# nihaomiao/CVPR23_LFDM

Measured on AMD Instinct MI355X. Metric: 40-frame 128x128 videos/sec (DDIM-100), higher is better.
Workload: dtype f32; 1 GPU; MUG 128x128, 40-frame DDIM-100 sample, batch=1 per GPU (BASELINE.json configs[1]); global_batch=1, frames=40, latent=32, image=128, sampler=DDIM-100 eta=1, cond_scale=1, parallelism=replicas x1 (videos sharded, no collective)

## Files before the change

### cvpr23_lfdm_amd/csrc/attention.hip

```cpp
#include <stdlib.h>
#include "lfdm_device.h"
#include "../../include/lfdm_hip.h"

namespace {

constexpr int HEADS = 8;
constexpr int DH = 32;
constexpr int QKV_LD = 3 * HEADS * DH;
constexpr int OUT_LD = HEADS * DH;

template <int LP>
__global__ __launch_bounds__(64) void attention_kernel(const float* __restrict__ qkv, float* __restrict__ out, int batch,
                                                       int frames, int hw, int mode, const float* __restrict__ bias,
                                                       const float* __restrict__ rot_cos,
                                                       const float* __restrict__ rot_sin) {
  constexpr int NT = LP / 16;

  const int lane = threadIdx.x & 63;
  const int l15 = lane & 15, lq = lane >> 4;
  const int L = mode == 0 ? frames : hw;
  const int64_t unit = blockIdx.x;
  const int64_t seq = unit / HEADS;
  const int head = (int)(unit - seq * HEADS);
  int64_t row0, tstride;
  if (mode == 0) {
    const int64_t b = seq / hw, pix = seq - b * hw;
    row0 = b * frames * hw + pix;
    tstride = hw;
  } else {
    row0 = seq * hw;
    tstride = 1;
  }
  const float scale = 0.17677669529663687f;
  const float* base = qkv + head * DH;

  float qf[NT][8], kf[NT][8];
#pragma unroll
  for (int ti = 0; ti < NT; ++ti) {
    const int t = ti * 16 + l15;
    float4 q0 = make_float4(0.f, 0.f, 0.f, 0.f), q1 = q0, k0 = q0, k1 = q0;
    if (t < L) {
      const float* src = base + (row0 + (int64_t)t * tstride) * QKV_LD + 8 * lq;
      q0 = *reinterpret_cast<const float4*>(src);
      q1 = *reinterpret_cast<const float4*>(src + 4);
      k0 = *reinterpret_cast<const float4*>(src + OUT_LD);
      k1 = *reinterpret_cast<const float4*>(src + OUT_LD + 4);
    }
    qf[ti][0] = q0.x * scale; qf[ti][1] = q0.y * scale; qf[ti][2] = q0.z * scale; qf[ti][3] = q0.w * scale;
    qf[ti][4] = q1.x * scale; qf[ti][5] = q1.y * scale; qf[ti][6] = q1.z * scale; qf[ti][7] = q1.w * scale;
    kf[ti][0] = k0.x; kf[ti][1] = k0.y; kf[ti][2] = k0.z; kf[ti][3] = k0.w;
    kf[ti][4] = k1.x; kf[ti][5] = k1.y; kf[ti][6] = k1.z; kf[ti][7] = k1.w;
  }
  float vf[2][4 * NT];
#pragma unroll
  for (int tj = 0; tj < NT; ++tj)
#pragma unroll
    for (int r = 0; r < 4; ++r) {
      const int t = 16 * tj + 4 * lq + r;
      vf[0][4 * tj + r] = vf[1][4 * tj + r] = 0.f;
      if (t < L) {
        const float* src = base + (row0 + (int64_t)t * tstride) * QKV_LD + 2 * OUT_LD;
        vf[0][4 * tj + r] = src[l15];
        vf[1][4 * tj + r] = src[16 + l15];
      }
    }
  if (rot_cos) {
#pragma unroll
    for (int ti = 0; ti < NT; ++ti) {
      const int t = ti * 16 + l15;
      if (t < L) {
#pragma unroll
        for (int pr = 0; pr < 4; ++pr) {
          const float c = rot_cos[t * 16 + 4 * lq + pr], sn = rot_sin[t * 16 + 4 * lq + pr];
          const float qx = qf[ti][2 * pr], qy = qf[ti][2 * pr + 1];
          const float kx = kf[ti][2 * pr], ky = kf[ti][2 * pr + 1];
          qf[ti][2 * pr] = qx * c - qy * sn;
          qf[ti][2 * pr + 1] = qy * c + qx * sn;
          kf[ti][2 * pr] = kx * c - ky * sn;
          kf[ti][2 * pr + 1] = ky * c + kx * sn;
        }
      }
    }
  }

  f32x4 st[NT][NT];
#pragma unroll
  for (int ti = 0; ti < NT; ++ti)
#pragma unroll
    for (int tj = 0; tj < NT; ++tj) {
      f32x4 acc = {0.f, 0.f, 0.f, 0.f};
#pragma unroll
      for (int s = 0; s < 8; ++s) acc = mfma_16x16x4(kf[tj][s], qf[ti][s], acc);
      st[ti][tj] = acc;
    }
  const bool bias_vec = bias && (L % 4 == 0) && ((((uintptr_t)bias) & 15) == 0);
#pragma unroll
  for (int ti = 0; ti < NT; ++ti) {
    const int qt = ti * 16 + l15;
    float m = -3.0e38f;
#pragma unroll
    for (int tj = 0; tj < NT; ++tj) {
      float bv[4] = {0.f, 0.f, 0.f, 0.f};
      const int key0 = tj * 16 + lq * 4;
      if (bias && qt < L && key0 < L) {
        const float* bp = bias + ((int64_t)head * L + qt) * L + key0;
        if (bias_vec) {
          const float4 b4 = *reinterpret_cast<const float4*>(bp);
          bv[0] = b4.x; bv[1] = b4.y; bv[2] = b4.z; bv[3] = b4.w;
        } else {
#pragma unroll
          for (int r = 0; r < 4; ++r) bv[r] = (key0 + r < L) ? bp[r] : 0.f;
        }
      }
#pragma unroll
      for (int r = 0; r < 4; ++r) {
        float v = st[ti][tj][r];
        if (key0 + r >= L) v = -3.0e38f;
        else v += bv[r];
        st[ti][tj][r] = v;
        m = fmaxf(m, v);
      }
    }
    m = fmaxf(m, __shfl_xor(m, 16));
    m = fmaxf(m, __shfl_xor(m, 32));
    float sum = 0.f;
#pragma unroll
    for (int tj = 0; tj < NT; ++tj)
#pragma unroll
      for (int r = 0; r < 4; ++r) {
        const float e = (tj * 16 + lq * 4 + r) < L ? expf(st[ti][tj][r] - m) : 0.f;
        st[ti][tj][r] = e;
        sum += e;
      }
    sum += __shfl_xor(sum, 16);
    sum += __shfl_xor(sum, 32);
#pragma unroll
    for (int tj = 0; tj < NT; ++tj)
#pragma unroll
      for (int r = 0; r < 4; ++r) st[ti][tj][r] = st[ti][tj][r] / sum;
  }

#pragma unroll
  for (int ti = 0; ti < NT; ++ti) {
    f32x4 o[2];
    o[0] = (f32x4){0.f, 0.f, 0.f, 0.f};
    o[1] = o[0];
#pragma unroll
    for (int tj = 0; tj < NT; ++tj)
#pragma unroll
      for (int r = 0; r < 4; ++r) {
        o[0] = mfma_16x16x4(st[ti][tj][r], vf[0][4 * tj + r], o[0]);
        o[1] = mfma_16x16x4(st[ti][tj][r], vf[1][4 * tj + r], o[1]);
      }
#pragma unroll
    for (int r = 0; r < 4; ++r) {
      const int t = ti * 16 + lq * 4 + r;
      if (t < L) {
        float* dst = out + (row0 + (int64_t)t * tstride) * OUT_LD + head * DH;
        dst[l15] = o[0][r];
        dst[16 + l15] = o[1][r];
      }
    }
  }
}

__global__ __launch_bounds__(256) void linattn_context_kernel(const float* __restrict__ qkv, int hw,
                                                              float* __restrict__ ctx_out) {
  __shared__ float red[4][32];
  __shared__ float kmax[32];
  __shared__ float ek[64][33];
  __shared__ __attribute__((aligned(16))) float vv[64][36];
  const int tid = threadIdx.x;
  const int f = blockIdx.x >> 3, h = blockIdx.x & 7;
  const float* kbase = qkv + (int64_t)f * hw * QKV_LD + OUT_LD + h * DH;
  const float* vbase = kbase + OUT_LD;

  {
    const int c4 = tid & 7, part = tid >> 3;
    float4 m = make_float4(-3.0e38f, -3.0e38f, -3.0e38f, -3.0e38f);
    for (int n = part; n < hw; n += 128) {
      float4 v[4];
#pragma unroll
      for (int u = 0; u < 4; ++u) {
        const int nn = n + 32 * u;
        v[u] = nn < hw ? *reinterpret_cast<const float4*>(kbase + (int64_t)nn * QKV_LD + 4 * c4) : m;
      }
#pragma unroll
      for (int u = 0; u < 4; ++u) {
        m.x = fmaxf(m.x, v[u].x); m.y = fmaxf(m.y, v[u].y); m.z = fmaxf(m.z, v[u].z); m.w = fmaxf(m.w, v[u].w);
      }
    }
#pragma unroll
    for (int x = 8; x <= 32; x <<= 1) {
      m.x = fmaxf(m.x, __shfl_xor(m.x, x)); m.y = fmaxf(m.y, __shfl_xor(m.y, x));
      m.z = fmaxf(m.z, __shfl_xor(m.z, x)); m.w = fmaxf(m.w, __shfl_xor(m.w, x));
    }
    if ((tid & 63) < 8) {
      const int w = tid >> 6;
      red[w][4 * c4 + 0] = m.x; red[w][4 * c4 + 1] = m.y; red[w][4 * c4 + 2] = m.z; red[w][4 * c4 + 3] = m.w;
    }
    __syncthreads();
    if (tid < 32) kmax[tid] = fmaxf(fmaxf(red[0][tid], red[1][tid]), fmaxf(red[2][tid], red[3][tid]));
    __syncthreads();
  }

  const int d = tid >> 3, e0 = (tid & 7) * 4;
  float acc[4] = {0.f, 0.f, 0.f, 0.f};
  float ssum = 0.f;
  const int ln = tid >> 3, lc4 = tid & 7;
  float4 rk[2], rv[2];
  auto load_tile = [&](int n0) {
#pragma unroll
    for (int u = 0; u < 2; ++u) {
      const int n = n0 + ln + 32 * u;
      rk[u] = rv[u] = make_float4(0.f, 0.f, 0.f, 0.f);
      if (n < hw) {
        rk[u] = *reinterpret_cast<const float4*>(kbase + (int64_t)n * QKV_LD + 4 * lc4);
        rv[u] = *reinterpret_cast<const float4*>(vbase + (int64_t)n * QKV_LD + 4 * lc4);
      }
    }
  };
  load_tile(0);
  for (int n0 = 0; n0 < hw; n0 += 64) {
#pragma unroll
    for (int u = 0; u < 2; ++u) {
      const int nl = ln + 32 * u;
      const bool ok = n0 + nl < hw;
      ek[nl][4 * lc4 + 0] = ok ? expf(rk[u].x - kmax[4 * lc4 + 0]) : 0.f;
      ek[nl][4 * lc4 + 1] = ok ? expf(rk[u].y - kmax[4 * lc4 + 1]) : 0.f;
      ek[nl][4 * lc4 + 2] = ok ? expf(rk[u].z - kmax[4 * lc4 + 2]) : 0.f;
      ek[nl][4 * lc4 + 3] = ok ? expf(rk[u].w - kmax[4 * lc4 + 3]) : 0.f;
      *reinterpret_cast<float4*>(&vv[nl][4 * lc4]) = rv[u];
    }
    __syncthreads();
    if (n0 + 64 < hw) load_tile(n0 + 64);
#pragma unroll 8
    for (int n = 0; n < 64; ++n) {
      const float e = ek[n][d];
      const float4 v4 = *reinterpret_cast<const float4*>(&vv[n][e0]);
      acc[0] = fmaf(e, v4.x, acc[0]);
      acc[1] = fmaf(e, v4.y, acc[1]);
      acc[2] = fmaf(e, v4.z, acc[2]);
      acc[3] = fmaf(e, v4.w, acc[3]);
      ssum += e;
    }
    __syncthreads();
  }
  float* dst = ctx_out + ((int64_t)blockIdx.x * DH + d) * DH + e0;
  dst[0] = acc[0] / ssum;
  dst[1] = acc[1] / ssum;
  dst[2] = acc[2] / ssum;
  dst[3] = acc[3] / ssum;
}

__global__ __launch_bounds__(256) void linattn_output_kernel(const float* __restrict__ qkv,
                                                             const float* __restrict__ ctx, int hw,
                                                             float* __restrict__ out) {
  constexpr int CS = DH * DH + 4;
  __shared__ __attribute__((aligned(16))) float cs[HEADS * CS];
  const int tid = threadIdx.x;
  const int f = blockIdx.y;
  for (int i = tid; i < HEADS * DH * DH; i += 256) {
    const int h = i / (DH * DH), r = i - h * DH * DH;
    cs[h * CS + r] = ctx[(int64_t)f * HEADS * DH * DH + i];
  }
  __syncthreads();
  const int tok = blockIdx.x * 32 + (tid >> 3), h = tid & 7;
  if (tok >= hw) return;
  const int64_t row = (int64_t)f * hw + tok;
  const float* qp = qkv + row * QKV_LD + h * DH;
  float q[DH];
#pragma unroll
  for (int i = 0; i < DH / 4; ++i) {
    const float4 v = reinterpret_cast<const float4*>(qp)[i];
    q[4 * i] = v.x; q[4 * i + 1] = v.y; q[4 * i + 2] = v.z; q[4 * i + 3] = v.w;
  }
  float m = q[0];
#pragma unroll
  for (int i = 1; i < DH; ++i) m = fmaxf(m, q[i]);
  float sum = 0.f;
#pragma unroll
  for (int i = 0; i < DH; ++i) {
    q[i] = expf(q[i] - m);
    sum += q[i];
  }
  const float scale = 0.17677669529663687f;
#pragma unroll
  for (int i = 0; i < DH; ++i) q[i] = q[i] / sum * scale;
  float* op = out + row * OUT_LD + h * DH;
  const float* ch = cs + h * CS;
#pragma unroll
  for (int e4 = 0; e4 < DH / 4; ++e4) {
    float4 o = make_float4(0.f, 0.f, 0.f, 0.f);
#pragma unroll
    for (int dd = 0; dd < DH; ++dd) {
      const float4 c = *reinterpret_cast<const float4*>(ch + dd * DH + 4 * e4);
      o.x = fmaf(c.x, q[dd], o.x);
      o.y = fmaf(c.y, q[dd], o.y);
      o.z = fmaf(c.z, q[dd], o.z);
      o.w = fmaf(c.w, q[dd], o.w);
    }
    reinterpret_cast<float4*>(op)[e4] = o;
  }
}

}

extern "C" int lfdm_attention_cl_f32(const float* qkv, float* out, int batch, int frames, int hw,
                                     int mode, const float* bias, const float* rot_cos,
                                     const float* rot_sin, lfdm_stream_t stream_) {
  hipStream_t stream = (hipStream_t)stream_;
  const int L = mode == 0 ? frames : hw;
  if (!qkv || !out || batch <= 0 || frames <= 0 || hw <= 0 || (mode != 0 && mode != 1) ||
      L > 64 || ((rot_cos == nullptr) != (rot_sin == nullptr))) {
    lfdm_set_error("attention: unsupported shape (sequence length must be <= 64)");
    return LFDM_EINVAL;
  }
  const int64_t nseq = mode == 0 ? (int64_t)batch * hw : (int64_t)batch * frames;
  const int64_t units = nseq * HEADS;
  const dim3 grid((unsigned)units), block(64);
  if (L <= 16) LFDM_LAUNCH((attention_kernel<16>), grid, block, 0, stream, qkv, out, batch, frames, hw, mode, bias, rot_cos, rot_sin);
  else if (L <= 32) LFDM_LAUNCH((attention_kernel<32>), grid, block, 0, stream, qkv, out, batch, frames, hw, mode, bias, rot_cos, rot_sin);
  else if (L <= 48) LFDM_LAUNCH((attention_kernel<48>), grid, block, 0, stream, qkv, out, batch, frames, hw, mode, bias, rot_cos, rot_sin);
  else LFDM_LAUNCH((attention_kernel<64>), grid, block, 0, stream, qkv, out, batch, frames, hw, mode, bias, rot_cos, rot_sin);
  return lfdm_check_launch("attention");
}

extern "C" size_t lfdm_linear_attention_ws_bytes(int n_frames) {
  return (size_t)n_frames * HEADS * DH * DH * sizeof(float);
}

extern "C" int lfdm_linear_attention_cl_f32(const float* qkv, float* out, int n_frames, int hw,
                                            void* ws, size_t ws_bytes, lfdm_stream_t stream_) {
  hipStream_t stream = (hipStream_t)stream_;
  if (!qkv || !out || n_frames <= 0 || hw <= 0) {
    lfdm_set_error("linear_attention: bad arguments");
    return LFDM_EINVAL;
  }
  if (!ws || ws_bytes < lfdm_linear_attention_ws_bytes(n_frames)) {
    lfdm_set_error("linear_attention: workspace too small");
    return LFDM_EWORKSPACE;
  }
  float* ctx = reinterpret_cast<float*>(ws);
  LFDM_LAUNCH(linattn_context_kernel, dim3(n_frames * HEADS), dim3(256), 0, stream, qkv, hw, ctx);
  LFDM_LAUNCH(linattn_output_kernel, dim3((hw + 31) / 32, n_frames), dim3(256), 0, stream, qkv,
              (const float*)ctx, hw, out);
  return lfdm_check_launch("linear_attention");
}
```

### cvpr23_lfdm_amd/csrc/attention_fused.hip

```cpp
#include <stdlib.h>

#include "lfdm_device.h"
#include "../../include/lfdm_hip.h"

namespace {

constexpr int HEADS = 8;
constexpr int DH = 32;
constexpr int OUT_LD = HEADS * DH;

#if defined(LFDM_EMU_BUILD)
static inline float fast_exp(float x) { return expf(x); }
#else
__device__ __forceinline__ float fast_exp(float x) { return __expf(x); }
#endif

template <int NT>
__device__ __forceinline__ void attend_store(const float (&qf)[NT][8], const float (&kf)[NT][8], const float (&vf)[2][4 * NT],
                                             int head, int L, int l15, int lq, const float* __restrict__ bias, bool bias_vec,
                                             float* __restrict__ out, int64_t row0, int hw, float* o_lds = nullptr) {
  f32x4 st[NT][NT];
#pragma unroll
  for (int ti = 0; ti < NT; ++ti)
#pragma unroll
    for (int tj = 0; tj < NT; ++tj) {
      f32x4 acc = {0.f, 0.f, 0.f, 0.f};
#pragma unroll
      for (int s = 0; s < 8; ++s) acc = mfma_16x16x4(kf[tj][s], qf[ti][s], acc);
      st[ti][tj] = acc;
    }
#pragma unroll
  for (int ti = 0; ti < NT; ++ti) {
    const int qt = ti * 16 + l15;
    float m = -3.0e38f;
#pragma unroll
    for (int tj = 0; tj < NT; ++tj) {
      float bv[4] = {0.f, 0.f, 0.f, 0.f};
      const int key0 = tj * 16 + lq * 4;
      if (bias && qt < L && key0 < L) {
        const float* bp = bias + ((int64_t)head * L + qt) * L + key0;
        if (bias_vec) {
          const float4 b4 = *reinterpret_cast<const float4*>(bp);
          bv[0] = b4.x; bv[1] = b4.y; bv[2] = b4.z; bv[3] = b4.w;
        } else {
#pragma unroll
          for (int r = 0; r < 4; ++r) bv[r] = (key0 + r < L) ? bp[r] : 0.f;
        }
      }
#pragma unroll
      for (int r = 0; r < 4; ++r) {
        const float v = (key0 + r >= L) ? -3.0e38f : st[ti][tj][r] + bv[r];
        st[ti][tj][r] = v;
        m = fmaxf(m, v);
      }
    }
    m = fmaxf(m, __shfl_xor(m, 16));
    m = fmaxf(m, __shfl_xor(m, 32));
    float sum = 0.f;
#pragma unroll
    for (int tj = 0; tj < NT; ++tj)
#pragma unroll
      for (int r = 0; r < 4; ++r) {
        const int key = tj * 16 + lq * 4 + r;
        const float e = key < L ? fast_exp(st[ti][tj][r] - m) : 0.f;
        st[ti][tj][r] = e;
        sum += e;
      }
    sum += __shfl_xor(sum, 16);
    sum += __shfl_xor(sum, 32);
    const float inv = 1.0f / sum;
#pragma unroll
    for (int tj = 0; tj < NT; ++tj)
#pragma unroll
      for (int r = 0; r < 4; ++r) st[ti][tj][r] = st[ti][tj][r] * inv;
  }

#pragma unroll
  for (int ti = 0; ti < NT; ++ti) {
    f32x4 o[2];
    o[0] = (f32x4){0.f, 0.f, 0.f, 0.f};
    o[1] = o[0];
#pragma unroll
    for (int tj = 0; tj < NT; ++tj)
#pragma unroll
      for (int r = 0; r < 4; ++r) {
        o[0] = mfma_16x16x4(st[ti][tj][r], vf[0][4 * tj + r], o[0]);
        o[1] = mfma_16x16x4(st[ti][tj][r], vf[1][4 * tj + r], o[1]);
      }
#pragma unroll
    for (int r = 0; r < 4; ++r) {
      const int t = ti * 16 + lq * 4 + r;
      if (t < L) {
        if (o_lds) {
#pragma unroll
          for (int half = 0; half < 2; ++half) {
            const int c = head * DH + 16 * half + l15;
            o_lds[t * OUT_LD + ((((c >> 2) ^ (t & 15)) << 2) | (c & 3))] = o[half][r];
          }
        } else {
          float* dst = out + (row0 + (int64_t)t * hw) * OUT_LD + head * DH;
          dst[l15] = o[0][r];
          dst[16 + l15] = o[1][r];
        }
      }
    }
  }
}

template <int LP, int C, bool ROT_RELOAD = false, bool WPACK = false>
__device__ __forceinline__ void tattn_heads(const float* __restrict__ x, int ldx, int head_begin, int heads_per_block,
                                            const float* __restrict__ wqkv, float* __restrict__ out, int frames, int hw, int64_t seq,
                                            const float* __restrict__ bias, const float* __restrict__ rot_cos,
                                            const float* __restrict__ rot_sin, float eps, float* o_lds) {
  constexpr int NT = LP / 16;
  constexpr int CQ = C / 4;

  const int lane = threadIdx.x & 63;
  const int l15 = lane & 15, lq = lane >> 4;
  const int L = frames;
  const int64_t b = seq / hw, pix = seq - b * hw;
  const int64_t row0 = b * frames * hw + pix;
  const float scale = 0.17677669529663687f;

  float xf[NT][CQ];
#pragma unroll
  for (int ti = 0; ti < NT; ++ti) {
    const int t = ti * 16 + l15;
    float s1 = 0.f, s2 = 0.f;
    if (t < L) {
      const float* src = x + (row0 + (int64_t)t * hw) * ldx + CQ * lq;
#pragma unroll
      for (int q = 0; q < CQ / 4; ++q) {
        const float4 v = *reinterpret_cast<const float4*>(src + 4 * q);
        xf[ti][4 * q] = v.x; xf[ti][4 * q + 1] = v.y; xf[ti][4 * q + 2] = v.z; xf[ti][4 * q + 3] = v.w;
        s1 += (v.x + v.y) + (v.z + v.w);
        s2 += (v.x * v.x + v.y * v.y) + (v.z * v.z + v.w * v.w);
      }
    } else {
#pragma unroll
      for (int s = 0; s < CQ; ++s) xf[ti][s] = 0.f;
    }
    s1 += __shfl_xor(s1, 16); s2 += __shfl_xor(s2, 16);
    s1 += __shfl_xor(s1, 32); s2 += __shfl_xor(s2, 32);
    const float mean = s1 * (1.0f / (float)C);
    float var = s2 * (1.0f / (float)C) - mean * mean;
    if (var < 0.f) var = 0.f;
    const float rstd = 1.0f / sqrtf(var + eps);
    if (t < L) {
#pragma unroll
      for (int s = 0; s < CQ; ++s) xf[ti][s] = (xf[ti][s] - mean) * rstd;
    }
  }

  float rc[NT][4], rs[NT][4];
  if (rot_cos && !ROT_RELOAD) {
#pragma unroll
    for (int ti = 0; ti < NT; ++ti) {
      const int t = ti * 16 + l15;
      const int tt = t < L ? t : 0;
#pragma unroll
      for (int fi = 0; fi < 2; ++fi)
#pragma unroll
        for (int pr = 0; pr < 2; ++pr) {
          rc[ti][2 * fi + pr] = rot_cos[tt * 16 + 8 * fi + 2 * lq + pr];
          rs[ti][2 * fi + pr] = rot_sin[tt * 16 + 8 * fi + 2 * lq + pr];
        }
    }
  }
  const bool bias_vec = bias && (L % 4 == 0) && ((((uintptr_t)bias) & 15) == 0);

#pragma unroll 1
  for (int head = head_begin; head < head_begin + heads_per_block; ++head) {
    float qf[NT][8], kf[NT][8];
    {
      float wa[4][CQ];
#pragma unroll
      for (int g = 0; g < 4; ++g) {
        const float* wsrc = WPACK ? wqkv + ((int64_t)(((g >> 1) * HEADS + head) * 2 + (g & 1)) * (CQ / 4) * 64 + lane) * 4
                                  : wqkv + ((int64_t)((g >> 1) * OUT_LD + head * DH + 16 * (g & 1) + l15)) * C + CQ * lq;
#pragma unroll
        for (int q = 0; q < CQ / 4; ++q) {
          const float4 v = *reinterpret_cast<const float4*>(wsrc + (WPACK ? 256 * q : 4 * q));
          wa[g][4 * q] = v.x; wa[g][4 * q + 1] = v.y; wa[g][4 * q + 2] = v.z; wa[g][4 * q + 3] = v.w;
        }
      }
#pragma unroll
      for (int g = 0; g < 4; ++g) {
        f32x4 acc[NT];
#pragma unroll
        for (int ti = 0; ti < NT; ++ti) acc[ti] = (f32x4){0.f, 0.f, 0.f, 0.f};
#pragma unroll
        for (int s = 0; s < CQ; ++s)
#pragma unroll
          for (int ti = 0; ti < NT; ++ti) acc[ti] = mfma_16x16x4(wa[g][s], xf[ti][s], acc[ti]);
#pragma unroll
        for (int ti = 0; ti < NT; ++ti)
#pragma unroll
          for (int r = 0; r < 4; ++r) {
            if ((g >> 1) == 0) qf[ti][4 * (g & 1) + r] = acc[ti][r] * scale;
            else kf[ti][4 * (g & 1) + r] = acc[ti][r];
          }
      }
    }
    if (rot_cos) {
#pragma unroll
      for (int ti = 0; ti < NT; ++ti) {
#pragma unroll
        for (int fi = 0; fi < 2; ++fi)
#pragma unroll
          for (int pr = 0; pr < 2; ++pr) {
            float c, sn;
            if (ROT_RELOAD) {
              const int t = ti * 16 + l15, tt = t < L ? t : 0;
              c = rot_cos[tt * 16 + 8 * fi + 2 * lq + pr];
              sn = rot_sin[tt * 16 + 8 * fi + 2 * lq + pr];
            } else {
              c = rc[ti][2 * fi + pr];
              sn = rs[ti][2 * fi + pr];
            }
            const float qx = qf[ti][4 * fi + 2 * pr], qy = qf[ti][4 * fi + 2 * pr + 1];
            const float kx = kf[ti][4 * fi + 2 * pr], ky = kf[ti][4 * fi + 2 * pr + 1];
            qf[ti][4 * fi + 2 * pr] = qx * c - qy * sn;
            qf[ti][4 * fi + 2 * pr + 1] = qy * c + qx * sn;
            kf[ti][4 * fi + 2 * pr] = kx * c - ky * sn;
            kf[ti][4 * fi + 2 * pr + 1] = ky * c + kx * sn;
          }
      }
    }
    float vf[2][4 * NT];
    {
      float wb[2][CQ];
#pragma unroll
      for (int half = 0; half < 2; ++half) {
        const float* wsrc = WPACK ? wqkv + ((int64_t)((2 * HEADS + head) * 2 + half) * (CQ / 4) * 64 + lane) * 4
                                  : wqkv + ((int64_t)(2 * OUT_LD + head * DH + 16 * half + l15)) * C + CQ * lq;
#pragma unroll
        for (int q = 0; q < CQ / 4; ++q) {
          const float4 v = *reinterpret_cast<const float4*>(wsrc + (WPACK ? 256 * q : 4 * q));
          wb[half][4 * q] = v.x; wb[half][4 * q + 1] = v.y; wb[half][4 * q + 2] = v.z; wb[half][4 * q + 3] = v.w;
        }
      }
#pragma unroll
      for (int half = 0; half < 2; ++half) {
        f32x4 acc[NT];
#pragma unroll
        for (int ti = 0; ti < NT; ++ti) acc[ti] = (f32x4){0.f, 0.f, 0.f, 0.f};
#pragma unroll
        for (int s = 0; s < CQ; ++s)
#pragma unroll
          for (int ti = 0; ti < NT; ++ti) acc[ti] = mfma_16x16x4(xf[ti][s], wb[half][s], acc[ti]);
#pragma unroll
        for (int ti = 0; ti < NT; ++ti)
#pragma unroll
          for (int r = 0; r < 4; ++r) vf[half][4 * ti + r] = acc[ti][r];
      }
    }

    attend_store<NT>(qf, kf, vf, head, L, l15, lq, bias, bias_vec, out, row0, hw, o_lds);
  }
}

template <int LP, int C>
__global__ __launch_bounds__(64, 2) void temporal_attn_fused_kernel(const float* __restrict__ x, int ldx, int heads_per_block,
                                                                 const float* __restrict__ wqkv,
                                                                 float* __restrict__ out, int batch, int frames, int hw,
                                                                 const float* __restrict__ bias,
                                                                 const float* __restrict__ rot_cos,
                                                                 const float* __restrict__ rot_sin, float eps) {
  tattn_heads<LP, C>(x, ldx, blockIdx.y * heads_per_block, heads_per_block, wqkv, out, frames, hw, blockIdx.x, bias, rot_cos, rot_sin, eps, nullptr);
}

template <int LP, int LROWS, int NW>
__global__ __launch_bounds__(64 * NW, 2) void temporal_attn_fused_out_kernel(const float* __restrict__ x, int ldx,
                                                                          const float* __restrict__ wqkv, const float* __restrict__ wout,
                                                                          float* __restrict__ out, int ldo, int frames, int hw,
                                                                          const float* __restrict__ bias, const float* __restrict__ rot_cos,
                                                                          const float* __restrict__ rot_sin, float eps) {
  constexpr int C = 64, NT = LP / 16, CT = C / 16;
  __shared__ __attribute__((aligned(16))) float o_lds[LROWS * OUT_LD];
  const int wave = lfdm_uniform((int)(threadIdx.x >> 6));
  const int lane = threadIdx.x & 63, l15 = lane & 15, lq = lane >> 4;
  const int L = frames;
  const int64_t seq = blockIdx.x;
  tattn_heads<LP, C, (NW < 8), true>(x, ldx, wave * (HEADS / NW), HEADS / NW, wqkv, nullptr, frames, hw, seq, bias, rot_cos, rot_sin, eps, o_lds);
  __syncthreads();
  const int64_t b = seq / hw, pix = seq - b * hw;
  const int64_t row0 = b * frames * hw + pix;
  for (int tile = wave; tile < NT * CT; tile += NW) {
    const int ti = tile / CT, ct = tile - ti * CT;
    const int t = ti * 16 + l15;
    const int tr = t < L ? t : L - 1;
    const float* arow = o_lds + tr * OUT_LD;
    const float* brow = wout + ((int64_t)ct * (OUT_LD / 16) * 64 + lane) * 4;
    f32x4 acc = {0.f, 0.f, 0.f, 0.f}, acc1 = acc;
    float xr[4];
#pragma unroll
    for (int r = 0; r < 4; ++r) {
      const int tok = ti * 16 + 4 * lq + r;
      xr[r] = x[(row0 + (int64_t)(tok < L ? tok : L - 1) * hw) * ldx + ct * 16 + l15];
    }
#pragma unroll 4
    for (int S = 0; S < OUT_LD / 16; S += 2) {
      const float4 a = *reinterpret_cast<const float4*>(arow + (((4 * S + lq) ^ (tr & 15)) << 2));
      const float4 a1 = *reinterpret_cast<const float4*>(arow + (((4 * S + 4 + lq) ^ (tr & 15)) << 2));
      const float4 w = *reinterpret_cast<const float4*>(brow + 256 * S);
      const float4 w1 = *reinterpret_cast<const float4*>(brow + 256 * S + 256);
      acc = mfma_16x16x4(a.x, w.x, acc);
      acc1 = mfma_16x16x4(a1.x, w1.x, acc1);
      acc = mfma_16x16x4(a.y, w.y, acc);
      acc1 = mfma_16x16x4(a1.y, w1.y, acc1);
      acc = mfma_16x16x4(a.z, w.z, acc);
      acc1 = mfma_16x16x4(a1.z, w1.z, acc1);
      acc = mfma_16x16x4(a.w, w.w, acc);
      acc1 = mfma_16x16x4(a1.w, w1.w, acc1);
    }
#pragma unroll
    for (int r = 0; r < 4; ++r) acc[r] += acc1[r];
#pragma unroll
    for (int r = 0; r < 4; ++r) {
      const int tok = ti * 16 + 4 * lq + r;
      if (tok < L) {
        const int64_t row = row0 + (int64_t)tok * hw;
        out[row * ldo + ct * 16 + l15] = acc[r] + xr[r];
      }
    }
  }
}

template <int LP>
__global__ __launch_bounds__(64, 1) void temporal_attn_fused_wide_kernel(const float* __restrict__ x, int ldx, int channels,
                                                                      int heads_per_block, const float* __restrict__ wqkv,
                                                                      float* __restrict__ out, int batch, int frames, int hw,
                                                                      const float* __restrict__ bias,
                                                                      const float* __restrict__ rot_cos,
                                                                      const float* __restrict__ rot_sin, float eps) {
  constexpr int NT = LP / 16;
  const int lane = threadIdx.x & 63;
  const int l15 = lane & 15, lq = lane >> 4;
  const int L = frames;
  const int64_t seq = blockIdx.x;
  const int64_t b = seq / hw, pix = seq - b * hw;
  const int64_t row0 = b * frames * hw + pix;
  const float scale = 0.17677669529663687f;
  const int ncb = channels / 64;

  float mean[NT], rstd[NT];
#pragma unroll
  for (int ti = 0; ti < NT; ++ti) {
    const int t = ti * 16 + l15;
    float s1 = 0.f, s2 = 0.f;
    if (t < L) {
      const float* src = x + (row0 + (int64_t)t * hw) * ldx + 16 * lq;
      for (int cb = 0; cb < ncb; ++cb)
#pragma unroll
        for (int q = 0; q < 4; ++q) {
          const float4 v = *reinterpret_cast<const float4*>(src + 64 * cb + 4 * q);
          s1 += (v.x + v.y) + (v.z + v.w);
          s2 += (v.x * v.x + v.y * v.y) + (v.z * v.z + v.w * v.w);
        }
    }
    s1 += __shfl_xor(s1, 16); s2 += __shfl_xor(s2, 16);
    s1 += __shfl_xor(s1, 32); s2 += __shfl_xor(s2, 32);
    const float m = s1 / (float)channels;
    float var = s2 / (float)channels - m * m;
    if (var < 0.f) var = 0.f;
    mean[ti] = m;
    rstd[ti] = 1.0f / sqrtf(var + eps);
  }
  const bool bias_vec = bias && (L % 4 == 0) && ((((uintptr_t)bias) & 15) == 0);

  const int head_begin = blockIdx.y * heads_per_block;
#pragma unroll 1
  for (int head = head_begin; head < head_begin + heads_per_block; ++head) {
    f32x4 aq[2][NT], ak[2][NT], av[2][NT];
#pragma unroll
    for (int g = 0; g < 2; ++g)
#pragma unroll
      for (int ti = 0; ti < NT; ++ti) aq[g][ti] = ak[g][ti] = av[g][ti] = (f32x4){0.f, 0.f, 0.f, 0.f};
#pragma unroll 1
    for (int cb = 0; cb < ncb; ++cb) {
      float w[6][16];
#pragma unroll
      for (int g = 0; g < 6; ++g) {
        const float* wsrc = wqkv + ((int64_t)((g >> 1) * OUT_LD + head * DH + 16 * (g & 1) + l15)) * channels + 64 * cb + 16 * lq;
#pragma unroll
        for (int q = 0; q < 4; ++q) {
          const float4 v = *reinterpret_cast<const float4*>(wsrc + 4 * q);
          w[g][4 * q] = v.x; w[g][4 * q + 1] = v.y; w[g][4 * q + 2] = v.z; w[g][4 * q + 3] = v.w;
        }
      }
#pragma unroll
      for (int ti = 0; ti < NT; ++ti) {
        const int t = ti * 16 + l15;
        float xf[16];
        if (t < L) {
          const float* src = x + (row0 + (int64_t)t * hw) * ldx + 64 * cb + 16 * lq;
#pragma unroll
          for (int q = 0; q < 4; ++q) {
            const float4 v = *reinterpret_cast<const float4*>(src + 4 * q);
            xf[4 * q] = (v.x - mean[ti]) * rstd[ti]; xf[4 * q + 1] = (v.y - mean[ti]) * rstd[ti];
            xf[4 * q + 2] = (v.z - mean[ti]) * rstd[ti]; xf[4 * q + 3] = (v.w - mean[ti]) * rstd[ti];
          }
        } else {
#pragma unroll
          for (int s2 = 0; s2 < 16; ++s2) xf[s2] = 0.f;
        }
#pragma unroll
        for (int s2 = 0; s2 < 16; ++s2) {
          aq[0][ti] = mfma_16x16x4(w[0][s2], xf[s2], aq[0][ti]);
          aq[1][ti] = mfma_16x16x4(w[1][s2], xf[s2], aq[1][ti]);
          ak[0][ti] = mfma_16x16x4(w[2][s2], xf[s2], ak[0][ti]);
          ak[1][ti] = mfma_16x16x4(w[3][s2], xf[s2], ak[1][ti]);
          av[0][ti] = mfma_16x16x4(xf[s2], w[4][s2], av[0][ti]);
          av[1][ti] = mfma_16x16x4(xf[s2], w[5][s2], av[1][ti]);
        }
      }
    }
    float qf[NT][8], kf[NT][8], vf[2][4 * NT];
#pragma unroll
    for (int ti = 0; ti < NT; ++ti)
#pragma unroll
      for (int fi = 0; fi < 2; ++fi)
#pragma unroll
        for (int r = 0; r < 4; ++r) {
          qf[ti][4 * fi + r] = aq[fi][ti][r] * scale;
          kf[ti][4 * fi + r] = ak[fi][ti][r];
          vf[fi][4 * ti + r] = av[fi][ti][r];
        }
    if (rot_cos) {
#pragma unroll
      for (int ti = 0; ti < NT; ++ti) {
        const int t = ti * 16 + l15;
        const int tt = t < L ? t : 0;
#pragma unroll
        for (int fi = 0; fi < 2; ++fi)
#pragma unroll
          for (int pr = 0; pr < 2; ++pr) {
            const float c = rot_cos[tt * 16 + 8 * fi + 2 * lq + pr], sn = rot_sin[tt * 16 + 8 * fi + 2 * lq + pr];
            const float qx = qf[ti][4 * fi + 2 * pr], qy = qf[ti][4 * fi + 2 * pr + 1];
            const float kx = kf[ti][4 * fi + 2 * pr], ky = kf[ti][4 * fi + 2 * pr + 1];
            qf[ti][4 * fi + 2 * pr] = qx * c - qy * sn;
            qf[ti][4 * fi + 2 * pr + 1] = qy * c + qx * sn;
            kf[ti][4 * fi + 2 * pr] = kx * c - ky * sn;
            kf[ti][4 * fi + 2 * pr + 1] = ky * c + kx * sn;
          }
      }
    }
    attend_store<NT>(qf, kf, vf, head, L, l15, lq, bias, bias_vec, out, row0, hw);
  }
}

int launch_fused_wide(const float* x, int ldx, int channels, const float* wqkv, float* out, int batch, int frames, int hw,
                      const float* bias, const float* rot_cos, const float* rot_sin, float eps, hipStream_t stream) {
  const int64_t nseq = (int64_t)batch * hw;
  int hpb = 8;
  while (hpb > 1 && nseq * (HEADS / hpb) < 2048) hpb >>= 1;
  const dim3 grid((unsigned)nseq, (unsigned)(HEADS / hpb)), block(64);
  if (frames <= 16) LFDM_LAUNCH((temporal_attn_fused_wide_kernel<16>), grid, block, 0, stream, x, ldx, channels, hpb, wqkv, out, batch, frames, hw, bias, rot_cos, rot_sin, eps);
  else if (frames <= 32) LFDM_LAUNCH((temporal_attn_fused_wide_kernel<32>), grid, block, 0, stream, x, ldx, channels, hpb, wqkv, out, batch, frames, hw, bias, rot_cos, rot_sin, eps);
  else if (frames <= 48) LFDM_LAUNCH((temporal_attn_fused_wide_kernel<48>), grid, block, 0, stream, x, ldx, channels, hpb, wqkv, out, batch, frames, hw, bias, rot_cos, rot_sin, eps);
  else LFDM_LAUNCH((temporal_attn_fused_wide_kernel<64>), grid, block, 0, stream, x, ldx, channels, hpb, wqkv, out, batch, frames, hw, bias, rot_cos, rot_sin, eps);
  return lfdm_check_launch("temporal_attention_fused_wide");
}

template <int C>
int launch_fused(const float* x, int ldx, const float* wqkv, float* out, int batch, int frames, int hw, const float* bias,
                 const float* rot_cos, const float* rot_sin, float eps, hipStream_t stream) {
  const int64_t nseq = (int64_t)batch * hw;
  int hpb = 8;
  while (hpb > 1 && nseq * (HEADS / hpb) < 2048) hpb >>= 1;
  if (const char* e = lfdm_knob("LFDM_TATTN_HPB")) {
    const int v = atoi(e);
    if (v == 1 || v == 2 || v == 4 || v == 8) hpb = v;
  }
  const dim3 grid((unsigned)nseq, (unsigned)(HEADS / hpb)), block(64);
  if (frames <= 16) LFDM_LAUNCH((temporal_attn_fused_kernel<16, C>), grid, block, 0, stream, x, ldx, hpb, wqkv, out, batch, frames, hw, bias, rot_cos, rot_sin, eps);
  else if (frames <= 32) LFDM_LAUNCH((temporal_attn_fused_kernel<32, C>), grid, block, 0, stream, x, ldx, hpb, wqkv, out, batch, frames, hw, bias, rot_cos, rot_sin, eps);
  else if (frames <= 48) LFDM_LAUNCH((temporal_attn_fused_kernel<48, C>), grid, block, 0, stream, x, ldx, hpb, wqkv, out, batch, frames, hw, bias, rot_cos, rot_sin, eps);
  else LFDM_LAUNCH((temporal_attn_fused_kernel<64, C>), grid, block, 0, stream, x, ldx, hpb, wqkv, out, batch, frames, hw, bias, rot_cos, rot_sin, eps);
  return lfdm_check_launch("temporal_attention_fused");
}

template <int LP, int LROWS>
int launch_fused_out_lp(const float* x, int ldx, const float* wqkv, const float* wout, float* out, int ldo, int batch, int frames, int hw,
                        const float* bias, const float* rot_cos, const float* rot_sin, float eps, hipStream_t stream) {
  const int64_t nseq = (int64_t)batch * hw;
  int nw = 2;
  while (nw < 8 && nseq * nw < 2048) nw <<= 1;
  if (const char* e = getenv("LFDM_TATTN_OUT_NW")) {
    const int v = atoi(e);
    if (v == 1 || v == 2 || v == 4 || v == 8) nw = v;
  }
  const dim3 grid((unsigned)nseq);
  if (nw == 1) LFDM_LAUNCH((temporal_attn_fused_out_kernel<LP, LROWS, 1>), grid, dim3(64), 0, stream, x, ldx, wqkv, wout, out, ldo, frames, hw, bias, rot_cos, rot_sin, eps);
  else if (nw == 2) LFDM_LAUNCH((temporal_attn_fused_out_kernel<LP, LROWS, 2>), grid, dim3(128), 0, stream, x, ldx, wqkv, wout, out, ldo, frames, hw, bias, rot_cos, rot_sin, eps);
  else if (nw == 4) LFDM_LAUNCH((temporal_attn_fused_out_kernel<LP, LROWS, 4>), grid, dim3(256), 0, stream, x, ldx, wqkv, wout, out, ldo, frames, hw, bias, rot_cos, rot_sin, eps);
  else LFDM_LAUNCH((temporal_attn_fused_out_kernel<LP, LROWS, 8>), grid, dim3(512), 0, stream, x, ldx, wqkv, wout, out, ldo, frames, hw, bias, rot_cos, rot_sin, eps);
  return lfdm_check_launch("temporal_attention_fused_out");
}

}

extern "C" int lfdm_temporal_attention_fused_out_cl_f32(const float* x, int ldx, int channels, const float* wqkv, const float* wout,
                                                        float* out, int ldo, int batch, int frames, int hw, const float* bias,
                                                        const float* rot_cos, const float* rot_sin, float ln_eps, lfdm_stream_t stream_) {
  hipStream_t stream = (hipStream_t)stream_;
  if (!x || !wqkv || !wout || !out || batch <= 0 || frames <= 0 || frames > 64 || hw <= 0 || channels != 64 || ldx < 64 || ldx % 4 != 0 ||
      ldo < 64 || (((uintptr_t)x | (uintptr_t)wqkv | (uintptr_t)wout) & 15) || ((rot_cos == nullptr) != (rot_sin == nullptr)) || out == x) {
    lfdm_set_error("temporal_attention_fused_out: needs C == 64, frames <= 64, 16-byte aligned rows, out != x");
    return LFDM_EINVAL;
  }
  if (frames <= 16) return launch_fused_out_lp<16, 16>(x, ldx, wqkv, wout, out, ldo, batch, frames, hw, bias, rot_cos, rot_sin, ln_eps, stream);
  if (frames <= 32) return launch_fused_out_lp<32, 32>(x, ldx, wqkv, wout, out, ldo, batch, frames, hw, bias, rot_cos, rot_sin, ln_eps, stream);
  if (frames <= 40) return launch_fused_out_lp<48, 40>(x, ldx, wqkv, wout, out, ldo, batch, frames, hw, bias, rot_cos, rot_sin, ln_eps, stream);
  if (frames <= 48) return launch_fused_out_lp<48, 48>(x, ldx, wqkv, wout, out, ldo, batch, frames, hw, bias, rot_cos, rot_sin, ln_eps, stream);
  return launch_fused_out_lp<64, 64>(x, ldx, wqkv, wout, out, ldo, batch, frames, hw, bias, rot_cos, rot_sin, ln_eps, stream);
}

extern "C" int lfdm_temporal_attention_fused_cl_f32(const float* x, int ldx, int channels, const float* wqkv, float* out,
                                                    int batch, int frames, int hw, const float* bias,
                                                    const float* rot_cos, const float* rot_sin, float ln_eps,
                                                    lfdm_stream_t stream_) {
  hipStream_t stream = (hipStream_t)stream_;
  if (!x || !wqkv || !out || batch <= 0 || frames <= 0 || frames > 64 || hw <= 0 || ldx < channels || ldx % 4 != 0 ||
      (((uintptr_t)x | (uintptr_t)wqkv) & 15) || ((rot_cos == nullptr) != (rot_sin == nullptr)) ||
      channels < 64 || channels % 64 != 0) {
    lfdm_set_error("temporal_attention_fused: needs C % 64 == 0, frames <= 64, 16-byte aligned rows");
    return LFDM_EINVAL;
  }
  if (channels == 64) return launch_fused<64>(x, ldx, wqkv, out, batch, frames, hw, bias, rot_cos, rot_sin, ln_eps, stream);
  return launch_fused_wide(x, ldx, channels, wqkv, out, batch, frames, hw, bias, rot_cos, rot_sin, ln_eps, stream);
}
```

### cvpr23_lfdm_amd/csrc/attn_lowres.hip

```cpp
#include <stdlib.h>

#include "lfdm_device.h"
#include "../../include/lfdm_hip.h"

namespace {

constexpr int HEADS = 8;
constexpr int DH = 32;
constexpr int OUT_LD = HEADS * DH;
constexpr int NQ = 3 * DH;
constexpr int LDQ = NQ + 4;
constexpr float ATT_SCALE = 0.17677669529663687f;

template <int NT, int D>
__device__ __forceinline__ void project_wave_d(const float* __restrict__ x, int ldx, int64_t row0, int64_t rstride, int nrows,
                                               int c_begin, int c_end, const float* __restrict__ wf, int C, int head,
                                               f32x4 (&acc)[NT][6], float (&s1)[NT], float (&s2)[NT]) {
  const int lane = threadIdx.x & 63, l15 = lane & 15, ks = lane >> 4;
  const float* arow[NT];
#pragma unroll
  for (int ti = 0; ti < NT; ++ti) {
    int r = 16 * ti + l15;
    if (r >= nrows) r = nrows - 1;
    arow[ti] = x + (row0 + (int64_t)r * rstride) * ldx + 4 * ks;
    s1[ti] = s2[ti] = 0.f;
  }
  const float* brow[6];
#pragma unroll
  for (int nj = 0; nj < 6; ++nj) {
    const int gcol = (nj >> 1) * OUT_LD + head * DH + (nj & 1) * 16 + l15;
    brow[nj] = wf + (int64_t)gcol * C + 4 * ks;
#pragma unroll
    for (int ti = 0; ti < NT; ++ti) acc[ti][nj] = (f32x4){0.f, 0.f, 0.f, 0.f};
  }
  float4 ra[D][NT], rb[D][6];
  const int last = c_end - 16;
#pragma unroll
  for (int d = 0; d < D; ++d) {
    const int c = c_begin + 16 * d < last ? c_begin + 16 * d : last;
#pragma unroll
    for (int ti = 0; ti < NT; ++ti) ra[d][ti] = *reinterpret_cast<const float4*>(arow[ti] + c);
#pragma unroll
    for (int nj = 0; nj < 6; ++nj) rb[d][nj] = *reinterpret_cast<const float4*>(brow[nj] + c);
  }
  for (int c0 = c_begin; c0 < c_end; c0 += 16 * D) {
#pragma unroll
    for (int d = 0; d < D; ++d) {
      float4 a[NT], b[6];
#pragma unroll
      for (int ti = 0; ti < NT; ++ti) a[ti] = ra[d][ti];
#pragma unroll
      for (int nj = 0; nj < 6; ++nj) b[nj] = rb[d][nj];
      const int cn = c0 + 16 * (d + D) < last ? c0 + 16 * (d + D) : last;
#pragma unroll
      for (int ti = 0; ti < NT; ++ti) ra[d][ti] = *reinterpret_cast<const float4*>(arow[ti] + cn);
#pragma unroll
      for (int nj = 0; nj < 6; ++nj) rb[d][nj] = *reinterpret_cast<const float4*>(brow[nj] + cn);
#pragma unroll
      for (int ti = 0; ti < NT; ++ti) {
        s1[ti] += (a[ti].x + a[ti].y) + (a[ti].z + a[ti].w);
        s2[ti] += (a[ti].x * a[ti].x + a[ti].y * a[ti].y) + (a[ti].z * a[ti].z + a[ti].w * a[ti].w);
      }
#pragma unroll
      for (int nj = 0; nj < 6; ++nj)
#pragma unroll
        for (int ti = 0; ti < NT; ++ti) {
          acc[ti][nj] = mfma_16x16x4(a[ti].x, b[nj].x, acc[ti][nj]);
          acc[ti][nj] = mfma_16x16x4(a[ti].y, b[nj].y, acc[ti][nj]);
          acc[ti][nj] = mfma_16x16x4(a[ti].z, b[nj].z, acc[ti][nj]);
          acc[ti][nj] = mfma_16x16x4(a[ti].w, b[nj].w, acc[ti][nj]);
        }
    }
  }
#pragma unroll
  for (int ti = 0; ti < NT; ++ti) {
    s1[ti] += __shfl_xor(s1[ti], 16); s2[ti] += __shfl_xor(s2[ti], 16);
    s1[ti] += __shfl_xor(s1[ti], 32); s2[ti] += __shfl_xor(s2[ti], 32);
  }
}

template <int NT, int G, int D>
__device__ __forceinline__ void project_wave_asm(const float* __restrict__ x, int ldx, int64_t row0, int64_t rstride, int nrows,
                                                 int c_begin, const float* __restrict__ wf, int C, int head,
                                                 f32x4 (&acc)[NT][6], float (&s1)[NT], float (&s2)[NT]) {
  const int lane = threadIdx.x & 63, l15 = lane & 15, ks = lane >> 4;
  const float* arow[NT];
#pragma unroll
  for (int ti = 0; ti < NT; ++ti) {
    int r = 16 * ti + l15;
    if (r >= nrows) r = nrows - 1;
    arow[ti] = x + (row0 + (int64_t)r * rstride) * ldx + c_begin + 4 * ks;
    s1[ti] = s2[ti] = 0.f;
  }
  const float* brow[6];
#pragma unroll
  for (int nj = 0; nj < 6; ++nj) {
    const int gcol = (nj >> 1) * OUT_LD + head * DH + (nj & 1) * 16 + l15;
    brow[nj] = wf + (int64_t)gcol * C + c_begin + 4 * ks;
#pragma unroll
    for (int ti = 0; ti < NT; ++ti) acc[ti][nj] = (f32x4){0.f, 0.f, 0.f, 0.f};
  }
  f32x4 ra[D][NT], rb[D][6];
  auto issue = [&](auto gc) {
    constexpr int g = decltype(gc)::value, st = g % D;
    lfdm_static_for<0, NT>([&](auto ti) { lfdm_gload_f4<64 * g>(ra[st][decltype(ti)::value], arow[decltype(ti)::value]); });
    lfdm_static_for<0, 6>([&](auto nj) { lfdm_gload_f4<64 * g>(rb[st][decltype(nj)::value], brow[decltype(nj)::value]); });
  };
  lfdm_static_for<0, (D < G ? D : G)>(issue);
  lfdm_static_for<0, G>([&](auto gc) {
    constexpr int g = decltype(gc)::value, st = g % D;
    constexpr int younger = (G - 1 - g) < (D - 1) ? (G - 1 - g) : (D - 1);
    lfdm_vmwait<younger * (NT + 6)>();
#pragma unroll
    for (int ti = 0; ti < NT; ++ti) lfdm_tie(ra[st][ti]);
#pragma unroll
    for (int nj = 0; nj < 6; ++nj) lfdm_tie(rb[st][nj]);
    f32x4 a[NT], b[6];
#pragma unroll
    for (int ti = 0; ti < NT; ++ti) a[ti] = ra[st][ti];
#pragma unroll
    for (int nj = 0; nj < 6; ++nj) b[nj] = rb[st][nj];
    if constexpr (NT <= 2 && g + D < G) issue(std::integral_constant<int, g + D>{});
#pragma unroll
    for (int ti = 0; ti < NT; ++ti) {
      s1[ti] += (a[ti][0] + a[ti][1]) + (a[ti][2] + a[ti][3]);
      s2[ti] += (a[ti][0] * a[ti][0] + a[ti][1] * a[ti][1]) + (a[ti][2] * a[ti][2] + a[ti][3] * a[ti][3]);
    }
#pragma unroll
    for (int e = 0; e < 4; ++e)
#pragma unroll
      for (int nj = 0; nj < 6; ++nj)
#pragma unroll
        for (int ti = 0; ti < NT; ++ti) acc[ti][nj] = mfma_16x16x4(a[ti][e], b[nj][e], acc[ti][nj]);
    if constexpr (NT > 2 && g + D < G) issue(std::integral_constant<int, g + D>{});
  });
#pragma unroll
  for (int ti = 0; ti < NT; ++ti) {
    s1[ti] += __shfl_xor(s1[ti], 16); s2[ti] += __shfl_xor(s2[ti], 16);
    s1[ti] += __shfl_xor(s1[ti], 32); s2[ti] += __shfl_xor(s2[ti], 32);
  }
}

template <int NT, bool ASM = true>
__device__ __forceinline__ void project_wave(const float* __restrict__ x, int ldx, int64_t row0, int64_t rstride, int nrows,
                                             int c_begin, int c_end, const float* __restrict__ wf, int C, int head,
                                             f32x4 (&acc)[NT][6], float (&s1)[NT], float (&s2)[NT]) {
  const int groups = ASM ? (c_end - c_begin) >> 4 : 0;
  constexpr int D = NT == 1 ? 4 : 2;
  if (groups == 8) project_wave_asm<NT, 8, D>(x, ldx, row0, rstride, nrows, c_begin, wf, C, head, acc, s1, s2);
  else if (groups == 4) project_wave_asm<NT, 4, D>(x, ldx, row0, rstride, nrows, c_begin, wf, C, head, acc, s1, s2);
  else if (groups == 2) project_wave_asm<NT, 2, 2>(x, ldx, row0, rstride, nrows, c_begin, wf, C, head, acc, s1, s2);
  else project_wave_d<NT, 1>(x, ldx, row0, rstride, nrows, c_begin, c_end, wf, C, head, acc, s1, s2);
}

template <int NT, bool ASM = true>
__device__ __forceinline__ void project_ksplit(const float* __restrict__ x, int ldx, int64_t row0, int64_t rstride, int nrows,
                                               const float* __restrict__ wf, int C, int head, float eps, float* part,
                                               float* pstat, float* wsl, float wsum_val) {
  constexpr int R = 16 * NT;
  const int tid = threadIdx.x, lane = tid & 63, wave = tid >> 6, l15 = lane & 15, ks = lane >> 4;
  f32x4 acc[NT][6];
  float s1[NT], s2[NT];
  const int cw = C / 4;
  project_wave<NT, ASM>(x, ldx, row0, rstride, nrows, wave * cw, (wave + 1) * cw, wf, C, head, acc, s1, s2);
  float* mine = part + wave * (R * LDQ);
  if (tid < NQ) wsl[tid] = wsum_val;
#pragma unroll
  for (int ti = 0; ti < NT; ++ti) {
    if (ks == 0) {
      pstat[(0 * 4 + wave) * R + 16 * ti + l15] = s1[ti];
      pstat[(1 * 4 + wave) * R + 16 * ti + l15] = s2[ti];
    }
#pragma unroll
    for (int nj = 0; nj < 6; ++nj)
#pragma unroll
      for (int r = 0; r < 4; ++r) mine[(16 * ti + 4 * ks + r) * LDQ + 16 * nj + l15] = acc[ti][nj][r];
  }
  __syncthreads();
  const float inv_c = 1.0f / (float)C;
  for (int it = tid; it < R * (NQ / 4); it += 256) {
    const int row = it / (NQ / 4), q4 = it - row * (NQ / 4);
    float sv = 0.f, qv = 0.f;
#pragma unroll
    for (int w = 0; w < 4; ++w) {
      sv += pstat[(0 * 4 + w) * R + row];
      qv += pstat[(1 * 4 + w) * R + row];
    }
    const float mean = sv * inv_c;
    float var = qv * inv_c - mean * mean;
    if (var < 0.f) var = 0.f;
    const float rstd = 1.0f / sqrtf(var + eps);
    float4 v = *reinterpret_cast<const float4*>(part + row * LDQ + 4 * q4);
#pragma unroll
    for (int w = 1; w < 4; ++w) {
      const float4 u = *reinterpret_cast<const float4*>(part + w * (R * LDQ) + row * LDQ + 4 * q4);
      v.x += u.x; v.y += u.y; v.z += u.z; v.w += u.w;
    }
    const float4 ws = *reinterpret_cast<const float4*>(wsl + 4 * q4);
    v.x = rstd * (v.x - mean * ws.x); v.y = rstd * (v.y - mean * ws.y);
    v.z = rstd * (v.z - mean * ws.z); v.w = rstd * (v.w - mean * ws.w);
    *reinterpret_cast<float4*>(part + row * LDQ + 4 * q4) = v;
  }
  __syncthreads();
}

__device__ __forceinline__ float load_wsum(const float* __restrict__ wsum, int head) {
  const int tid = threadIdx.x;
  return tid < NQ ? wsum[(tid >> 5) * OUT_LD + head * DH + (tid & 31)] : 0.f;
}

template <int NT, bool MSPLIT>
__global__ __launch_bounds__(256) void linattn_lowres_kernel(const float* __restrict__ x, int ldx, int C,
                                                             const float* __restrict__ wf, const float* __restrict__ wsum,
                                                             float* __restrict__ out, int hw, float eps) {
  constexpr int R = 16 * NT;
  constexpr int ROWS = MSPLIT ? 4 * R : R;
  __shared__ __attribute__((aligned(16))) float qkv[(MSPLIT ? ROWS : 4 * R) * LDQ];
  __shared__ float pstat[2 * 4 * R];
  __shared__ __attribute__((aligned(16))) float wsl[NQ];
  __shared__ float red[8][DH], kmax[DH], ksum[DH];
  __shared__ __attribute__((aligned(16))) float ctx[DH][DH + 4];
  const int tid = threadIdx.x, lane = tid & 63, wave = tid >> 6, l15 = lane & 15, ks = lane >> 4;
  const int f = blockIdx.x >> 3, head = blockIdx.x & 7;
  const int64_t row0 = (int64_t)f * hw;
  const float wsum_val = load_wsum(wsum, head);

  if (MSPLIT) {
    f32x4 acc[NT][6];
    float s1[NT], s2[NT];
    const int nrows_w = hw - wave * R;
    project_wave<NT>(x, ldx, row0 + wave * R, 1, nrows_w < R ? nrows_w : R, 0, C, wf, C, head, acc, s1, s2);
    if (tid < NQ) wsl[tid] = wsum_val;
    if (ks == 0) {
#pragma unroll
      for (int ti = 0; ti < NT; ++ti) {
        const float mean = s1[ti] / (float)C;
        float var = s2[ti] / (float)C - mean * mean;
        if (var < 0.f) var = 0.f;
        pstat[wave * R + 16 * ti + l15] = mean;
        pstat[4 * R + wave * R + 16 * ti + l15] = 1.0f / sqrtf(var + eps);
      }
    }
    __syncthreads();
#pragma unroll
    for (int ti = 0; ti < NT; ++ti)
#pragma unroll
      for (int r = 0; r < 4; ++r) {
        const int rl = 16 * ti + 4 * ks + r;
        const float mean = pstat[wave * R + rl], rstd = pstat[4 * R + wave * R + rl];
#pragma unroll
        for (int nj = 0; nj < 6; ++nj)
          qkv[(wave * R + rl) * LDQ + 16 * nj + l15] = rstd * (acc[ti][nj][r] - mean * wsl[16 * nj + l15]);
      }
    __syncthreads();
  } else {
    project_ksplit<NT>(x, ldx, row0, 1, hw, wf, C, head, eps, qkv, pstat, wsl, wsum_val);
  }

  {
    const int d = tid & 31, part = tid >> 5;
    float m = -3.0e38f;
    for (int n = part; n < hw; n += 8) m = fmaxf(m, qkv[n * LDQ + DH + d]);
    red[part][d] = m;
    __syncthreads();
    if (tid < DH) {
      float mm = red[0][tid];
#pragma unroll
      for (int p = 1; p < 8; ++p) mm = fmaxf(mm, red[p][tid]);
      kmax[tid] = mm;
    }
    __syncthreads();
    const float mx = kmax[d];
    float s = 0.f;
    for (int n = part; n < hw; n += 8) {
      const float e = expf(qkv[n * LDQ + DH + d] - mx);
      qkv[n * LDQ + DH + d] = e;
      s += e;
    }
    red[part][d] = s;
    __syncthreads();
    if (tid < DH) {
      float ss = 0.f;
#pragma unroll
      for (int p = 0; p < 8; ++p) ss += red[p][tid];
      ksum[tid] = ss;
    }
    __syncthreads();
  }
  {
    const int d = tid >> 3, e0 = (tid & 7) * 4;
    float a0 = 0.f, a1 = 0.f, a2 = 0.f, a3 = 0.f;
    for (int n = 0; n < hw; ++n) {
      const float e = qkv[n * LDQ + DH + d];
      const float4 v4 = *reinterpret_cast<const float4*>(qkv + n * LDQ + 2 * DH + e0);
      a0 = fmaf(e, v4.x, a0); a1 = fmaf(e, v4.y, a1); a2 = fmaf(e, v4.z, a2); a3 = fmaf(e, v4.w, a3);
    }
    const float ss = ksum[d];
    *reinterpret_cast<float4*>(&ctx[d][e0]) = make_float4(a0 / ss, a1 / ss, a2 / ss, a3 / ss);
  }
  for (int n0 = 0; n0 < hw; n0 += 32) {
    const bool live = n0 + (tid >> 3) < hw;
    const int n = live ? n0 + (tid >> 3) : hw - 1;
    float4 q4 = *reinterpret_cast<const float4*>(qkv + n * LDQ + 4 * (tid & 7));
    float m = fmaxf(fmaxf(q4.x, q4.y), fmaxf(q4.z, q4.w));
    m = fmaxf(m, __shfl_xor(m, 1)); m = fmaxf(m, __shfl_xor(m, 2)); m = fmaxf(m, __shfl_xor(m, 4));
    q4.x = expf(q4.x - m); q4.y = expf(q4.y - m); q4.z = expf(q4.z - m); q4.w = expf(q4.w - m);
    float s = (q4.x + q4.y) + (q4.z + q4.w);
    s += __shfl_xor(s, 1); s += __shfl_xor(s, 2); s += __shfl_xor(s, 4);
    q4.x = q4.x / s * ATT_SCALE; q4.y = q4.y / s * ATT_SCALE; q4.z = q4.z / s * ATT_SCALE; q4.w = q4.w / s * ATT_SCALE;
    if (live) *reinterpret_cast<float4*>(qkv + n * LDQ + 4 * (tid & 7)) = q4;
  }
  __syncthreads();
  for (int it = tid; it < hw * 8; it += 256) {
    const int n = it >> 3, e0 = (it & 7) * 4;
    float4 o = make_float4(0.f, 0.f, 0.f, 0.f);
#pragma unroll
    for (int d4 = 0; d4 < DH / 4; ++d4) {
      const float4 q4 = *reinterpret_cast<const float4*>(qkv + n * LDQ + 4 * d4);
      const float qd[4] = {q4.x, q4.y, q4.z, q4.w};
#pragma unroll
      for (int i = 0; i < 4; ++i) {
        const float4 c4 = *reinterpret_cast<const float4*>(&ctx[4 * d4 + i][e0]);
        o.x = fmaf(c4.x, qd[i], o.x); o.y = fmaf(c4.y, qd[i], o.y); o.z = fmaf(c4.z, qd[i], o.z); o.w = fmaf(c4.w, qd[i], o.w);
      }
    }
    *reinterpret_cast<float4*>(out + (row0 + n) * OUT_LD + head * DH + e0) = o;
  }
}

template <int NT>
__global__ __launch_bounds__(256) void attn_lowres_kernel(const float* __restrict__ x, int ldx, int C,
                                                          const float* __restrict__ wf, const float* __restrict__ wsum,
                                                          float* __restrict__ out, int frames, int hw, int mode,
                                                          const float* __restrict__ bias, const float* __restrict__ rot_cos,
                                                          const float* __restrict__ rot_sin, float eps) {
  constexpr int R = 16 * NT;
  __shared__ __attribute__((aligned(16))) float qkv[4 * R * LDQ];
  __shared__ float pstat[2 * 4 * R];
  __shared__ __attribute__((aligned(16))) float wsl[NQ];
  const int tid = threadIdx.x, lane = tid & 63, wave = tid >> 6, l15 = lane & 15, lq = lane >> 4;
  const int64_t unit = blockIdx.x;
  const int64_t seq = unit >> 3;
  const int head = (int)(unit & 7);
  int64_t row0, tstride;
  if (mode == 0) {
    const int64_t b = seq / hw, pix = seq - b * hw;
    row0 = b * frames * hw + pix;
    tstride = hw;
  } else {
    row0 = seq * hw;
    tstride = 1;
  }
  const int L = mode == 0 ? frames : hw;
  const float wsum_val = load_wsum(wsum, head);
  project_ksplit<NT, (NT <= 3)>(x, ldx, row0, tstride, L, wf, C, head, eps, qkv, pstat, wsl, wsum_val);

  for (int ti = wave; ti < NT; ti += 4) {
    float qf[8], kf[NT][8];
    {
      const int t = ti * 16 + l15;
      const float* src = qkv + t * LDQ + 8 * lq;
      const float4 q0 = *reinterpret_cast<const float4*>(src), q1 = *reinterpret_cast<const float4*>(src + 4);
      qf[0] = q0.x * ATT_SCALE; qf[1] = q0.y * ATT_SCALE; qf[2] = q0.z * ATT_SCALE; qf[3] = q0.w * ATT_SCALE;
      qf[4] = q1.x * ATT_SCALE; qf[5] = q1.y * ATT_SCALE; qf[6] = q1.z * ATT_SCALE; qf[7] = q1.w * ATT_SCALE;
      if (rot_cos && t < L) {
#pragma unroll
        for (int pr = 0; pr < 4; ++pr) {
          const float c = rot_cos[t * 16 + 4 * lq + pr], sn = rot_sin[t * 16 + 4 * lq + pr];
          const float qx = qf[2 * pr], qy = qf[2 * pr + 1];
          qf[2 * pr] = qx * c - qy * sn;
          qf[2 * pr + 1] = qy * c + qx * sn;
        }
      }
    }
#pragma unroll
    for (int tj = 0; tj < NT; ++tj) {
      const int t = tj * 16 + l15;
      const float* src = qkv + t * LDQ + DH + 8 * lq;
      const float4 k0 = *reinterpret_cast<const float4*>(src), k1 = *reinterpret_cast<const float4*>(src + 4);
      kf[tj][0] = k0.x; kf[tj][1] = k0.y; kf[tj][2] = k0.z; kf[tj][3] = k0.w;
      kf[tj][4] = k1.x; kf[tj][5] = k1.y; kf[tj][6] = k1.z; kf[tj][7] = k1.w;
      if (rot_cos && t < L) {
#pragma unroll
        for (int pr = 0; pr < 4; ++pr) {
          const float c = rot_cos[t * 16 + 4 * lq + pr], sn = rot_sin[t * 16 + 4 * lq + pr];
          const float kx = kf[tj][2 * pr], ky = kf[tj][2 * pr + 1];
          kf[tj][2 * pr] = kx * c - ky * sn;
          kf[tj][2 * pr + 1] = ky * c + kx * sn;
        }
      }
    }
    f32x4 st[NT];
#pragma unroll
    for (int tj = 0; tj < NT; ++tj) {
      f32x4 a = {0.f, 0.f, 0.f, 0.f};
#pragma unroll
      for (int s = 0; s < 8; ++s) a = mfma_16x16x4(kf[tj][s], qf[s], a);
      st[tj] = a;
    }
    const int qt = ti * 16 + l15;
    float m = -3.0e38f;
#pragma unroll
    for (int tj = 0; tj < NT; ++tj)
#pragma unroll
      for (int r = 0; r < 4; ++r) {
        const int key = tj * 16 + lq * 4 + r;
        float v = st[tj][r];
        if (key >= L) v = -3.0e38f;
        else if (bias && qt < L) v += bias[((int64_t)head * L + qt) * L + key];
        st[tj][r] = v;
        m = fmaxf(m, v);
      }
    m = fmaxf(m, __shfl_xor(m, 16));
    m = fmaxf(m, __shfl_xor(m, 32));
    float sum = 0.f;
#pragma unroll
    for (int tj = 0; tj < NT; ++tj)
#pragma unroll
      for (int r = 0; r < 4; ++r) {
        const float e = (tj * 16 + lq * 4 + r) < L ? expf(st[tj][r] - m) : 0.f;
        st[tj][r] = e;
        sum += e;
      }
    sum += __shfl_xor(sum, 16);
    sum += __shfl_xor(sum, 32);
    f32x4 o0 = {0.f, 0.f, 0.f, 0.f}, o1 = o0;
#pragma unroll
    for (int tj = 0; tj < NT; ++tj)
#pragma unroll
      for (int r = 0; r < 4; ++r) {
        const float p = st[tj][r] / sum;
        const float* vr = qkv + (16 * tj + 4 * lq + r) * LDQ + 2 * DH;
        o0 = mfma_16x16x4(p, vr[l15], o0);
        o1 = mfma_16x16x4(p, vr[16 + l15], o1);
      }
#pragma unroll
    for (int r = 0; r < 4; ++r) {
      const int t = ti * 16 + lq * 4 + r;
      if (t < L) {
        float* dst = out + (row0 + (int64_t)t * tstride) * OUT_LD + head * DH;
        dst[l15] = o0[r];
        dst[16 + l15] = o1[r];
      }
    }
  }
}

bool lowres_args_ok(const float* x, int ldx, int channels, const float* wqkv, const float* wsum, const float* out) {
  return x && wqkv && wsum && out && channels >= 64 && channels % 64 == 0 && ldx >= channels && ldx % 4 == 0 &&
         ((((uintptr_t)x) | ((uintptr_t)wqkv) | ((uintptr_t)out)) & 15) == 0;
}

}

extern "C" int lfdm_linear_attention_lowres_cl_f32(const float* x, int ldx, int channels, const float* wqkv, const float* wsum,
                                                   float* out, int n_frames, int hw, float ln_eps, lfdm_stream_t stream_) {
  hipStream_t stream = (hipStream_t)stream_;
  if (!lowres_args_ok(x, ldx, channels, wqkv, wsum, out) || n_frames <= 0 || hw <= 0 || hw > 256 || (int64_t)n_frames * HEADS > 0x7fffffff) {
    lfdm_set_error("linear_attention_lowres: needs C % 64 == 0, 1 <= hw <= 256 pixels per frame, 16-byte aligned rows");
    return LFDM_EINVAL;
  }
  const dim3 grid((unsigned)(n_frames * HEADS)), block(256);
  if (hw <= 16) LFDM_LAUNCH((linattn_lowres_kernel<1, false>), grid, block, 0, stream, x, ldx, channels, wqkv, wsum, out, hw, ln_eps);
  else if (hw <= 32) LFDM_LAUNCH((linattn_lowres_kernel<2, false>), grid, block, 0, stream, x, ldx, channels, wqkv, wsum, out, hw, ln_eps);
  else if (hw <= 64) LFDM_LAUNCH((linattn_lowres_kernel<4, false>), grid, block, 0, stream, x, ldx, channels, wqkv, wsum, out, hw, ln_eps);
  else if (hw > 192) LFDM_LAUNCH((linattn_lowres_kernel<4, true>), grid, block, 0, stream, x, ldx, channels, wqkv, wsum, out, hw, ln_eps);
  else {
    lfdm_set_error("linear_attention_lowres: 64 < hw <= 192 pixels per frame is not built (use the unfused entry points)");
    return LFDM_EINVAL;
  }
  return lfdm_check_launch("linear_attention_lowres");
}

extern "C" int lfdm_attention_lowres_cl_f32(const float* x, int ldx, int channels, const float* wqkv, const float* wsum,
                                            float* out, int batch, int frames, int hw, int mode, const float* bias,
                                            const float* rot_cos, const float* rot_sin, float ln_eps, lfdm_stream_t stream_) {
  hipStream_t stream = (hipStream_t)stream_;
  const int L = mode == 0 ? frames : hw;
  const int64_t nseq = mode == 0 ? (int64_t)batch * hw : (int64_t)batch * frames;
  if (!lowres_args_ok(x, ldx, channels, wqkv, wsum, out) || batch <= 0 || frames <= 0 || hw <= 0 || (mode != 0 && mode != 1) || L > 64 ||
      ((rot_cos == nullptr) != (rot_sin == nullptr)) || nseq * HEADS > 0x7fffffff) {
    lfdm_set_error("attention_lowres: needs C % 64 == 0, <= 64 tokens per sequence, 16-byte aligned rows");
    return LFDM_EINVAL;
  }
  const dim3 grid((unsigned)(nseq * HEADS)), block(256);
  if (L <= 16) LFDM_LAUNCH((attn_lowres_kernel<1>), grid, block, 0, stream, x, ldx, channels, wqkv, wsum, out, frames, hw, mode, bias, rot_cos, rot_sin, ln_eps);
  else if (L <= 32) LFDM_LAUNCH((attn_lowres_kernel<2>), grid, block, 0, stream, x, ldx, channels, wqkv, wsum, out, frames, hw, mode, bias, rot_cos, rot_sin, ln_eps);
  else if (L <= 48) LFDM_LAUNCH((attn_lowres_kernel<3>), grid, block, 0, stream, x, ldx, channels, wqkv, wsum, out, frames, hw, mode, bias, rot_cos, rot_sin, ln_eps);
  else LFDM_LAUNCH((attn_lowres_kernel<4>), grid, block, 0, stream, x, ldx, channels, wqkv, wsum, out, frames, hw, mode, bias, rot_cos, rot_sin, ln_eps);
  return lfdm_check_launch("attention_lowres");
}
```

### cvpr23_lfdm_amd/csrc/conv_pw.hip

```cpp
#include <stdlib.h>

#include "lfdm_device.h"
#include "../../include/lfdm_hip.h"

namespace {

template <int TN, int KW, bool LN, bool GATHER = false>
__global__ __launch_bounds__(256) void conv_pw_kernel(lfdm_conv_params p, int gx, int ny) {
  constexpr int NW = 4 / KW;
  constexpr int LD = 36;
  __shared__ __attribute__((aligned(16))) float scratch[4 * 32 * LD];
  __shared__ float s_ln[2][4][32];
  constexpr int BN = (4 / KW) * TN * 32;
  __shared__ __attribute__((aligned(16))) float s_ga[BN], s_gb[BN];
  __shared__ float s_gstat[2][64];

  const int tid = threadIdx.x, lane = tid & 63;
  const int wave = lfdm_uniform(tid >> 6);
  const int wk = wave % KW, wn = wave / KW;
  const int id = blockIdx.x, slot = id >> 3;
  const int bx = (id & 7) + 8 * (slot / ny), by = slot % ny;
  if (bx >= gx) return;
  const int M = p.n_img * p.hq * p.wq;
  const int m0 = bx * 32;
  const int n0 = by * (NW * TN * 32);
  const int K = GATHER ? p.kh * p.kw * p.c0 : p.c0 + p.c1;
  const int kw_len = K / KW;
  const int kbeg = wk * kw_len;
  const int ng = kw_len >> 5;
  const int l31 = lane & 31, kh = lane >> 5;

  const int64_t in_rows = GATHER ? (int64_t)p.n_img * p.hi * p.wi : (int64_t)M;
  const lfdm_buf buf0 = lfdm_make_buf(p.src0, (uint32_t)(((in_rows - 1) * p.ld0 + p.c0) * 4));
  const lfdm_buf buf1 = p.c1 > 0 ? lfdm_make_buf(p.src1, (uint32_t)(((int64_t)(M - 1) * p.ld1 + p.c1) * 4)) : buf0;
  const bool wpk = p.weight_pw != nullptr;
  const lfdm_buf bufw = lfdm_make_buf(wpk ? p.weight_pw : p.weight, (uint32_t)((int64_t)(K >> 5) * p.coutp * 128));
  const uint32_t ustride = wpk ? 1024u : 32u;
  const int row = m0 + l31;
  const bool row_ok = row < M;
  int g_pix0 = 0;
  unsigned g_valid = 0;
  if (GATHER && row_ok) {
    const int ox = row % p.wq, t1 = row / p.wq;
    const int oy = t1 % p.hq, n = t1 / p.hq;
    const int iy0 = oy * p.stride - p.pad_y, ix0 = ox * p.stride - p.pad_x;
    g_pix0 = (n * p.hi + iy0) * p.wi + ix0;
    for (int ky = 0; ky < p.kh; ++ky)
      for (int kx = 0; kx < p.kw; ++kx)
        if (iy0 + ky >= 0 && iy0 + ky < p.hi && ix0 + kx >= 0 && ix0 + kx < p.wi) g_valid |= 1u << (ky * p.kw + kx);
  }
  const uint32_t a_off0 = row_ok ? ((uint32_t)row * (uint32_t)p.ld0 + 4u * kh) * 4u : LFDM_BUF_OOB;
  const uint32_t a_off1 = row_ok ? ((uint32_t)row * (uint32_t)p.ld1 + 4u * kh) * 4u : LFDM_BUF_OOB;
  uint32_t b_off[TN];
#pragma unroll
  for (int j = 0; j < TN; ++j) {
    const int n = n0 + (wn * TN + j) * 32 + l31;
    b_off[j] = n >= p.coutp ? LFDM_BUF_OOB : wpk ? (uint32_t)(n >> 5) * 4096u + (uint32_t)lane * 16u : ((uint32_t)n * 32u + 4u * kh) * 4u;
  }
  const uint32_t wgroup_bytes = (uint32_t)p.coutp * 128u;

  f32x16 acc[TN];
#pragma unroll
  for (int j = 0; j < TN; ++j)
#pragma unroll
    for (int r = 0; r < 16; ++r) acc[j][r] = 0.f;
  float ln_s = 0.f, ln_q = 0.f;

  float4 ra[4], rb[4][TN];
  auto fetch = [&](int g) {
    const int kk = kbeg + 32 * g;
    const bool second = !GATHER && kk >= p.c0;
    const lfdm_buf buf = second ? buf1 : buf0;
    uint32_t abase = second ? a_off1 + (uint32_t)(kk - p.c0) * 4u : a_off0 + (uint32_t)kk * 4u;
    bool a_ok = row_ok;
    if (GATHER) {
      const int tap = kk / p.c0, cch = kk - tap * p.c0;
      const int ky = tap / p.kw, kx = tap - ky * p.kw;
      a_ok = (g_valid >> tap) & 1u;
      abase = ((uint32_t)(g_pix0 + ky * p.wi + kx) * (uint32_t)p.ld0 + (uint32_t)cch + 4u * kh) * 4u;
    }
    const uint32_t wbase = (uint32_t)(kk >> 5) * wgroup_bytes;
#pragma unroll
    for (int u = 0; u < 4; ++u) {
      ra[u] = lfdm_buf_load_f4(buf, a_ok ? abase + 32u * u : LFDM_BUF_OOB);
#pragma unroll
      for (int j = 0; j < TN; ++j)
        rb[u][j] = lfdm_buf_load_f4(bufw, b_off[j] == LFDM_BUF_OOB ? LFDM_BUF_OOB : wbase + b_off[j] + ustride * u);
    }
  };

  fetch(0);
  if (p.res_gn_partial) {
    const int groups = p.res_gn_groups, nchunk = p.res_gn_nchunk, cg = p.cout / groups;
    const int b = m0 / p.res_gn_pixels;
    const int g_lo = n0 / cg;
    const int g_hi = (((n0 + BN < p.cout ? n0 + BN : p.cout) - 1) / cg);
    const int sub = tid & 31;
    const int pcol = n0 + tid;
    const bool pcol_ok = tid < BN && pcol < p.cout;
    const float pre_gamma = p.res_gn_gamma[pcol_ok ? pcol : 0], pre_beta = p.res_gn_beta[pcol_ok ? pcol : 0];
    for (int g0 = g_lo; g0 <= g_hi; g0 += 8) {
      const int g = g0 + (tid >> 5);
      double sm = 0.0, sq = 0.0;
      if (g <= g_hi) {
        const float2* src = reinterpret_cast<const float2*>(p.res_gn_partial) + ((int64_t)b * nchunk) * groups + g;
        int k = sub;
        for (; k + 96 < nchunk; k += 128) {
          const float2 v0 = src[(int64_t)k * groups], v1 = src[(int64_t)(k + 32) * groups];
          const float2 v2 = src[(int64_t)(k + 64) * groups], v3 = src[(int64_t)(k + 96) * groups];
          sm += (double)v0.x; sq += (double)v0.y;
          sm += (double)v1.x; sq += (double)v1.y;
          sm += (double)v2.x; sq += (double)v2.y;
          sm += (double)v3.x; sq += (double)v3.y;
        }
        for (; k < nchunk; k += 32) {
          const float2 v = src[(int64_t)k * groups];
          sm += (double)v.x;
          sq += (double)v.y;
        }
      }
      for (int msk = 16; msk >= 1; msk >>= 1) {
        sm += __shfl_xor(sm, msk);
        sq += __shfl_xor(sq, msk);
      }
      if (g <= g_hi && sub == 0) {
        const double n = (double)p.res_gn_pixels * (double)cg;
        const double mean = sm / n;
        double var = sq / n - mean * mean;
        if (var < 0.0) var = 0.0;
        s_gstat[0][g - g_lo] = (float)mean;
        s_gstat[1][g - g_lo] = (float)(1.0 / sqrt(var + (double)p.res_gn_eps));
      }
    }
    __syncthreads();
    if (pcol_ok) {
      const int g = pcol / cg - g_lo;
      const float a = s_gstat[1][g] * pre_gamma;
      s_ga[tid] = a;
      s_gb[tid] = pre_beta - s_gstat[0][g] * a;
    }
    if constexpr (BN > 256) {
      for (int c = tid + 256; c < BN; c += 256) {
        const int col = n0 + c;
        if (col >= p.cout) break;
        const int g = col / cg - g_lo;
        const float a = s_gstat[1][g] * p.res_gn_gamma[col];
        s_ga[c] = a;
        s_gb[c] = p.res_gn_beta[col] - s_gstat[0][g] * a;
      }
    }
  }
  for (int g = 0; g < ng; ++g) {
    float4 a[4], b[4][TN];
#pragma unroll
    for (int u = 0; u < 4; ++u) {
      a[u] = ra[u];
#pragma unroll
      for (int j = 0; j < TN; ++j) b[u][j] = rb[u][j];
    }
    fetch(g + 1 < ng ? g + 1 : g);
#pragma unroll
    for (int u = 0; u < 4; ++u) {
      if (LN) {
        ln_s += (a[u].x + a[u].y) + (a[u].z + a[u].w);
        ln_q += (a[u].x * a[u].x + a[u].y * a[u].y) + (a[u].z * a[u].z + a[u].w * a[u].w);
      }
#pragma unroll
      for (int j = 0; j < TN; ++j) {
        acc[j] = mfma_32x32x2(a[u].x, b[u][j].x, acc[j]);
        acc[j] = mfma_32x32x2(a[u].y, b[u][j].y, acc[j]);
        acc[j] = mfma_32x32x2(a[u].z, b[u][j].z, acc[j]);
        acc[j] = mfma_32x32x2(a[u].w, b[u][j].w, acc[j]);
      }
    }
  }

  if (LN) {
    ln_s += __shfl_xor(ln_s, 32);
    ln_q += __shfl_xor(ln_q, 32);
    if (lane < 32) {
      s_ln[0][wave][l31] = ln_s;
      s_ln[1][wave][l31] = ln_q;
    }
  }

  const int trow = tid >> 3, c4 = tid & 7;
  const int orow = m0 + trow;
  const bool vec_row = orow < M;
  float mean = 0.f, rstd = 1.f;
  constexpr int NP = NW * TN;
  float4 pre_b[NP], pre_w[NP], pre_r[NP];
#pragma unroll
  for (int g = 0; g < NW; ++g)
#pragma unroll
    for (int j = 0; j < TN; ++j) {
      const int col = n0 + (g * TN + j) * 32 + 4 * c4;
      const bool ok = vec_row && col < p.cout;
      const float4 z = make_float4(0.f, 0.f, 0.f, 0.f);
      pre_b[g * TN + j] = (ok && p.bias) ? *reinterpret_cast<const float4*>(p.bias + col) : z;
      pre_w[g * TN + j] = (LN && ok) ? *reinterpret_cast<const float4*>(p.ln_wsum + col) : z;
      pre_r[g * TN + j] = (ok && p.residual) ? *reinterpret_cast<const float4*>(p.residual + (int64_t)orow * p.ldr + col) : z;
    }
#pragma unroll
  for (int j = 0; j < TN; ++j) {
    if (j > 0) __syncthreads();
#pragma unroll
    for (int r = 0; r < 16; ++r)
      scratch[wave * (32 * LD) + ((r & 3) + 8 * (r >> 2) + 4 * kh) * LD + l31] = acc[j][r];
    __syncthreads();
    if (LN && j == 0) {
      float sv = 0.f, qv = 0.f;
#pragma unroll
      for (int k = 0; k < KW; ++k) {
        sv += s_ln[0][k][trow];
        qv += s_ln[1][k][trow];
      }
      const float inv_c = 1.0f / (float)K;
      mean = sv * inv_c;
      float var = qv * inv_c - mean * mean;
      if (var < 0.f) var = 0.f;
      rstd = 1.0f / sqrtf(var + p.ln_eps);
    }
#pragma unroll
    for (int g = 0; g < NW; ++g) {
      float4 v = *reinterpret_cast<const float4*>(scratch + (g * KW) * (32 * LD) + trow * LD + 4 * c4);
#pragma unroll
      for (int k = 1; k < KW; ++k) {
        const float4 u = *reinterpret_cast<const float4*>(scratch + (g * KW + k) * (32 * LD) + trow * LD + 4 * c4);
        v.x += u.x; v.y += u.y; v.z += u.z; v.w += u.w;
      }
      const int col = n0 + (g * TN + j) * 32 + 4 * c4;
      if (!vec_row || col >= p.cout) continue;
      if (LN) {
        const float4 ws = pre_w[g * TN + j];
        v.x = rstd * (v.x - mean * ws.x); v.y = rstd * (v.y - mean * ws.y);
        v.z = rstd * (v.z - mean * ws.z); v.w = rstd * (v.w - mean * ws.w);
      }
      {
        const float4 bb = pre_b[g * TN + j];
        float4 rr = pre_r[g * TN + j];
        if (p.res_gn_partial) {
          const float4 ga = *reinterpret_cast<const float4*>(s_ga + col - n0), gb = *reinterpret_cast<const float4*>(s_gb + col - n0);
          rr.x = siluf_(fmaf(rr.x, ga.x, gb.x)); rr.y = siluf_(fmaf(rr.y, ga.y, gb.y));
          rr.z = siluf_(fmaf(rr.z, ga.z, gb.z)); rr.w = siluf_(fmaf(rr.w, ga.w, gb.w));
        }
        v.x += bb.x + rr.x; v.y += bb.y + rr.y; v.z += bb.z + rr.z; v.w += bb.w + rr.w;
      }
      if (p.act) {
        v.x = apply_act(v.x, p.act); v.y = apply_act(v.y, p.act);
        v.z = apply_act(v.z, p.act); v.w = apply_act(v.w, p.act);
      }
      *reinterpret_cast<float4*>(p.out + (int64_t)orow * p.ldo + col) = v;
    }
  }
}

template <int TN, int KW>
void launch_pw(const lfdm_conv_params& p, int gx, int ny, hipStream_t stream) {
  const dim3 grid((unsigned)(((gx + 7) / 8) * 8 * ny)), block(256);
  if (p.kh * p.kw > 1) {
    if constexpr (TN <= 2 && KW == 4) LFDM_LAUNCH((conv_pw_kernel<TN, 4, false, true>), grid, block, 0, stream, p, gx, ny);
    return;
  }
  if (p.ln_wsum) LFDM_LAUNCH((conv_pw_kernel<TN, KW, true>), grid, block, 0, stream, p, gx, ny);
  else LFDM_LAUNCH((conv_pw_kernel<TN, KW, false>), grid, block, 0, stream, p, gx, ny);
}

int env_int(const char* name, int dflt) {
  const char* e = lfdm_knob(name);
  return e ? atoi(e) : dflt;
}

}

void lfdm_conv_pw_shape(const lfdm_conv_params& p, int* tn, int* kw) {
  const int K = p.kh * p.kw > 1 ? p.kh * p.kw * p.c0 : p.c0 + p.c1;
  const int64_t M = (int64_t)p.n_img * p.hq * p.wq;
  if (p.kh * p.kw > 1) {
    *tn = (p.coutp % 64 == 0 && ((M + 31) / 32) * (p.coutp / 64) >= 256) ? 2 : 1;
    *kw = 4;
    return;
  }
  int k = K % 128 == 0 ? 4 : K % 64 == 0 ? 2 : 1;
  const int fk = env_int("LFDM_PW_KW", 0);
  if ((fk == 1 || fk == 2 || fk == 4) && K % (32 * fk) == 0) k = fk;
  int t = (M <= 1024 && p.coutp >= 768 && p.coutp % ((4 / k) * 96) == 0) ? 3 : 1;
  const int ft = env_int("LFDM_PW_TN", 0);
  if (ft >= 1 && ft <= 3) t = ft;
  *tn = t;
  *kw = k;
}

int lfdm_conv_pw_launch(const lfdm_conv_params& p, hipStream_t stream) {
  int tn, kw;
  lfdm_conv_pw_shape(p, &tn, &kw);
  const int64_t M = (int64_t)p.n_img * p.hq * p.wq;
  const int gx = (int)((M + 31) / 32);
  const int bn = (4 / kw) * tn * 32;
  const int ny = (p.coutp + bn - 1) / bn;
#define LFDM_PW_CASE(T, W) if (tn == T && kw == W) launch_pw<T, W>(p, gx, ny, stream)
  LFDM_PW_CASE(1, 4); else LFDM_PW_CASE(2, 4); else LFDM_PW_CASE(3, 4);
  else LFDM_PW_CASE(1, 2); else LFDM_PW_CASE(2, 2); else LFDM_PW_CASE(3, 2);
  else LFDM_PW_CASE(1, 1); else LFDM_PW_CASE(2, 1); else LFDM_PW_CASE(3, 1);
#undef LFDM_PW_CASE
  return lfdm_check_launch("conv_pw");
}
```

### cvpr23_lfdm_amd/csrc/lfdm_device.h

```cpp
#pragma once
#include <stddef.h>
#include <stdint.h>
#include <type_traits>

#if defined(LFDM_EMU_BUILD)
#include "hip_emu.h"
typedef emu_f32x16 f32x16;
typedef emu_f32x4 f32x4;
#define LFDM_LAUNCH(kern, grid, block, smem, stream, ...) \
  emu::launch(grid, block, smem, [=]() { kern(__VA_ARGS__); })
static inline f32x16 mfma_32x32x2(float a, float b, f32x16 c) { return emu_mfma_32x32x2(a, b, c); }
static inline f32x4 mfma_16x16x4(float a, float b, f32x4 c) { return emu_mfma_16x16x4(a, b, c); }
static inline f32x4 mfma_4x4x1(float a, float b, f32x4 c) { return emu_mfma_4x4x1(a, b, c); }
struct lfdm_bf16x8 { uint16_t h[8]; };
static inline uint16_t lfdm_f32_to_bf16(float f) {
  uint32_t u;
  memcpy(&u, &f, 4);
  if ((u & 0x7fffffffu) > 0x7f800000u) return (uint16_t)((u >> 16) | 0x40u);
  u += 0x7fffu + ((u >> 16) & 1u);
  return (uint16_t)(u >> 16);
}
static inline float lfdm_bf16_to_f32(uint16_t h) {
  const uint32_t u = (uint32_t)h << 16;
  float f;
  memcpy(&f, &u, 4);
  return f;
}
static inline lfdm_bf16x8 lfdm_cvt_bf16x8(float4 a0, float4 a1) {
  const float f[8] = {a0.x, a0.y, a0.z, a0.w, a1.x, a1.y, a1.z, a1.w};
  lfdm_bf16x8 r;
  for (int i = 0; i < 8; ++i) r.h[i] = lfdm_f32_to_bf16(f[i]);
  return r;
}
static inline uint32_t lfdm_cvt_pk_bf16(float lo, float hi) { return (uint32_t)lfdm_f32_to_bf16(lo) | ((uint32_t)lfdm_f32_to_bf16(hi) << 16); }
static inline lfdm_bf16x8 lfdm_bf16x8_bits(float4 v) {
  lfdm_bf16x8 r;
  memcpy(&r, &v, 16);
  return r;
}
static inline f32x16 mfma_32x32x16_bf16(lfdm_bf16x8 a, lfdm_bf16x8 b, f32x16 c) {
  struct Pair { lfdm_bf16x8 a, b; };
  struct Whole { lfdm_bf16x8 a[2], b[2]; };
  const unsigned lane = emu::lane_id(), h = lane >> 5;
  const Pair other = emu::wave_read_from(Pair{a, b}, lane ^ 32u);
  Whole mine;
  mine.a[h] = a;
  mine.a[1 - h] = other.a;
  mine.b[h] = b;
  mine.b[1 - h] = other.b;
  for (int r = 0; r < 16; ++r) {
    const unsigned row = (r & 3) + 8 * (r >> 2) + 4 * h;
    const Whole src = emu::wave_read_from(mine, row);
    float acc = c[r];
    for (int k = 0; k < 16; ++k)
      acc = fmaf(lfdm_bf16_to_f32(src.a[k >> 3].h[k & 7]), lfdm_bf16_to_f32(mine.b[k >> 3].h[k & 7]), acc);
    c[r] = acc;
  }
  return c;
}
#else
#include <hip/hip_runtime.h>
typedef float f32x16 __attribute__((ext_vector_type(16)));
typedef float f32x4 __attribute__((ext_vector_type(4)));
#define LFDM_LAUNCH(kern, grid, block, smem, stream, ...) \
  hipLaunchKernelGGL(kern, grid, block, smem, stream, __VA_ARGS__)
__device__ __forceinline__ f32x16 mfma_32x32x2(float a, float b, f32x16 c) {
  return __builtin_amdgcn_mfma_f32_32x32x2f32(a, b, c, 0, 0, 0);
}
__device__ __forceinline__ f32x4 mfma_16x16x4(float a, float b, f32x4 c) {
  return __builtin_amdgcn_mfma_f32_16x16x4f32(a, b, c, 0, 0, 0);
}
__device__ __forceinline__ f32x4 mfma_4x4x1(float a, float b, f32x4 c) {
  return __builtin_amdgcn_mfma_f32_4x4x1f32(a, b, c, 0, 0, 0);
}
typedef __bf16 lfdm_bf16x8 __attribute__((ext_vector_type(8)));
typedef __bf16 lfdm_bf16x2 __attribute__((ext_vector_type(2)));
typedef float lfdm_f32x8 __attribute__((ext_vector_type(8)));
typedef float lfdm_f32x2 __attribute__((ext_vector_type(2)));
__device__ __forceinline__ lfdm_bf16x8 lfdm_cvt_bf16x8(float4 a0, float4 a1) {
  const lfdm_f32x8 f = {a0.x, a0.y, a0.z, a0.w, a1.x, a1.y, a1.z, a1.w};
  return __builtin_convertvector(f, lfdm_bf16x8);
}
__device__ __forceinline__ uint32_t lfdm_cvt_pk_bf16(float lo, float hi) {
  const lfdm_f32x2 f = {lo, hi};
  return __builtin_bit_cast(uint32_t, __builtin_convertvector(f, lfdm_bf16x2));
}
__device__ __forceinline__ lfdm_bf16x8 lfdm_bf16x8_bits(float4 v) { return __builtin_bit_cast(lfdm_bf16x8, v); }
__device__ __forceinline__ f32x16 mfma_32x32x16_bf16(lfdm_bf16x8 a, lfdm_bf16x8 b, f32x16 c) {
  return __builtin_amdgcn_mfma_f32_32x32x16_bf16(a, b, c, 0, 0, 0);
}
#endif

#define LFDM_WAVE 64

template <int BEGIN, int END, class F>
__device__ __forceinline__ void lfdm_static_for(F&& f) {
  if constexpr (BEGIN < END) {
    f(std::integral_constant<int, BEGIN>{});
    lfdm_static_for<BEGIN + 1, END>(f);
  }
}

#if defined(LFDM_EMU_BUILD)
struct lfdm_buf {
  const char* base;
  uint32_t bytes;
};
static inline lfdm_buf lfdm_make_buf(const void* p, uint32_t bytes) { return lfdm_buf{(const char*)p, bytes}; }
static inline float4 lfdm_buf_load_f4(lfdm_buf b, uint32_t off) {
  float4 v = make_float4(0.f, 0.f, 0.f, 0.f);
  if ((uint64_t)off + 16u <= (uint64_t)b.bytes) memcpy(&v, b.base + off, 16);
  return v;
}
static inline float2 lfdm_buf_load_f2(lfdm_buf b, uint32_t off) {
  float2 v = make_float2(0.f, 0.f);
  if ((uint64_t)off + 8u <= (uint64_t)b.bytes) memcpy(&v, b.base + off, 8);
  return v;
}
#else
typedef __amdgpu_buffer_rsrc_t lfdm_buf;
typedef int lfdm_i32x4 __attribute__((ext_vector_type(4)));
__device__ __forceinline__ lfdm_buf lfdm_make_buf(const void* p, uint32_t bytes) {
  return __builtin_amdgcn_make_buffer_rsrc(const_cast<void*>(p), 0, (int)bytes, 0x00020000);
}
__device__ __forceinline__ float4 lfdm_buf_load_f4(lfdm_buf b, uint32_t off) {
  const lfdm_i32x4 v = __builtin_amdgcn_raw_buffer_load_b128(b, (int)off, 0, 0);
  float4 f;
  f.x = __int_as_float(v.x);
  f.y = __int_as_float(v.y);
  f.z = __int_as_float(v.z);
  f.w = __int_as_float(v.w);
  return f;
}
typedef int lfdm_i32x2 __attribute__((ext_vector_type(2)));
__device__ __forceinline__ float2 lfdm_buf_load_f2(lfdm_buf b, uint32_t off) {
  const lfdm_i32x2 v = __builtin_amdgcn_raw_buffer_load_b64(b, (int)off, 0, 0);
  return make_float2(__int_as_float(v.x), __int_as_float(v.y));
}
#endif
#define LFDM_BUF_OOB 0xFFFFFFF0u

#if defined(LFDM_EMU_BUILD)
static inline void lfdm_buf_store_f4_sc1(lfdm_buf b, uint32_t off, float4 v) {
  if ((uint64_t)off + 16u <= (uint64_t)b.bytes) memcpy(const_cast<char*>(b.base) + off, &v, 16);
}
static inline float4 lfdm_buf_load_f4_sc1(lfdm_buf b, uint32_t off) { return lfdm_buf_load_f4(b, off); }
#else
__device__ __forceinline__ void lfdm_buf_store_f4_sc1(lfdm_buf b, uint32_t off, float4 v) {
  lfdm_i32x4 d;
  d.x = __float_as_int(v.x); d.y = __float_as_int(v.y); d.z = __float_as_int(v.z); d.w = __float_as_int(v.w);
  __builtin_amdgcn_raw_buffer_store_b128(d, b, (int)off, 0, 16);
}
__device__ __forceinline__ float4 lfdm_buf_load_f4_sc1(lfdm_buf b, uint32_t off) {
  const lfdm_i32x4 v = __builtin_amdgcn_raw_buffer_load_b128(b, (int)off, 0, 16);
  float4 f;
  f.x = __int_as_float(v.x); f.y = __int_as_float(v.y); f.z = __int_as_float(v.z); f.w = __int_as_float(v.w);
  return f;
}
#endif

#if defined(LFDM_EMU_BUILD)
template <int OFF = 0> static inline void lfdm_gload_f4(f32x4& dst, const float* p) { memcpy(&dst, (const char*)p + OFF, 16); }
template <int N> static inline void lfdm_vmwait() {}
template <int N> static inline void lfdm_vmwait(f32x4&) {}
template <int N> static inline void lfdm_vmwait(f32x4&, f32x4&) {}
template <int N> static inline void lfdm_vmwait(f32x4&, f32x4&, f32x4&, f32x4&) {}
static inline void lfdm_tie(f32x4&) {}
static inline int lfdm_uniform(int v) { return v; }
#else
template <int OFF = 0>
__device__ __forceinline__ void lfdm_gload_f4(f32x4& dst, const float* p) {
  asm volatile("global_load_dwordx4 %0, %1, off offset:%2" : "=v"(dst) : "v"(p), "n"(OFF) : "memory");
}
template <int N> __device__ __forceinline__ void lfdm_vmwait() { asm volatile("s_waitcnt vmcnt(%0)" ::"n"(N) : "memory"); }
template <int N> __device__ __forceinline__ void lfdm_vmwait(f32x4& a) { asm volatile("s_waitcnt vmcnt(%1)" : "+v"(a) : "n"(N) : "memory"); }
template <int N> __device__ __forceinline__ void lfdm_vmwait(f32x4& a, f32x4& b) {
  asm volatile("s_waitcnt vmcnt(%2)" : "+v"(a), "+v"(b) : "n"(N) : "memory");
}
template <int N> __device__ __forceinline__ void lfdm_vmwait(f32x4& a, f32x4& b, f32x4& c, f32x4& d) {
  asm volatile("s_waitcnt vmcnt(%4)" : "+v"(a), "+v"(b), "+v"(c), "+v"(d) : "n"(N) : "memory");
}
__device__ __forceinline__ void lfdm_tie(f32x4& a) { asm volatile("" : "+v"(a)::"memory"); }
__device__ __forceinline__ int lfdm_uniform(int v) { return __builtin_amdgcn_readfirstlane(v); }
#endif

#if defined(LFDM_EMU_BUILD)
#define LFDM_DRAIN_STORES() ((void)0)
#define LFDM_FENCE_RELEASE_AGENT() ((void)0)
#define LFDM_FENCE_ACQUIRE_AGENT() ((void)0)
static inline unsigned lfdm_ticket_take(unsigned* c) { return __atomic_fetch_add(c, 1u, __ATOMIC_SEQ_CST); }
static inline void lfdm_ticket_reset(unsigned* c) { __atomic_store_n(c, 0u, __ATOMIC_SEQ_CST); }
#else
#define LFDM_DRAIN_STORES() asm volatile("s_waitcnt vmcnt(0)" ::: "memory")
#define LFDM_FENCE_RELEASE_AGENT() __builtin_amdgcn_fence(__ATOMIC_RELEASE, "agent")
#define LFDM_FENCE_ACQUIRE_AGENT() __builtin_amdgcn_fence(__ATOMIC_ACQUIRE, "agent")
__device__ __forceinline__ unsigned lfdm_ticket_take(unsigned* c) {
  return __hip_atomic_fetch_add(c, 1u, __ATOMIC_RELAXED, __HIP_MEMORY_SCOPE_AGENT);
}
__device__ __forceinline__ void lfdm_ticket_reset(unsigned* c) {
  __hip_atomic_store(c, 0u, __ATOMIC_RELAXED, __HIP_MEMORY_SCOPE_AGENT);
}
#endif

#if defined(__HIP_DEVICE_COMPILE__) && !defined(__gfx950__) && !defined(LFDM_EMU_BUILD)
#error "fence-free hand-off (lfdm_agent_store_u64 / lfdm_agent_load_u64 / lfdm_ticket_take) validated on gfx950 only: re-validate, or use LFDM_FENCE_RELEASE_AGENT / LFDM_FENCE_ACQUIRE_AGENT, before building for another target"
#endif
#if defined(LFDM_EMU_BUILD)
static inline void lfdm_agent_store_u64(unsigned long long* p, unsigned long long v) { __atomic_store_n(p, v, __ATOMIC_SEQ_CST); }
static inline unsigned long long lfdm_agent_load_u64(const unsigned long long* p) { return __atomic_load_n(p, __ATOMIC_SEQ_CST); }
static inline unsigned lfdm_agent_load_u32(const unsigned* p) { return __atomic_load_n(p, __ATOMIC_SEQ_CST); }
static inline void lfdm_sleep() {}
#else
__device__ __forceinline__ void lfdm_agent_store_u64(unsigned long long* p, unsigned long long v) {
  __hip_atomic_store(p, v, __ATOMIC_RELAXED, __HIP_MEMORY_SCOPE_AGENT);
}
__device__ __forceinline__ unsigned long long lfdm_agent_load_u64(const unsigned long long* p) {
  return __hip_atomic_load(p, __ATOMIC_RELAXED, __HIP_MEMORY_SCOPE_AGENT);
}
__device__ __forceinline__ unsigned lfdm_agent_load_u32(const unsigned* p) { return __hip_atomic_load(p, __ATOMIC_RELAXED, __HIP_MEMORY_SCOPE_AGENT); }
__device__ __forceinline__ void lfdm_sleep() { __builtin_amdgcn_s_sleep(2); }
#endif

#if defined(LFDM_EMU_BUILD)
static inline void lfdm_wave_lds_sync() { emu::wave_sync(); }
#else
__device__ __forceinline__ void lfdm_wave_lds_sync() {
  __builtin_amdgcn_fence(__ATOMIC_RELEASE, "wavefront");
  __builtin_amdgcn_wave_barrier();
  __builtin_amdgcn_fence(__ATOMIC_ACQUIRE, "wavefront");
}
#endif

__device__ __forceinline__ float wave_sum(float v) {
#pragma unroll
  for (int m = 32; m >= 1; m >>= 1) v += __shfl_xor(v, m);
  return v;
}
__device__ __forceinline__ float wave_max(float v) {
#pragma unroll
  for (int m = 32; m >= 1; m >>= 1) v = fmaxf(v, __shfl_xor(v, m));
  return v;
}
__device__ __forceinline__ float sigmoidf_(float x) { return 1.0f / (1.0f + expf(-x)); }
__device__ __forceinline__ float siluf_(float x) { return x / (1.0f + expf(-x)); }

#if defined(LFDM_EMU_BUILD)
static inline float silu_fast_(float x) { return x / (1.0f + expf(-x)); }
#else
__device__ __forceinline__ float silu_fast_(float x) { return x * __builtin_amdgcn_rcpf(1.0f + __expf(-x)); }
#endif

#if defined(LFDM_TUNING_KNOBS) || defined(LFDM_EMU_BUILD)
static inline const char* lfdm_knob(const char* name) { return getenv(name); }
#else
static inline const char* lfdm_knob(const char*) { return nullptr; }
#endif

__device__ __forceinline__ float apply_act(float v, int act) {
  if (act == 1) return v > 0.f ? v : 0.f;
  if (act == 2) return sigmoidf_(v);
  if (act == 3) return siluf_(v);
  return v;
}

extern "C" void lfdm_set_error(const char* msg);
int lfdm_check_launch(const char* what);
```

### cvpr23_lfdm_amd/csrc/linattn_fused.hip

```cpp
#include <stdlib.h>

#include "lfdm_device.h"
#include "../../include/lfdm_hip.h"

namespace {

constexpr int HEADS = 8;
constexpr int DH = 32;
constexpr int OUT_LD = HEADS * DH;
constexpr int C = 64;
constexpr int CH = C / 2;
constexpr int SPLIT_TOK = 32;
constexpr int PART = DH * DH + 2 * DH;
constexpr float LA_SCALE = 0.17677669529663687f;

__device__ __forceinline__ void load_xraw(const float* __restrict__ xrow, int kh, float4 (&raw)[CH / 4]) {
#pragma unroll
  for (int q = 0; q < CH / 4; ++q) raw[q] = *reinterpret_cast<const float4*>(xrow + CH * kh + 4 * q);
}
__device__ __forceinline__ void xhat_stats(const float4 (&raw)[CH / 4], float eps, float& mean, float& rstd) {
  float s1 = 0.f, s2 = 0.f;
#pragma unroll
  for (int q = 0; q < CH / 4; ++q) {
    const float4 v = raw[q];
    s1 += (v.x + v.y) + (v.z + v.w);
    s2 += (v.x * v.x + v.y * v.y) + (v.z * v.z + v.w * v.w);
  }
  s1 += __shfl_xor(s1, 32);
  s2 += __shfl_xor(s2, 32);
  mean = s1 * (1.0f / (float)C);
  float var = s2 * (1.0f / (float)C) - mean * mean;
  if (var < 0.f) var = 0.f;
  rstd = 1.0f / sqrtf(var + eps);
}
__device__ __forceinline__ void xhat_apply(const float4 (&raw)[CH / 4], bool ok, float mean, float rstd, float (&xf)[CH]) {
#pragma unroll
  for (int q = 0; q < CH / 4; ++q) {
    const float4 v = raw[q];
    xf[4 * q] = ok ? (v.x - mean) * rstd : 0.f;
    xf[4 * q + 1] = ok ? (v.y - mean) * rstd : 0.f;
    xf[4 * q + 2] = ok ? (v.z - mean) * rstd : 0.f;
    xf[4 * q + 3] = ok ? (v.w - mean) * rstd : 0.f;
  }
}
__device__ __forceinline__ void load_xhat(const float* __restrict__ xrow, bool ok, int kh, float eps, float (&xf)[CH]) {
  float4 raw[CH / 4];
  float mean, rstd;
  load_xraw(xrow, kh, raw);
  xhat_stats(raw, eps, mean, rstd);
  xhat_apply(raw, ok, mean, rstd, xf);
}

__device__ __forceinline__ void load_wfrag(const float* __restrict__ wp, int which, int head, int lane, float (&wf)[CH]) {
  const float* src = wp + ((int64_t)(which * HEADS + head) * (CH / 4) * 64 + lane) * 4;
#pragma unroll
  for (int q = 0; q < CH / 4; ++q) {
    const float4 v = *reinterpret_cast<const float4*>(src + 256 * q);
    wf[4 * q] = v.x; wf[4 * q + 1] = v.y; wf[4 * q + 2] = v.z; wf[4 * q + 3] = v.w;
  }
}

__global__ __launch_bounds__(64, 3) void linattn_fused_ctx_kernel(const float* __restrict__ x, int ldx,
                                                                  const float* __restrict__ wqkv, int hw, float eps,
                                                                  float* __restrict__ part, int split_tok) {
  const int lane = threadIdx.x & 63, l31 = lane & 31, kh = lane >> 5;
  const int f = blockIdx.x >> 3, h = blockIdx.x & 7;
  const int split = blockIdx.y, nsplit = gridDim.y;
  const int n0 = split * split_tok;
  const int n1 = (n0 + split_tok < hw) ? n0 + split_tok : hw;

  float wk[CH], wv[CH];
  load_wfrag(wqkv, 1, h, lane, wk);
  load_wfrag(wqkv, 2, h, lane, wv);

  float m_run = -3.0e38f, s_run = 0.f;
  f32x16 ctx;
#pragma unroll
  for (int r = 0; r < 16; ++r) ctx[r] = 0.f;
  for (int t0 = n0; t0 < n1; t0 += 32) {
    const int n = t0 + l31;
    float xf[CH];
    load_xhat(x + ((int64_t)f * hw + (n < n1 ? n : n1 - 1)) * ldx, n < n1, kh, eps, xf);
    f32x16 ka, va;
#pragma unroll
    for (int r = 0; r < 16; ++r) ka[r] = va[r] = 0.f;
#pragma unroll
    for (int s = 0; s < CH; ++s) {
      ka = mfma_32x32x2(xf[s], wk[s], ka);
      va = mfma_32x32x2(xf[s], wv[s], va);
    }
    float m = -3.0e38f;
#pragma unroll
    for (int r = 0; r < 16; ++r) {
      const int tok = t0 + (r & 3) + 8 * (r >> 2) + 4 * kh;
      if (tok < n1) m = fmaxf(m, ka[r]);
    }
    m = fmaxf(m, __shfl_xor(m, 32));
    const float m_new = fmaxf(m_run, m);
    const float alpha = expf(m_run - m_new);
    float ssum = 0.f;
    float e[16];
#pragma unroll
    for (int r = 0; r < 16; ++r) {
      const int tok = t0 + (r & 3) + 8 * (r >> 2) + 4 * kh;
      e[r] = tok < n1 ? expf(ka[r] - m_new) : 0.f;
      ssum += e[r];
    }
    ssum += __shfl_xor(ssum, 32);
    s_run = s_run * alpha + ssum;
    m_run = m_new;
#pragma unroll
    for (int r = 0; r < 16; ++r) ctx[r] *= __shfl(alpha, (r & 3) + 8 * (r >> 2) + 4 * kh);
#pragma unroll
    for (int r = 0; r < 16; ++r) ctx = mfma_32x32x2(e[r], va[r], ctx);
  }
  float* dst = part + ((int64_t)blockIdx.x * nsplit + split) * PART;
#pragma unroll
  for (int r = 0; r < 16; ++r) dst[((r & 3) + 8 * (r >> 2) + 4 * kh) * DH + l31] = ctx[r];
  if (kh == 0) {
    dst[DH * DH + l31] = m_run;
    dst[DH * DH + DH + l31] = s_run;
  }
}

__global__ __launch_bounds__(256) void linattn_fused_merge_kernel(const float* __restrict__ part, int nsplit,
                                                                  float* __restrict__ ctx_out) {
  constexpr int MAXS = 64;
  __shared__ float s_w[MAXS][DH];
  const int tid = threadIdx.x;
  const float* base = part + (int64_t)blockIdx.x * nsplit * PART;
  if (nsplit <= 8) {
    constexpr int PS = 8;
    float cv[4][PS], pm[PS], psum[PS];
#pragma unroll
    for (int p = 0; p < PS; ++p) {
      const int pc = p < nsplit ? p : nsplit - 1;
#pragma unroll
      for (int e = 0; e < 4; ++e) cv[e][p] = base[(int64_t)pc * PART + tid + 256 * e];
      pm[p] = base[(int64_t)pc * PART + DH * DH + (tid & (DH - 1))];
      psum[p] = base[(int64_t)pc * PART + DH * DH + DH + (tid & (DH - 1))];
    }
    if (tid < DH) {
      float mm = -3.0e38f;
#pragma unroll
      for (int p = 0; p < PS; ++p)
        if (p < nsplit) mm = fmaxf(mm, pm[p]);
      float den = 0.f, w[PS];
#pragma unroll
      for (int p = 0; p < PS; ++p) {
        w[p] = p < nsplit ? expf(pm[p] - mm) : 0.f;
        den += w[p] * psum[p];
      }
      const float inv = 1.0f / den;
#pragma unroll
      for (int p = 0; p < PS; ++p)
        if (p < nsplit) s_w[p][tid] = w[p] * inv;
    }
    __syncthreads();
#pragma unroll
    for (int e = 0; e < 4; ++e) {
      const int i = tid + 256 * e, d = i >> 5;
      float acc = 0.f;
#pragma unroll
      for (int p = 0; p < PS; ++p)
        if (p < nsplit) acc += s_w[p][d] * cv[e][p];
      ctx_out[(int64_t)blockIdx.x * DH * DH + i] = acc;
    }
    return;
  }
  if (tid < DH) {
    float mm = -3.0e38f;
#pragma unroll 4
    for (int p = 0; p < nsplit; ++p) mm = fmaxf(mm, base[(int64_t)p * PART + DH * DH + tid]);
    float den = 0.f;
#pragma unroll 4
    for (int p = 0; p < nsplit; ++p) {
      const float w = expf(base[(int64_t)p * PART + DH * DH + tid] - mm);
      s_w[p][tid] = w;
      den += w * base[(int64_t)p * PART + DH * DH + DH + tid];
    }
    const float inv = 1.0f / den;
    for (int p = 0; p < nsplit; ++p) s_w[p][tid] *= inv;
  }
  __syncthreads();
  for (int i = tid; i < DH * DH; i += 256) {
    const int d = i >> 5;
    float acc = 0.f;
#pragma unroll 4
    for (int p = 0; p < nsplit; ++p) acc += s_w[p][d] * base[(int64_t)p * PART + i];
    ctx_out[(int64_t)blockIdx.x * DH * DH + i] = acc;
  }
}

__global__ __launch_bounds__(64, 2) void linattn_fused_out_kernel(const float* __restrict__ x, int ldx,
                                                                  const float* __restrict__ wqkv,
                                                                  const float* __restrict__ ctx, int hw, float eps,
                                                                  float* __restrict__ out) {
  const int lane = threadIdx.x & 63, l31 = lane & 31, kh = lane >> 5;
  const int f = blockIdx.y;
  const int n = blockIdx.x * 32 + l31;
  float xf[CH];
  load_xhat(x + ((int64_t)f * hw + (n < hw ? n : 0)) * ldx, n < hw, kh, eps, xf);
  const int hpb = HEADS / gridDim.z;
#pragma unroll 1
  for (int h = blockIdx.z * hpb; h < (blockIdx.z + 1) * hpb; ++h) {
    float wq[CH];
    load_wfrag(wqkv, 0, h, lane, wq);
    f32x16 q;
#pragma unroll
    for (int r = 0; r < 16; ++r) q[r] = 0.f;
#pragma unroll
    for (int s = 0; s < CH; ++s) q = mfma_32x32x2(wq[s], xf[s], q);
    float m = q[0];
#pragma unroll
    for (int r = 1; r < 16; ++r) m = fmaxf(m, q[r]);
    m = fmaxf(m, __shfl_xor(m, 32));
    float sum = 0.f;
#pragma unroll
    for (int r = 0; r < 16; ++r) {
      q[r] = expf(q[r] - m);
      sum += q[r];
    }
    sum += __shfl_xor(sum, 32);
    const float inv = LA_SCALE / sum;
    const float* cb = ctx + ((int64_t)f * HEADS + h) * DH * DH + l31;
    f32x16 o;
#pragma unroll
    for (int r = 0; r < 16; ++r) o[r] = 0.f;
#pragma unroll
    for (int r = 0; r < 16; ++r) o = mfma_32x32x2(q[r] * inv, cb[((r & 3) + 8 * (r >> 2) + 4 * kh) * DH], o);
#pragma unroll
    for (int r = 0; r < 16; ++r) {
      const int tok = blockIdx.x * 32 + (r & 3) + 8 * (r >> 2) + 4 * kh;
      if (tok < hw) out[((int64_t)f * hw + tok) * OUT_LD + h * DH + l31] = o[r];
    }
  }
}


constexpr int LDY = C + 4;
__global__ __launch_bounds__(256, 2) void linattn_fused_out2_kernel(const float* __restrict__ x, int ldx, const float* __restrict__ wqkv,
                                                                    const float* __restrict__ wout, const float* __restrict__ bias_out,
                                                                    const float* __restrict__ ctx, int hw, float eps, float* __restrict__ out,
                                                                    int ldo) {
  __shared__ __attribute__((aligned(16))) float s_y[4 * 32 * LDY];
  const int tid = threadIdx.x;
  const int wave = lfdm_uniform(tid >> 6);
  const int lane = tid & 63, l31 = lane & 31, kh = lane >> 5;
  const int f = blockIdx.y;
  const int n0 = blockIdx.x * 32;
  const int n = n0 + l31;
  float xf[CH];
  load_xhat(x + ((int64_t)f * hw + (n < hw ? n : 0)) * ldx, n < hw, kh, eps, xf);
  f32x16 yT[2];
#pragma unroll
  for (int cb = 0; cb < 2; ++cb)
#pragma unroll
    for (int r = 0; r < 16; ++r) yT[cb][r] = 0.f;
#pragma unroll 1
  for (int h = 2 * wave; h < 2 * wave + 2; ++h) {
    float wq[CH];
    load_wfrag(wqkv, 0, h, lane, wq);
    f32x16 q;
#pragma unroll
    for (int r = 0; r < 16; ++r) q[r] = 0.f;
#pragma unroll
    for (int s = 0; s < CH; ++s) q = mfma_32x32x2(wq[s], xf[s], q);
    float m = q[0];
#pragma unroll
    for (int r = 1; r < 16; ++r) m = fmaxf(m, q[r]);
    m = fmaxf(m, __shfl_xor(m, 32));
    float sum = 0.f;
#pragma unroll
    for (int r = 0; r < 16; ++r) {
      q[r] = expf(q[r] - m);
      sum += q[r];
    }
    sum += __shfl_xor(sum, 32);
    const float inv = LA_SCALE / sum;
    const float* cb_ = ctx + ((int64_t)f * HEADS + h) * DH * DH + l31;
    f32x16 oT;
#pragma unroll
    for (int r = 0; r < 16; ++r) oT[r] = 0.f;
#pragma unroll
    for (int r = 0; r < 16; ++r) oT = mfma_32x32x2(cb_[((r & 3) + 8 * (r >> 2) + 4 * kh) * DH], q[r] * inv, oT);
#pragma unroll
    for (int cb = 0; cb < 2; ++cb) {
      const float* wsrc = wout + ((int64_t)((h * 2 + cb) * 4) * 64 + lane) * 4;
      float4 wo[4];
#pragma unroll
      for (int qd = 0; qd < 4; ++qd) wo[qd] = *reinterpret_cast<const float4*>(wsrc + 256 * qd);
#pragma unroll
      for (int qd = 0; qd < 4; ++qd) {
        yT[cb] = mfma_32x32x2(wo[qd].x, oT[4 * qd + 0], yT[cb]);
        yT[cb] = mfma_32x32x2(wo[qd].y, oT[4 * qd + 1], yT[cb]);
        yT[cb] = mfma_32x32x2(wo[qd].z, oT[4 * qd + 2], yT[cb]);
        yT[cb] = mfma_32x32x2(wo[qd].w, oT[4 * qd + 3], yT[cb]);
      }
    }
  }
  float* ys = s_y + (wave * 32 + l31) * LDY;
#pragma unroll
  for (int cb = 0; cb < 2; ++cb)
#pragma unroll
    for (int g = 0; g < 4; ++g)
      *reinterpret_cast<float4*>(ys + 32 * cb + 8 * g + 4 * kh) = make_float4(yT[cb][4 * g], yT[cb][4 * g + 1], yT[cb][4 * g + 2], yT[cb][4 * g + 3]);
  __syncthreads();
  const int tok = tid >> 3, c8 = (tid & 7) * 8;
  if (n0 + tok < hw) {
    const int64_t row = (int64_t)f * hw + n0 + tok;
#pragma unroll
    for (int j = 0; j < 2; ++j) {
      const int c = c8 + 4 * j;
      float4 v = *reinterpret_cast<const float4*>(x + row * ldx + c);
      const float4 b4 = bias_out ? *reinterpret_cast<const float4*>(bias_out + c) : make_float4(0.f, 0.f, 0.f, 0.f);
      v.x += b4.x; v.y += b4.y; v.z += b4.z; v.w += b4.w;
#pragma unroll
      for (int w4 = 0; w4 < 4; ++w4) {
        const float4 u = *reinterpret_cast<const float4*>(s_y + (w4 * 32 + tok) * LDY + c);
        v.x += u.x; v.y += u.y; v.z += u.z; v.w += u.w;
      }
      *reinterpret_cast<float4*>(out + row * ldo + c) = v;
    }
  }
}

}

extern "C" size_t lfdm_linear_attention_fused_ws_bytes(int n_frames, int hw) {
  const int nsplit = (hw + SPLIT_TOK - 1) / SPLIT_TOK;
  return ((size_t)n_frames * HEADS * nsplit * PART + (size_t)n_frames * HEADS * DH * DH) * sizeof(float);
}

namespace {
void launch_ctx_and_merge(const float* x, int ldx, const float* wqkv, int n_frames, int hw, float ln_eps, void* ws, float** ctx_out,
                          hipStream_t stream) {
  const int tiles = (hw + 31) / 32;
  const int64_t pairs = (int64_t)n_frames * HEADS;
  int want = (int)((pairs <= 1536 ? 3072 : 4 * 3072 + pairs - 1) / pairs);
  if (const char* e = lfdm_knob("LFDM_LINATTN_SPLITS")) want = atoi(e);
  if (want < 1) want = 1;
  if (want > 64) want = 64;
  if (want > tiles) want = tiles;
  const int split_tok = ((tiles + want - 1) / want) * 32;
  const int nsplit = (hw + split_tok - 1) / split_tok;
  float* part = (float*)ws;
  float* ctx = part + (size_t)n_frames * HEADS * ((hw + SPLIT_TOK - 1) / SPLIT_TOK) * PART;
  LFDM_LAUNCH(linattn_fused_ctx_kernel, dim3(n_frames * HEADS, nsplit), dim3(64), 0, stream, x, ldx, wqkv, hw, ln_eps, part, split_tok);
  LFDM_LAUNCH(linattn_fused_merge_kernel, dim3(n_frames * HEADS), dim3(256), 0, stream, (const float*)part, nsplit, ctx);
  *ctx_out = ctx;
}
}

extern "C" int lfdm_linear_attention_fused_cl_f32(const float* x, int ldx, int channels, const float* wqkv, float* out,
                                                  int n_frames, int hw, float ln_eps, void* ws, size_t ws_bytes,
                                                  lfdm_stream_t stream_) {
  hipStream_t stream = (hipStream_t)stream_;
  if (!x || !wqkv || !out || n_frames <= 0 || hw <= 0 || hw > 64 * 64 || channels != C || ldx < C || ldx % 4 != 0 ||
      (((uintptr_t)x | (uintptr_t)wqkv) & 15) || (int64_t)n_frames * HEADS > 0x7fffffff) {
    lfdm_set_error("linear_attention_fused: needs C == 64 and 16-byte aligned rows");
    return LFDM_EINVAL;
  }
  if (!ws || ws_bytes < lfdm_linear_attention_fused_ws_bytes(n_frames, hw)) {
    lfdm_set_error("linear_attention_fused: workspace too small");
    return LFDM_EWORKSPACE;
  }
  float* ctx = nullptr;
  launch_ctx_and_merge(x, ldx, wqkv, n_frames, hw, ln_eps, ws, &ctx, stream);
  const int64_t otiles = (int64_t)((hw + 31) / 32) * n_frames;
  const int hgroups = otiles >= 4096 ? 1 : (otiles >= 2048 ? 2 : 4);
  LFDM_LAUNCH(linattn_fused_out_kernel, dim3((hw + 31) / 32, n_frames, hgroups), dim3(64), 0, stream, x, ldx, wqkv,
              (const float*)ctx, hw, ln_eps, out);
  return lfdm_check_launch("linear_attention_fused");
}

extern "C" int lfdm_linear_attention_fused_out_cl_f32(const float* x, int ldx, int channels, const float* wqkv, const float* wout,
                                                      const float* bias_out, float* out, int ldo, int n_frames, int hw, float ln_eps,
                                                      void* ws, size_t ws_bytes, lfdm_stream_t stream_) {
  hipStream_t stream = (hipStream_t)stream_;
  if (!x || !wqkv || !wout || !out || out == x || n_frames <= 0 || hw <= 0 || hw > 64 * 64 || channels != C || ldx < C || ldx % 4 != 0 || ldo < C ||
      ldo % 4 != 0 || (((uintptr_t)x | (uintptr_t)wqkv | (uintptr_t)wout | (uintptr_t)out | (uintptr_t)bias_out) & 15) ||
      (int64_t)n_frames * HEADS > 0x7fffffff || n_frames > 65535) {
    lfdm_set_error("linear_attention_fused_out: needs C == 64, 16-byte aligned rows, out != x, <= 65535 frames");
    return LFDM_EINVAL;
  }
  if (!ws || ws_bytes < lfdm_linear_attention_fused_ws_bytes(n_frames, hw)) {
    lfdm_set_error("linear_attention_fused_out: workspace too small");
    return LFDM_EWORKSPACE;
  }
  float* ctx = nullptr;
  launch_ctx_and_merge(x, ldx, wqkv, n_frames, hw, ln_eps, ws, &ctx, stream);
  LFDM_LAUNCH(linattn_fused_out2_kernel, dim3((hw + 31) / 32, n_frames), dim3(256), 0, stream, x, ldx, wqkv, wout, bias_out, (const float*)ctx, hw,
              ln_eps, out, ldo);
  return lfdm_check_launch("linear_attention_fused_out");
}
```

### cvpr23_lfdm_amd/csrc/norm.hip

```cpp
#include <stdlib.h>
#include "lfdm_device.h"
#include "../../include/lfdm_hip.h"

namespace {

constexpr int GN_MAX_CHUNKS = 256;

__host__ __device__ inline int gn_num_chunks(int pixels) {
  int n = (pixels + 15) / 16;
  if (n < 1) n = 1;
  if (n > GN_MAX_CHUNKS) n = GN_MAX_CHUNKS;
  return n;
}

__global__ __launch_bounds__(256) void gn_partial_kernel(const float* __restrict__ x, int pixels,
                                                         int channels, int groups,
                                                         float* __restrict__ partial) {
  __shared__ float red_s[256], red_q[256];
  const int tid = threadIdx.x;
  const int c4n = channels >> 2;
  const int rows_per_iter = 256 / c4n;
  const int c4 = tid % c4n, prow = tid / c4n;
  const int nchunk = gridDim.x, chunk = blockIdx.x, b = blockIdx.y;
  const int per = (pixels + nchunk - 1) / nchunk;
  const int p0 = chunk * per;
  const int p1 = (p0 + per < pixels) ? p0 + per : pixels;
  const float* xb = x + (int64_t)b * pixels * channels;
  float s = 0.f, q = 0.f;
  if (prow < rows_per_iter) {
    for (int p = p0 + prow; p < p1; p += rows_per_iter) {
      const float4 v = *reinterpret_cast<const float4*>(xb + (int64_t)p * channels + 4 * c4);
      s += (v.x + v.y) + (v.z + v.w);
      q += (v.x * v.x + v.y * v.y) + (v.z * v.z + v.w * v.w);
    }
  }
  red_s[tid] = s;
  red_q[tid] = q;
  __syncthreads();
  if (tid < groups) {
    const int cg4 = c4n / groups;
    float ts = 0.f, tq = 0.f;
    for (int r = 0; r < rows_per_iter; ++r)
      for (int k = 0; k < cg4; ++k) {
        const int t = r * c4n + tid * cg4 + k;
        ts += red_s[t];
        tq += red_q[t];
      }
    float* dst = partial + (((int64_t)b * nchunk + chunk) * groups + tid) * 2;
    dst[0] = ts;
    dst[1] = tq;
  }
}

constexpr int GN_MAX_C = 1024;
template <int NT>
__global__ __launch_bounds__(NT) void gn_apply_kernel(
    const float* __restrict__ x, float* __restrict__ out, int pixels, int channels, int groups,
    const float* __restrict__ partial, int nchunk, const float* __restrict__ gamma,
    const float* __restrict__ beta, const float* __restrict__ scale_shift, int ss_ld, float eps, int silu,
    const float* __restrict__ residual, int xcd_r) {
  __shared__ float s_mean[64], s_rstd[64];
  __shared__ __attribute__((aligned(16))) float s_a[GN_MAX_C], s_b[GN_MAX_C];
  const int b = blockIdx.y, tid = threadIdx.x;
  unsigned jb = blockIdx.x;
  if (xcd_r > 0) {
    const unsigned r8 = 8u * (unsigned)xcd_r, q = jb / r8, rem = jb - q * r8;
    jb = q * r8 + (rem & 7u) * (unsigned)xcd_r + (rem >> 3);
  }
  const int c4n = channels >> 2;
  const int64_t per_b = (int64_t)pixels * c4n;
  const float4* xb = reinterpret_cast<const float4*>(x) + (int64_t)b * per_b;
  float4* ob = reinterpret_cast<float4*>(out) + (int64_t)b * per_b;
  const float4* rb = residual ? reinterpret_cast<const float4*>(residual) + (int64_t)b * per_b : nullptr;
  const int64_t stride = (int64_t)gridDim.x * NT;
  const int64_t i0 = (int64_t)jb * NT + tid;
  float4 pre_v[2], pre_r[2];
#pragma unroll
  for (int k = 0; k < 2; ++k) {
    const int64_t i = i0 + k * stride;
    pre_v[k] = make_float4(0.f, 0.f, 0.f, 0.f);
    pre_r[k] = make_float4(0.f, 0.f, 0.f, 0.f);
    if (i < per_b) {
      pre_v[k] = xb[i];
      if (rb) pre_r[k] = rb[i];
    }
  }
  constexpr int PREC = 2;
  float p_g[PREC], p_b[PREC], p_sc[PREC], p_sh[PREC];
#pragma unroll
  for (int j = 0; j < PREC; ++j) {
    const int c = tid + j * NT, cc = c < channels ? c : 0;
    p_g[j] = gamma[cc];
    p_b[j] = beta[cc];
    p_sc[j] = scale_shift ? scale_shift[(int64_t)b * ss_ld + cc] : 0.f;
    p_sh[j] = scale_shift ? scale_shift[(int64_t)b * ss_ld + channels + cc] : 0.f;
  }
  const int lpg = (NT >= 64 * groups) ? 64 : 32;
  const int gpp = NT / lpg;
  const int sub = tid & (lpg - 1);
  for (int g0 = 0; g0 < groups; g0 += gpp) {
    const int g = g0 + tid / lpg;
    double s = 0.0, q = 0.0;
    if (g < groups) {
      const float2* src = reinterpret_cast<const float2*>(partial) + ((int64_t)b * nchunk) * groups + g;
      int k = sub;
      for (; k + 3 * lpg < nchunk; k += 4 * lpg) {
        const float2 v0 = src[(int64_t)k * groups], v1 = src[(int64_t)(k + lpg) * groups];
        const float2 v2 = src[(int64_t)(k + 2 * lpg) * groups], v3 = src[(int64_t)(k + 3 * lpg) * groups];
        s += (double)v0.x; q += (double)v0.y;
        s += (double)v1.x; q += (double)v1.y;
        s += (double)v2.x; q += (double)v2.y;
        s += (double)v3.x; q += (double)v3.y;
      }
      for (; k < nchunk; k += lpg) {
        const float2 v = src[(int64_t)k * groups];
        s += (double)v.x;
        q += (double)v.y;
      }
    }
    for (int m = lpg >> 1; m >= 1; m >>= 1) {
      s += __shfl_xor(s, m);
      q += __shfl_xor(q, m);
    }
    if (g < groups && sub == 0) {
      const double n = (double)pixels * (double)(channels / groups);
      const double mean = s / n;
      double var = q / n - mean * mean;
      if (var < 0.0) var = 0.0;
      s_mean[g] = (float)mean;
      s_rstd[g] = (float)(1.0 / sqrt(var + (double)eps));
    }
  }
  __syncthreads();
  const int cg = channels / groups;
  {
    int j = 0;
    for (int c = tid; c < channels; c += NT, ++j) {
      const int g = c / cg;
      const bool pre = j < PREC;
      const float a = s_rstd[g] * (pre ? (j == 0 ? p_g[0] : p_g[1]) : gamma[c]);
      float bb = (pre ? (j == 0 ? p_b[0] : p_b[1]) : beta[c]) - s_mean[g] * a;
      float aa = a;
      if (scale_shift) {
        const float sc = (pre ? (j == 0 ? p_sc[0] : p_sc[1]) : scale_shift[(int64_t)b * ss_ld + c]) + 1.0f;
        const float sh = pre ? (j == 0 ? p_sh[0] : p_sh[1]) : scale_shift[(int64_t)b * ss_ld + channels + c];
        aa = a * sc;
        bb = bb * sc + sh;
      }
      s_a[c] = aa;
      s_b[c] = bb;
    }
  }
  __syncthreads();
  int k = 0;
  for (int64_t i = i0; i < per_b; i += stride, ++k) {
    const int c4 = (int)(i % c4n);
    const float4 v = k == 0 ? pre_v[0] : k == 1 ? pre_v[1] : xb[i];
    const float4 a = *reinterpret_cast<const float4*>(s_a + 4 * c4);
    const float4 d = *reinterpret_cast<const float4*>(s_b + 4 * c4);
    float4 y;
    y.x = fmaf(v.x, a.x, d.x);
    y.y = fmaf(v.y, a.y, d.y);
    y.z = fmaf(v.z, a.z, d.z);
    y.w = fmaf(v.w, a.w, d.w);
    if (silu) {
      y.x = siluf_(y.x);
      y.y = siluf_(y.y);
      y.z = siluf_(y.z);
      y.w = siluf_(y.w);
    }
    if (rb) {
      const float4 r = k == 0 ? pre_r[0] : k == 1 ? pre_r[1] : rb[i];
      y.x += r.x;
      y.y += r.y;
      y.z += r.z;
      y.w += r.w;
    }
    ob[i] = y;
  }
}

template <int C4N>
__global__ __launch_bounds__(256) void layernorm_small_kernel(const float* __restrict__ x, float* __restrict__ out, int64_t rows,
                                                              const float* __restrict__ gamma, float eps) {
  constexpr int RPW = 64 / C4N, C = 4 * C4N;
  const int lane = threadIdx.x & 63, wave = threadIdx.x >> 6;
  const int sub = lane / C4N, f = lane % C4N;
  const float4 g = reinterpret_cast<const float4*>(gamma)[f];
  auto group_sum = [&](float v) {
#pragma unroll
    for (int m = 1; m < C4N; m <<= 1) v += __shfl_xor(v, m);
    return v;
  };
  const int64_t stride = (int64_t)gridDim.x * 4 * RPW * 2;
  for (int64_t row0 = ((int64_t)blockIdx.x * 4 + wave) * RPW * 2; row0 < rows; row0 += stride) {
    float4 v[2];
    bool live[2];
#pragma unroll
    for (int u = 0; u < 2; ++u) {
      const int64_t row = row0 + u * RPW + sub;
      live[u] = row < rows;
      v[u] = live[u] ? reinterpret_cast<const float4*>(x + row * C)[f] : make_float4(0.f, 0.f, 0.f, 0.f);
    }
#pragma unroll
    for (int u = 0; u < 2; ++u) {
      const float mean = group_sum((v[u].x + v[u].y) + (v[u].z + v[u].w)) / (float)C;
      const float a = v[u].x - mean, b = v[u].y - mean, c = v[u].z - mean, d = v[u].w - mean;
      const float var = group_sum((a * a + b * b) + (c * c + d * d)) / (float)C;
      const float denom = sqrtf(var + eps);
      if (live[u]) {
        float4 y;
        y.x = a / denom * g.x;
        y.y = b / denom * g.y;
        y.z = c / denom * g.z;
        y.w = d / denom * g.w;
        reinterpret_cast<float4*>(out + (row0 + u * RPW + sub) * C)[f] = y;
      }
    }
  }
}

__global__ __launch_bounds__(256) void layernorm_kernel(const float* __restrict__ x,
                                                        float* __restrict__ out, int64_t rows,
                                                        int channels, const float* __restrict__ gamma,
                                                        float eps) {
  const int lane = threadIdx.x & 63, wave = threadIdx.x >> 6;
  const int c4n = channels >> 2;
  for (int64_t row = (int64_t)blockIdx.x * 4 + wave; row < rows; row += (int64_t)gridDim.x * 4) {
    const float4* xr = reinterpret_cast<const float4*>(x + row * channels);
    float4 v[4];
    float s = 0.f;
#pragma unroll
    for (int i = 0; i < 4; ++i) {
      const int f = lane + 64 * i;
      v[i] = make_float4(0.f, 0.f, 0.f, 0.f);
      if (f < c4n) {
        v[i] = xr[f];
        s += (v[i].x + v[i].y) + (v[i].z + v[i].w);
      }
    }
    const float mean = wave_sum(s) / (float)channels;
    float q = 0.f;
#pragma unroll
    for (int i = 0; i < 4; ++i) {
      const int f = lane + 64 * i;
      if (f < c4n) {
        const float a = v[i].x - mean, b = v[i].y - mean, c = v[i].z - mean, d = v[i].w - mean;
        q += (a * a + b * b) + (c * c + d * d);
      }
    }
    const float var = wave_sum(q) / (float)channels;
    const float denom = sqrtf(var + eps);
    float4* orow = reinterpret_cast<float4*>(out + row * channels);
#pragma unroll
    for (int i = 0; i < 4; ++i) {
      const int f = lane + 64 * i;
      if (f < c4n) {
        const float4 g = reinterpret_cast<const float4*>(gamma)[f];
        float4 y;
        y.x = (v[i].x - mean) / denom * g.x;
        y.y = (v[i].y - mean) / denom * g.y;
        y.z = (v[i].z - mean) / denom * g.z;
        y.w = (v[i].w - mean) / denom * g.w;
        orow[f] = y;
      }
    }
  }
}

__global__ __launch_bounds__(256) void affine_act_kernel(const float* __restrict__ x,
                                                         float* __restrict__ out, int64_t rows,
                                                         int channels, int ldx, int ldo,
                                                         const float* __restrict__ a,
                                                         const float* __restrict__ b, int act) {
  const int c4n = channels >> 2;
  const int64_t total = rows * c4n;
  for (int64_t i = (int64_t)blockIdx.x * 256 + threadIdx.x; i < total; i += (int64_t)gridDim.x * 256) {
    const int64_t r = i / c4n;
    const int c = (int)(i - r * c4n) * 4;
    const float4 v = *reinterpret_cast<const float4*>(x + r * ldx + c);
    const float4 aa = *reinterpret_cast<const float4*>(a + c);
    const float4 bb = *reinterpret_cast<const float4*>(b + c);
    float4 y;
    y.x = apply_act(fmaf(v.x, aa.x, bb.x), act);
    y.y = apply_act(fmaf(v.y, aa.y, bb.y), act);
    y.z = apply_act(fmaf(v.z, aa.z, bb.z), act);
    y.w = apply_act(fmaf(v.w, aa.w, bb.w), act);
    *reinterpret_cast<float4*>(out + r * ldo + c) = y;
  }
}

__global__ __launch_bounds__(256) void avgpool2_kernel(const float* __restrict__ x,
                                                       float* __restrict__ out, int n_img, int h,
                                                       int w, int channels) {
  const int c4n = channels >> 2;
  const int ho = h >> 1, wo = w >> 1;
  const int64_t total = (int64_t)n_img * ho * wo * c4n;
  for (int64_t i = (int64_t)blockIdx.x * 256 + threadIdx.x; i < total; i += (int64_t)gridDim.x * 256) {
    const int c = (int)(i % c4n) * 4;
    int64_t pix = i / c4n;
    const int ox = (int)(pix % wo);
    pix /= wo;
    const int oy = (int)(pix % ho);
    const int n = (int)(pix / ho);
    const float* base = x + (((int64_t)n * h + 2 * oy) * w + 2 * ox) * channels + c;
    const float4 v00 = *reinterpret_cast<const float4*>(base);
    const float4 v01 = *reinterpret_cast<const float4*>(base + channels);
    const float4 v10 = *reinterpret_cast<const float4*>(base + (int64_t)w * channels);
    const float4 v11 = *reinterpret_cast<const float4*>(base + (int64_t)w * channels + channels);
    float4 y;
    y.x = ((v00.x + v01.x) + (v10.x + v11.x)) * 0.25f;
    y.y = ((v00.y + v01.y) + (v10.y + v11.y)) * 0.25f;
    y.z = ((v00.z + v01.z) + (v10.z + v11.z)) * 0.25f;
    y.w = ((v00.w + v01.w) + (v10.w + v11.w)) * 0.25f;
    *reinterpret_cast<float4*>(out + (((int64_t)n * ho + oy) * wo + ox) * channels + c) = y;
  }
}

__global__ __launch_bounds__(256) void planar_to_cl_kernel(const float* __restrict__ x,
                                                           float* __restrict__ out, int channels,
                                                           int hw, int ldo) {
  __shared__ float tile[32][33];
  const int n = blockIdx.z, p0 = blockIdx.x * 32, c0 = blockIdx.y * 32;
  const int tx = threadIdx.x & 31, ty = threadIdx.x >> 5;
  for (int i = ty; i < 32; i += 8) {
    const int c = c0 + i, p = p0 + tx;
    tile[i][tx] = (c < channels && p < hw) ? x[((int64_t)n * channels + c) * hw + p] : 0.f;
  }
  __syncthreads();
  for (int i = ty; i < 32; i += 8) {
    const int p = p0 + i, c = c0 + tx;
    if (p < hw && c < channels) out[((int64_t)n * hw + p) * ldo + c] = tile[tx][i];
  }
}

__global__ __launch_bounds__(256) void cl_to_planar_kernel(const float* __restrict__ x,
                                                           float* __restrict__ out, int channels,
                                                           int hw, int ldx) {
  __shared__ float tile[32][33];
  const int n = blockIdx.z, p0 = blockIdx.x * 32, c0 = blockIdx.y * 32;
  const int tx = threadIdx.x & 31, ty = threadIdx.x >> 5;
  for (int i = ty; i < 32; i += 8) {
    const int p = p0 + i, c = c0 + tx;
    tile[i][tx] = (p < hw && c < channels) ? x[((int64_t)n * hw + p) * ldx + c] : 0.f;
  }
  __syncthreads();
  for (int i = ty; i < 32; i += 8) {
    const int c = c0 + i, p = p0 + tx;
    if (c < channels && p < hw) out[((int64_t)n * channels + c) * hw + p] = tile[tx][i];
  }
}

inline unsigned grid_for(int64_t work_items, unsigned cap = 8192) {
  int64_t nb = (work_items + 255) / 256;
  if (nb < 1) nb = 1;
  if (nb > cap) nb = cap;
  return (unsigned)nb;
}

void launch_gn_apply(const float* x, float* out, int batch, int pixels, int channels, int groups,
                     const float* partial, int nchunk, const float* gamma, const float* beta,
                     const float* scale_shift, int ss_ld, float eps, int silu, const float* residual,
                     hipStream_t stream) {
  const int64_t per_b = (int64_t)pixels * (channels / 4);
  static const int env_f4 = [] { const char* e = lfdm_knob("LFDM_GN_F4"); return e ? atoi(e) : 0; }();
  static const int env_nt = [] { const char* e = lfdm_knob("LFDM_GN_BLOCK"); return e ? atoi(e) : 0; }();
  int f4 = 2, nt = 256;
  if ((int64_t)nchunk * groups >= 4096) {
    nt = per_b >= (1 << 20) ? 1024 : 512;
    f4 = per_b >= (1 << 20) ? 8 : 2;
  }
  if (env_f4 > 0) f4 = env_f4;
  if (env_nt == 256 || env_nt == 512 || env_nt == 1024) nt = env_nt;
  int64_t nb = (per_b + (int64_t)nt * f4 - 1) / ((int64_t)nt * f4);
  if (nb < 1) nb = 1;
  if (nb > 8192) nb = 8192;
  const dim3 grid((unsigned)nb, batch);
  int xcd_r = 0;
  {
    const char* e = lfdm_knob("LFDM_GN_XCD");
    const int64_t blk_f4 = 128ll * (channels / 4);
    if (!(e && e[0] == '0') && blk_f4 % nt == 0) {
      const int64_t r = blk_f4 / nt;
      if (r >= 1 && r <= 64 && (r & (r - 1)) == 0 && nb % (8 * r) == 0 && (per_b % ((int64_t)nt)) == 0) xcd_r = (int)r;
    }
  }
  if (nt == 1024)
    LFDM_LAUNCH(gn_apply_kernel<1024>, grid, dim3(1024), 0, stream, x, out, pixels, channels, groups, partial, nchunk, gamma, beta,
                scale_shift, ss_ld, eps, silu, residual, xcd_r);
  else if (nt == 512)
    LFDM_LAUNCH(gn_apply_kernel<512>, grid, dim3(512), 0, stream, x, out, pixels, channels, groups, partial, nchunk, gamma, beta,
                scale_shift, ss_ld, eps, silu, residual, xcd_r);
  else
    LFDM_LAUNCH(gn_apply_kernel<256>, grid, dim3(256), 0, stream, x, out, pixels, channels, groups, partial, nchunk, gamma, beta,
                scale_shift, ss_ld, eps, silu, residual, xcd_r);
}



}

extern "C" size_t lfdm_groupnorm_ws_bytes(int batch, int pixels, int channels) {
  const size_t partial = (size_t)batch * gn_num_chunks(pixels) * 64 * 2;
  const size_t ab = (size_t)batch * 2 * channels;
  return (partial + ab) * sizeof(float);
}

extern "C" int lfdm_groupnorm_silu_cl_f32(const float* x, float* out, int batch, int pixels,
                                          int channels, int groups, const float* gamma,
                                          const float* beta, const float* scale_shift, int ss_ld,
                                          const float* residual, float eps, int apply_silu, void* ws,
                                          size_t ws_bytes, lfdm_stream_t stream_) {
  hipStream_t stream = (hipStream_t)stream_;
  if (!x || !out || !gamma || !beta || batch <= 0 || pixels <= 0 || channels <= 0 || groups <= 0 ||
      groups > 64 || (scale_shift && ss_ld < 2 * channels) || channels % groups != 0 || (channels / groups) % 4 != 0 ||
      256 % (channels / 4) != 0) {
    lfdm_set_error("groupnorm: unsupported shape (need C%G==0, (C/G)%4==0, 256%(C/4)==0)");
    return LFDM_EINVAL;
  }
  if (!ws || ws_bytes < lfdm_groupnorm_ws_bytes(batch, pixels, channels)) {
    lfdm_set_error("groupnorm: workspace too small");
    return LFDM_EWORKSPACE;
  }
  const int nchunk = gn_num_chunks(pixels);
  float* partial = reinterpret_cast<float*>(ws);
  LFDM_LAUNCH(gn_partial_kernel, dim3(nchunk, batch), dim3(256), 0, stream, x, pixels, channels,
              groups, partial);
  launch_gn_apply(x, out, batch, pixels, channels, groups, (const float*)partial, nchunk, gamma, beta,
                  scale_shift, ss_ld, eps, apply_silu, residual, stream);
  return lfdm_check_launch("groupnorm");
}

extern "C" int lfdm_groupnorm_apply_cl_f32(const float* x, float* out, int batch, int pixels,
                                           int channels, int groups, const float* gamma,
                                           const float* beta, const float* scale_shift, int ss_ld,
                                           const float* residual, float eps, int apply_silu,
                                           const float* partial, int nchunk, void* ws,
                                           size_t ws_bytes, lfdm_stream_t stream_) {
  hipStream_t stream = (hipStream_t)stream_;
  if (!x || !out || !gamma || !beta || !partial || nchunk <= 0 || batch <= 0 || pixels <= 0 ||
      channels <= 0 || channels > GN_MAX_C || groups <= 0 || groups > 64 || channels % groups != 0 ||
      channels % 4 != 0 || (scale_shift && ss_ld < 2 * channels)) {
    lfdm_set_error("groupnorm_apply: bad arguments");
    return LFDM_EINVAL;
  }
  (void)ws;
  (void)ws_bytes;
  launch_gn_apply(x, out, batch, pixels, channels, groups, partial, nchunk, gamma, beta, scale_shift,
                  ss_ld, eps, apply_silu, residual, stream);
  return lfdm_check_launch("groupnorm_apply");
}

extern "C" int lfdm_layernorm_cl_f32(const float* x, float* out, int64_t rows, int channels,
                                     const float* gamma, float eps, lfdm_stream_t stream_) {
  hipStream_t stream = (hipStream_t)stream_;
  if (!x || !out || !gamma || rows <= 0 || channels <= 0 || channels % 4 != 0 || channels > 1024) {
    lfdm_set_error("layernorm: unsupported shape (C%4==0, C<=1024)");
    return LFDM_EINVAL;
  }
  int64_t nb = (rows + 3) / 4;
  if (nb > 16384) nb = 16384;
  const bool al16 = ((((uintptr_t)x) | ((uintptr_t)out) | ((uintptr_t)gamma)) & 15) == 0;
  if ((channels == 64 || channels == 128) && al16 && rows >= 4096) {
    int64_t nbs = (rows + 4 * (256 / channels) * 2 * 4 - 1) / (4 * (256 / channels) * 2 * 4);
    if (nbs > 8192) nbs = 8192;
    if (nbs < 1) nbs = 1;
    if (channels == 64) LFDM_LAUNCH((layernorm_small_kernel<16>), dim3((unsigned)nbs), dim3(256), 0, stream, x, out, rows, gamma, eps);
    else LFDM_LAUNCH((layernorm_small_kernel<32>), dim3((unsigned)nbs), dim3(256), 0, stream, x, out, rows, gamma, eps);
    return lfdm_check_launch("layernorm");
  }
  LFDM_LAUNCH(layernorm_kernel, dim3((unsigned)nb), dim3(256), 0, stream, x, out, rows, channels,
              gamma, eps);
  return lfdm_check_launch("layernorm");
}

extern "C" int lfdm_affine_act_cl_f32(const float* x, float* out, int64_t rows, int channels,
                                      int ldx, int ldo, const float* a, const float* b, int act,
                                      lfdm_stream_t stream_) {
  hipStream_t stream = (hipStream_t)stream_;
  if (!x || !out || !a || !b || rows <= 0 || channels % 4 != 0 || ldx % 4 != 0 || ldo % 4 != 0) {
    lfdm_set_error("affine_act: unsupported shape");
    return LFDM_EINVAL;
  }
  LFDM_LAUNCH(affine_act_kernel, dim3(grid_for(rows * (channels / 4))), dim3(256), 0, stream, x, out,
              rows, channels, ldx, ldo, a, b, act);
  return lfdm_check_launch("affine_act");
}

extern "C" int lfdm_avgpool2_cl_f32(const float* x, float* out, int n_img, int h, int w,
                                    int channels, lfdm_stream_t stream_) {
  hipStream_t stream = (hipStream_t)stream_;
  if (!x || !out || n_img <= 0 || (h & 1) || (w & 1) || channels % 4 != 0) {
    lfdm_set_error("avgpool2: unsupported shape");
    return LFDM_EINVAL;
  }
  const int64_t total = (int64_t)n_img * (h / 2) * (w / 2) * (channels / 4);
  LFDM_LAUNCH(avgpool2_kernel, dim3(grid_for(total)), dim3(256), 0, stream, x, out, n_img, h, w,
              channels);
  return lfdm_check_launch("avgpool2");
}

extern "C" int lfdm_planar_to_cl_f32(const float* x, float* out, int n_img, int channels, int hw,
                                     int ldo, lfdm_stream_t stream_) {
  hipStream_t stream = (hipStream_t)stream_;
  if (!x || !out || n_img <= 0 || channels <= 0 || hw <= 0 || ldo < channels) {
    lfdm_set_error("planar_to_cl: bad arguments");
    return LFDM_EINVAL;
  }
  LFDM_LAUNCH(planar_to_cl_kernel, dim3((hw + 31) / 32, (channels + 31) / 32, n_img), dim3(256), 0,
              stream, x, out, channels, hw, ldo);
  return lfdm_check_launch("planar_to_cl");
}

extern "C" int lfdm_cl_to_planar_f32(const float* x, float* out, int n_img, int channels, int hw,
                                     int ldx, lfdm_stream_t stream_) {
  hipStream_t stream = (hipStream_t)stream_;
  if (!x || !out || n_img <= 0 || channels <= 0 || hw <= 0 || ldx < channels) {
    lfdm_set_error("cl_to_planar: bad arguments");
    return LFDM_EINVAL;
  }
  LFDM_LAUNCH(cl_to_planar_kernel, dim3((hw + 31) / 32, (channels + 31) / 32, n_img), dim3(256), 0,
              stream, x, out, channels, hw, ldx);
  return lfdm_check_launch("cl_to_planar");
}
```

### cvpr23_lfdm_amd/csrc/small.hip

```cpp
#include <stdlib.h>
#include "lfdm_device.h"
#include "../../include/lfdm_hip.h"

namespace {

__device__ __forceinline__ float geluf_(float x) { return 0.5f * x * (1.0f + erff(x * 0.70710678118654752f)); }

__device__ __forceinline__ float small_act(float v, int act) {
  if (act == LFDM_ACT_GELU) return geluf_(v);
  return apply_act(v, act);
}

__global__ __launch_bounds__(256) void linear_small_kernel(const float* __restrict__ x,
                                                           const float* __restrict__ w,
                                                           const float* __restrict__ bias,
                                                           float* __restrict__ y, int k, int n,
                                                           int ldx, int ldw, int ldy, int act_in,
                                                           int act_out) {
  const int lane = threadIdx.x & 63, wave = threadIdx.x >> 6;
  const int col = blockIdx.x * 4 + wave;
  const int b = blockIdx.y;
  if (col >= n) return;
  const float* xr = x + (int64_t)b * ldx;
  const float* wr = w + (int64_t)col * ldw;
  float s = 0.f;
  for (int i = lane; i < k; i += 64) s = fmaf(small_act(xr[i], act_in), wr[i], s);
  s = wave_sum(s);
  if (lane == 0) {
    if (bias) s += bias[col];
    y[(int64_t)b * ldy + col] = small_act(s, act_out);
  }
}

__global__ __launch_bounds__(64) void sinusoidal_kernel(const int32_t* __restrict__ t_dev,
                                                        int t_stride, const float* __restrict__ freqs,
                                                        float* __restrict__ out, int dim, int ldo) {
  const int b = blockIdx.x;
  const int half = dim / 2;
  const float tt = (float)t_dev[(int64_t)b * t_stride];
  for (int i = threadIdx.x; i < half; i += 64) {
    const float a = tt * freqs[i];
    out[(int64_t)b * ldo + i] = sinf(a);
    out[(int64_t)b * ldo + half + i] = cosf(a);
  }
}

constexpr int CPI_MAX_K = 7 * 7 * 4;
constexpr int CPI_PIX = 128;
__global__ __launch_bounds__(256) void conv_planar_in_kernel(
    const float* __restrict__ x, int batch, int cin, int cin_total, int frames, int h, int w,
    const float* __restrict__ wgt, int kh, int kw, int cout, const float* __restrict__ bias,
    const float* __restrict__ add_term, float* __restrict__ out, int ldo, int act) {
  __shared__ __attribute__((aligned(16))) float ws[CPI_MAX_K * 64];
  const int tid = threadIdx.x;
  const int K = kh * kw * cin;
  const int co0 = blockIdx.y * 64;
  if ((cout & 3) == 0 && ((((uintptr_t)wgt) & 15) == 0)) {
    for (int i = tid; i < K * 16; i += 256) {
      const int kk = i >> 4, j4 = i & 15;
      *reinterpret_cast<float4*>(ws + kk * 64 + 4 * j4) = *reinterpret_cast<const float4*>(wgt + (int64_t)kk * cout + co0 + 4 * j4);
    }
  } else {
    for (int i = tid; i < K * 64; i += 256) {
      const int kk = i >> 6, j = i & 63;
      ws[i] = wgt[(int64_t)kk * cout + co0 + j];
    }
  }
  __syncthreads();
  const int hw = h * w;
  const int64_t total = (int64_t)batch * frames * hw;
  const int64_t gp = (int64_t)blockIdx.x * CPI_PIX + (tid & (CPI_PIX - 1));
  if (gp >= total) return;
  const int cg = tid >> 7;
  const int64_t bt = gp / hw;
  const int pix = (int)(gp - bt * hw);
  const int b = (int)(bt / frames), t = (int)(bt - (int64_t)b * frames);
  const int oy = pix / w, ox = pix - oy * w;
  const int py = kh / 2, px = kw / 2;
  float acc[32];
#pragma unroll
  for (int j = 0; j < 32; ++j) acc[j] = 0.f;
  for (int ky = 0; ky < kh; ++ky) {
    const int iy = oy + ky - py;
    if (iy < 0 || iy >= h) continue;
    for (int kx = 0; kx < kw; ++kx) {
      const int ix = ox + kx - px;
      if (ix < 0 || ix >= w) continue;
      for (int c = 0; c < cin; ++c) {
        const float v = x[(((int64_t)b * cin_total + c) * frames + t) * hw + iy * w + ix];
        const float4* wp = reinterpret_cast<const float4*>(ws + ((ky * kw + kx) * cin + c) * 64 + cg * 32);
#pragma unroll
        for (int j4 = 0; j4 < 8; ++j4) {
          const float4 ww = wp[j4];
          acc[4 * j4 + 0] = fmaf(v, ww.x, acc[4 * j4 + 0]);
          acc[4 * j4 + 1] = fmaf(v, ww.y, acc[4 * j4 + 1]);
          acc[4 * j4 + 2] = fmaf(v, ww.z, acc[4 * j4 + 2]);
          acc[4 * j4 + 3] = fmaf(v, ww.w, acc[4 * j4 + 3]);
        }
      }
    }
  }
  const int cbase = co0 + cg * 32;
  float* orow = out + gp * ldo + cbase;
  const float* arow = add_term ? add_term + ((int64_t)b * hw + pix) * cout + cbase : nullptr;
  const bool vec = (ldo & 3) == 0 && (cout & 3) == 0 && ((((uintptr_t)out) & 15) == 0) && (!arow || (((uintptr_t)add_term) & 15) == 0) &&
                   (!bias || (((uintptr_t)bias) & 15) == 0);
  if (vec) {
#pragma unroll
    for (int j4 = 0; j4 < 8; ++j4) {
      float4 v = make_float4(acc[4 * j4], acc[4 * j4 + 1], acc[4 * j4 + 2], acc[4 * j4 + 3]);
      if (bias) {
        const float4 bb = *reinterpret_cast<const float4*>(bias + cbase + 4 * j4);
        v.x += bb.x; v.y += bb.y; v.z += bb.z; v.w += bb.w;
      }
      if (arow) {
        const float4 aa = *reinterpret_cast<const float4*>(arow + 4 * j4);
        v.x += aa.x; v.y += aa.y; v.z += aa.z; v.w += aa.w;
      }
      v.x = apply_act(v.x, act); v.y = apply_act(v.y, act); v.z = apply_act(v.z, act); v.w = apply_act(v.w, act);
      *reinterpret_cast<float4*>(orow + 4 * j4) = v;
    }
  } else {
#pragma unroll
    for (int j = 0; j < 32; ++j) {
      float v = acc[j];
      if (bias) v += bias[cbase + j];
      if (arow) v += arow[j];
      orow[j] = apply_act(v, act);
    }
  }
}

template <bool EXTRA>
__global__ __launch_bounds__(256) void heads_kernel(const float* __restrict__ y_flow,
                                                    const float* __restrict__ y_occ, int channels, int ld,
                                                    const float* __restrict__ w_flow,
                                                    const float* __restrict__ b_flow,
                                                    const float* __restrict__ w_occ,
                                                    const float* __restrict__ b_occ,
                                                    float* __restrict__ out, int batch, int frames,
                                                    int hw, const float* __restrict__ x0, int ld0, int c0,
                                                    const float* __restrict__ x1, int ld1, int c1,
                                                    const float* __restrict__ w_extra) {
  __shared__ __attribute__((aligned(16))) float wl[3 * 256];
  __shared__ __attribute__((aligned(16))) float we[EXTRA ? 3 * 512 : 4];
  const int tid = threadIdx.x;
  for (int i = tid; i < 2 * channels; i += 256) wl[i] = w_flow[i];
  for (int i = tid; i < channels; i += 256) wl[2 * channels + i] = w_occ[i];
  if (EXTRA)
    for (int i = tid; i < 3 * (c0 + c1); i += 256) we[i] = w_extra[i];
  __syncthreads();
  const int64_t total = (int64_t)batch * frames * hw;
  const int64_t row = (int64_t)blockIdx.x * 256 + tid;
  if (row >= total) return;
  const float4* fr = reinterpret_cast<const float4*>(y_flow + row * ld);
  const float4* orr = reinterpret_cast<const float4*>(y_occ + row * ld);
  float s0 = 0.f, s1 = 0.f, s2 = 0.f;
  for (int i = 0; i < channels / 4; ++i) {
    const float4 a = fr[i];
    const float4 o = orr[i];
    const float4 w0 = reinterpret_cast<const float4*>(wl)[i];
    const float4 w1 = reinterpret_cast<const float4*>(wl + channels)[i];
    const float4 w2 = reinterpret_cast<const float4*>(wl + 2 * channels)[i];
    s0 += (a.x * w0.x + a.y * w0.y) + (a.z * w0.z + a.w * w0.w);
    s1 += (a.x * w1.x + a.y * w1.y) + (a.z * w1.z + a.w * w1.w);
    s2 += (o.x * w2.x + o.y * w2.y) + (o.z * w2.z + o.w * w2.w);
  }
  if (EXTRA) {
    const int ce = c0 + c1;
    for (int src = 0; src < 2; ++src) {
      const int cs = src == 0 ? c0 : c1, base = src == 0 ? 0 : c0;
      const float4* xr = reinterpret_cast<const float4*>(src == 0 ? x0 + row * ld0 : x1 + row * ld1);
      for (int i = 0; i < cs / 4; ++i) {
        const float4 a = xr[i];
        const float4 w0 = *reinterpret_cast<const float4*>(we + base + 4 * i);
        const float4 w1 = *reinterpret_cast<const float4*>(we + ce + base + 4 * i);
        const float4 w2 = *reinterpret_cast<const float4*>(we + 2 * ce + base + 4 * i);
        s0 += (a.x * w0.x + a.y * w0.y) + (a.z * w0.z + a.w * w0.w);
        s1 += (a.x * w1.x + a.y * w1.y) + (a.z * w1.z + a.w * w1.w);
        s2 += (a.x * w2.x + a.y * w2.y) + (a.z * w2.z + a.w * w2.w);
      }
    }
  }
  const int64_t bt = row / hw;
  const int pix = (int)(row - bt * hw);
  const int b = (int)(bt / frames), t = (int)(bt - (int64_t)b * frames);
  const int64_t fhw = (int64_t)frames * hw;
  float* ob = out + (int64_t)b * 3 * fhw + (int64_t)t * hw + pix;
  ob[0] = s0 + b_flow[0];
  ob[fhw] = s1 + b_flow[1];
  ob[2 * fhw] = s2 + b_occ[0];
}

__global__ __launch_bounds__(256) void heads_gn_kernel(const float* __restrict__ y, int ld, int channels,
                                                       const float* __restrict__ partial, int nchunk, int groups,
                                                       const float* __restrict__ gamma, const float* __restrict__ beta, float eps,
                                                       const float* __restrict__ w_flow, const float* __restrict__ b_flow,
                                                       const float* __restrict__ w_occ, const float* __restrict__ b_occ,
                                                       const float* __restrict__ x0, int ld0, int c0, const float* __restrict__ x1, int ld1, int c1,
                                                       const float* __restrict__ w_extra, float* __restrict__ out, int frames, int hw, int rows_per_wg) {
  __shared__ float s_mean[64], s_rstd[64];
  __shared__ __attribute__((aligned(16))) float s_a[512], s_b[512];
  __shared__ __attribute__((aligned(16))) float wl[3 * 512];
  __shared__ __attribute__((aligned(16))) float we[3 * 512];
  const int tid = threadIdx.x, b = blockIdx.y;
  const int c2 = 2 * channels;
  const int pixels = frames * hw;
  const int ce = c0 + c1;
  const bool pi_ok = tid < c2;
  const float pw_f0 = (pi_ok && tid < channels) ? w_flow[tid] : 0.f, pw_f1 = (pi_ok && tid < channels) ? w_flow[channels + tid] : 0.f;
  const float pw_oc = (pi_ok && tid >= channels) ? w_occ[tid - channels] : 0.f;
  const float pe0 = tid < 3 * ce ? w_extra[tid] : 0.f, pe1 = tid + 256 < 3 * ce ? w_extra[tid + 256] : 0.f;
  const float pre_gamma = gamma[pi_ok ? tid : 0], pre_beta = beta[pi_ok ? tid : 0];
  {
    const int lpg = 32, gpp = 256 / lpg, sub = tid & (lpg - 1);
    for (int g0 = 0; g0 < groups; g0 += gpp) {
      const int g = g0 + tid / lpg;
      double sm = 0.0, sq = 0.0;
      if (g < groups) {
        const float2* src = reinterpret_cast<const float2*>(partial) + ((int64_t)b * nchunk) * groups + g;
        int k = sub;
        for (; k + 3 * lpg < nchunk; k += 4 * lpg) {
          const float2 v0 = src[(int64_t)k * groups], v1 = src[(int64_t)(k + lpg) * groups];
          const float2 v2 = src[(int64_t)(k + 2 * lpg) * groups], v3 = src[(int64_t)(k + 3 * lpg) * groups];
          sm += (double)v0.x; sq += (double)v0.y;
          sm += (double)v1.x; sq += (double)v1.y;
          sm += (double)v2.x; sq += (double)v2.y;
          sm += (double)v3.x; sq += (double)v3.y;
        }
        for (; k < nchunk; k += lpg) {
          const float2 v = src[(int64_t)k * groups];
          sm += (double)v.x;
          sq += (double)v.y;
        }
      }
      for (int m = lpg >> 1; m >= 1; m >>= 1) {
        sm += __shfl_xor(sm, m);
        sq += __shfl_xor(sq, m);
      }
      if (g < groups && sub == 0) {
        const double n = (double)pixels * (double)(c2 / groups);
        const double mean = sm / n;
        double var = sq / n - mean * mean;
        if (var < 0.0) var = 0.0;
        s_mean[g] = (float)mean;
        s_rstd[g] = (float)(1.0 / sqrt(var + (double)eps));
      }
    }
  }
  for (int i = tid; i < c2; i += 256) {
    const bool pre = i == tid;
    wl[i] = pre ? pw_f0 : (i < channels ? w_flow[i] : 0.f);
    wl[512 + i] = pre ? pw_f1 : (i < channels ? w_flow[channels + i] : 0.f);
    wl[1024 + i] = pre ? pw_oc : (i < channels ? 0.f : w_occ[i - channels]);
  }
  for (int i = tid; i < 3 * ce; i += 256) we[(i / ce) * 512 + (i % ce)] = i == tid ? pe0 : (i == tid + 256 ? pe1 : w_extra[i]);
  __syncthreads();
  const int cg = c2 / groups;
  for (int c = tid; c < c2; c += 256) {
    const int g = c / cg;
    const float a = s_rstd[g] * (c == tid ? pre_gamma : gamma[c]);
    s_a[c] = a;
    s_b[c] = (c == tid ? pre_beta : beta[c]) - s_mean[g] * a;
  }
  __syncthreads();
  const int r8 = tid >> 3, seg = tid & 7;
  const float bf0 = b_flow[0], bf1 = b_flow[1], bo = b_occ[0];
  const int64_t fhw = (int64_t)frames * hw;
  auto finish = [&](int pix, float s0, float s1, float s2) {
#pragma unroll
    for (int m = 1; m <= 4; m <<= 1) {
      s0 += __shfl_xor(s0, m);
      s1 += __shfl_xor(s1, m);
      s2 += __shfl_xor(s2, m);
    }
    if (seg == 0) {
      const int t = pix / hw, px = pix - t * hw;
      float* ob = out + (int64_t)b * 3 * fhw + (int64_t)t * hw + px;
      ob[0] = s0 + bf0;
      ob[fhw] = s1 + bf1;
      ob[2 * fhw] = s2 + bo;
    }
  };
  if (c2 == 128 && c0 == 64 && c1 == 64) {
    float4 ra[4], rb[4], w0[4], w1[4], w2[4], e0[4], e1[4], e2[4];
#pragma unroll
    for (int j = 0; j < 4; ++j) {
      const int k = seg + 8 * j;
      ra[j] = *reinterpret_cast<const float4*>(s_a + 4 * k);
      rb[j] = *reinterpret_cast<const float4*>(s_b + 4 * k);
      w0[j] = *reinterpret_cast<const float4*>(wl + 4 * k);
      w1[j] = *reinterpret_cast<const float4*>(wl + 512 + 4 * k);
      w2[j] = *reinterpret_cast<const float4*>(wl + 1024 + 4 * k);
      const int ke = (j < 2 ? 0 : 64) + 4 * (seg + 8 * (j & 1));
      e0[j] = *reinterpret_cast<const float4*>(we + ke);
      e1[j] = *reinterpret_cast<const float4*>(we + 512 + ke);
      e2[j] = *reinterpret_cast<const float4*>(we + 1024 + ke);
    }
    for (int p0 = 0; p0 < rows_per_wg; p0 += 32) {
      const int pix = blockIdx.x * rows_per_wg + p0 + r8;
      if (pix >= pixels) break;
      const int64_t row = (int64_t)b * pixels + pix;
      const float4* yr = reinterpret_cast<const float4*>(y + row * ld);
      const float4* x0r = reinterpret_cast<const float4*>(x0 + row * ld0);
      const float4* x1r = reinterpret_cast<const float4*>(x1 + row * ld1);
      float4 v[4], xv[4];
#pragma unroll
      for (int j = 0; j < 4; ++j) v[j] = yr[seg + 8 * j];
      xv[0] = x0r[seg]; xv[1] = x0r[seg + 8]; xv[2] = x1r[seg]; xv[3] = x1r[seg + 8];
      float s0 = 0.f, s1 = 0.f, s2 = 0.f;
#pragma unroll
      for (int j = 0; j < 4; ++j) {
        const float t0 = siluf_(fmaf(v[j].x, ra[j].x, rb[j].x)), t1 = siluf_(fmaf(v[j].y, ra[j].y, rb[j].y));
        const float t2 = siluf_(fmaf(v[j].z, ra[j].z, rb[j].z)), t3 = siluf_(fmaf(v[j].w, ra[j].w, rb[j].w));
        s0 += (t0 * w0[j].x + t1 * w0[j].y) + (t2 * w0[j].z + t3 * w0[j].w);
        s1 += (t0 * w1[j].x + t1 * w1[j].y) + (t2 * w1[j].z + t3 * w1[j].w);
        s2 += (t0 * w2[j].x + t1 * w2[j].y) + (t2 * w2[j].z + t3 * w2[j].w);
      }
#pragma unroll
      for (int j = 0; j < 4; ++j) {
        s0 += (xv[j].x * e0[j].x + xv[j].y * e0[j].y) + (xv[j].z * e0[j].z + xv[j].w * e0[j].w);
        s1 += (xv[j].x * e1[j].x + xv[j].y * e1[j].y) + (xv[j].z * e1[j].z + xv[j].w * e1[j].w);
        s2 += (xv[j].x * e2[j].x + xv[j].y * e2[j].y) + (xv[j].z * e2[j].z + xv[j].w * e2[j].w);
      }
      finish(pix, s0, s1, s2);
    }
    return;
  }
  for (int p0 = 0; p0 < rows_per_wg; p0 += 32) {
    const int pix = blockIdx.x * rows_per_wg + p0 + r8;
    if (pix >= pixels) break;
    const int64_t row = (int64_t)b * pixels + pix;
    float s0 = 0.f, s1 = 0.f, s2 = 0.f;
    const float4* yr = reinterpret_cast<const float4*>(y + row * ld);
    for (int k = seg; k < c2 / 4; k += 8) {
      const float4 v = yr[k];
      const float4 a = *reinterpret_cast<const float4*>(s_a + 4 * k), d = *reinterpret_cast<const float4*>(s_b + 4 * k);
      const float4 w0 = *reinterpret_cast<const float4*>(wl + 4 * k), w1 = *reinterpret_cast<const float4*>(wl + 512 + 4 * k);
      const float4 w2 = *reinterpret_cast<const float4*>(wl + 1024 + 4 * k);
      const float t0 = siluf_(fmaf(v.x, a.x, d.x)), t1 = siluf_(fmaf(v.y, a.y, d.y)), t2 = siluf_(fmaf(v.z, a.z, d.z)), t3 = siluf_(fmaf(v.w, a.w, d.w));
      s0 += (t0 * w0.x + t1 * w0.y) + (t2 * w0.z + t3 * w0.w);
      s1 += (t0 * w1.x + t1 * w1.y) + (t2 * w1.z + t3 * w1.w);
      s2 += (t0 * w2.x + t1 * w2.y) + (t2 * w2.z + t3 * w2.w);
    }
#pragma unroll
    for (int src = 0; src < 2; ++src) {
      const int cs = src == 0 ? c0 : c1, base = src == 0 ? 0 : c0;
      if (cs == 0) continue;
      const float4* xr = reinterpret_cast<const float4*>(src == 0 ? x0 + row * ld0 : x1 + row * ld1);
      for (int k = seg; k < cs / 4; k += 8) {
        const float4 v = xr[k];
        const float4 w0 = *reinterpret_cast<const float4*>(we + base + 4 * k), w1 = *reinterpret_cast<const float4*>(we + 512 + base + 4 * k);
        const float4 w2 = *reinterpret_cast<const float4*>(we + 1024 + base + 4 * k);
        s0 += (v.x * w0.x + v.y * w0.y) + (v.z * w0.z + v.w * w0.w);
        s1 += (v.x * w1.x + v.y * w1.y) + (v.z * w1.z + v.w * w1.w);
        s2 += (v.x * w2.x + v.y * w2.y) + (v.z * w2.z + v.w * w2.w);
      }
    }
    finish(pix, s0, s1, s2);
  }
}

__global__ __launch_bounds__(256) void step_cond_kernel(const float* __restrict__ step_table,
                                                        const float* __restrict__ batch_base,
                                                        const int32_t* __restrict__ step_dev,
                                                        float* __restrict__ out, int batch, int n) {
  const float* row = step_table + (int64_t)(*step_dev) * n;
  const int64_t total = (int64_t)batch * n;
  for (int64_t i = (int64_t)blockIdx.x * 256 + threadIdx.x; i < total; i += (int64_t)gridDim.x * 256) {
    const int c = (int)(i % n);
    out[i] = row[c] + batch_base[i];
  }
}

__global__ __launch_bounds__(256) void pack_conv_weight_kernel(const float* __restrict__ w, int n_o, int n_i, int taps,
                                                               int64_t stride_o, int64_t stride_i, int mode, int K, int N,
                                                               int np, float* __restrict__ out) {
  const int64_t per = (int64_t)((K + 31) / 32) * np * 32;
  const int64_t idx = (int64_t)blockIdx.x * 256 + threadIdx.x;
  if (idx >= per * (mode == 2 ? 4 : 1)) return;
  const int q = (int)(idx / per);
  const int64_t r = idx - q * per;
  const int kk = (int)(r & 31);
  const int n = (int)((r >> 5) % np);
  const int k = (int)((r >> 5) / np) * 32 + kk;
  float v = 0.f;
  if (k < K && n < N) {
    if (mode == 0) {
      const int tap = k / n_i, i = k - tap * n_i;
      v = w[n * stride_o + i * stride_i + tap];
    } else if (mode == 1) {
      const int tap = k / n_o, o = k - tap * n_o;
      v = w[o * stride_o + n * stride_i + (taps - 1 - tap)];
    } else {
      const int t = k / n_o, ci = k - t * n_o;
      const int ky = (3 - (q >> 1)) - 2 * (t >> 1), kx = (3 - (q & 1)) - 2 * (t & 1);
      v = w[ci * stride_o + n * stride_i + ky * 4 + kx];
    }
  }
  out[idx] = v;
}

}

extern "C" int lfdm_step_cond_f32(const float* step_table, const float* batch_base,
                                  const int32_t* step_dev, float* out, int batch, int n,
                                  lfdm_stream_t stream_) {
  hipStream_t stream = (hipStream_t)stream_;
  if (!step_table || !batch_base || !step_dev || !out || batch <= 0 || n <= 0) {
    lfdm_set_error("step_cond: bad arguments");
    return LFDM_EINVAL;
  }
  int64_t nb = ((int64_t)batch * n + 255) / 256;
  if (nb > 1024) nb = 1024;
  LFDM_LAUNCH(step_cond_kernel, dim3((unsigned)nb), dim3(256), 0, stream, step_table, batch_base,
              step_dev, out, batch, n);
  return lfdm_check_launch("step_cond");
}

extern "C" int lfdm_linear_small_f32(const float* x, const float* w, const float* bias, float* y,
                                     int batch, int k, int n, int ldx, int ldw, int ldy,
                                     int act_in, int act_out, lfdm_stream_t stream_) {
  hipStream_t stream = (hipStream_t)stream_;
  if (!x || !w || !y || batch <= 0 || k <= 0 || n <= 0 || ldx < k || ldw < k || ldy < n) {
    lfdm_set_error("linear_small: bad arguments");
    return LFDM_EINVAL;
  }
  LFDM_LAUNCH(linear_small_kernel, dim3((n + 3) / 4, batch), dim3(256), 0, stream, x, w, bias, y, k,
              n, ldx, ldw, ldy, act_in, act_out);
  return lfdm_check_launch("linear_small");
}

extern "C" int lfdm_sinusoidal_f32(const int32_t* t_dev, int t_stride, const float* freqs,
                                   float* out, int batch, int dim, int ldo, lfdm_stream_t stream_) {
  hipStream_t stream = (hipStream_t)stream_;
  if (!t_dev || !freqs || !out || batch <= 0 || dim < 4 || (dim & 1) || ldo < dim) {
    lfdm_set_error("sinusoidal: bad arguments");
    return LFDM_EINVAL;
  }
  LFDM_LAUNCH(sinusoidal_kernel, dim3(batch), dim3(64), 0, stream, t_dev, t_stride, freqs, out, dim, ldo);
  return lfdm_check_launch("sinusoidal");
}

constexpr int CPM_ROWS = 4, CPM_COLS = 32;
__global__ __launch_bounds__(256) void conv_planar_in_mfma_kernel(
    const float* __restrict__ x, int batch, int cin, int cin_total, int frames, int h, int w,
    const float* __restrict__ wgt, int kh, int kw, int cout, const float* __restrict__ bias,
    const float* __restrict__ add_term, float* __restrict__ out, int ldo, int act, int tiles_x, int tiles_y) {
  __shared__ __attribute__((aligned(16))) float ws[(CPI_MAX_K + 1) * 64];
  __shared__ float win[8 * (CPM_ROWS + 6) * (CPM_COLS + 6)];
  const int tid = threadIdx.x, lane = tid & 63, wave = tid >> 6, l31 = lane & 31, khalf = lane >> 5;
  const int K = kh * kw * cin;
  const int Kp = (K + 1) & ~1;
  const int co0 = blockIdx.y * 64;
  const int tile = blockIdx.x % (tiles_x * tiles_y);
  const int bt = blockIdx.x / (tiles_x * tiles_y);
  const int b = bt / frames, t = bt - b * frames;
  const int oy0 = (tile / tiles_x) * CPM_ROWS, ox0 = (tile % tiles_x) * CPM_COLS;
  const int py = kh / 2, px = kw / 2;
  const int wr = CPM_ROWS + kh - 1, wc = CPM_COLS + kw - 1;
  constexpr int WMAX = ((CPI_MAX_K + 1) * 16 + 255) / 256;
  constexpr int XMAX = (8 * (CPM_ROWS + 6) * (CPM_COLS + 6) + 255) / 256;
  float4 wv[WMAX];
  float xv[XMAX];
#pragma unroll
  for (int j = 0; j < WMAX; ++j) {
    const int i = tid + 256 * j, kk = i >> 4, j4 = i & 15;
    wv[j] = make_float4(0.f, 0.f, 0.f, 0.f);
    if (kk < K) wv[j] = *reinterpret_cast<const float4*>(wgt + (int64_t)kk * cout + co0 + 4 * j4);
  }
  const int hw = h * w;
  const int nwin = cin * wr * wc;
#pragma unroll
  for (int j = 0; j < XMAX; ++j) {
    const int i = tid + 256 * j;
    const int c = i / (wr * wc), rem = i - c * (wr * wc);
    const int ry = rem / wc, rx = rem - ry * wc;
    const int iy = oy0 + ry - py, ix = ox0 + rx - px;
    xv[j] = 0.f;
    if (i < nwin && iy >= 0 && iy < h && ix >= 0 && ix < w) xv[j] = x[(((int64_t)b * cin_total + c) * frames + t) * hw + iy * w + ix];
  }
#pragma unroll
  for (int j = 0; j < WMAX; ++j) {
    const int i = tid + 256 * j;
    if (i < Kp * 16) *reinterpret_cast<float4*>(ws + (i >> 4) * 64 + 4 * (i & 15)) = wv[j];
  }
#pragma unroll
  for (int j = 0; j < XMAX; ++j) {
    const int i = tid + 256 * j;
    if (i < nwin) win[i] = xv[j];
  }
  __syncthreads();
  f32x16 acc[2];
#pragma unroll
  for (int nt = 0; nt < 2; ++nt)
#pragma unroll
    for (int r = 0; r < 16; ++r) acc[nt][r] = 0.f;
  const int half_k = Kp >> 1;
  if (kh == 7 && kw == 7 && cin == 3) {
    constexpr int KH = 7, KW = 7, CIN = 3, WR = CPM_ROWS + KH - 1, WC = CPM_COLS + KW - 1, HALF = (KH * KW * CIN + 1) / 2;
    const float* wbase = win + wave * WC + l31;
    const float* bbase = ws + (khalf * HALF) * 64 + l31;
#pragma unroll
    for (int st = 0; st < HALF; ++st) {
      const int k0 = st, k1 = HALF + st;
      const int ky0 = k0 / (KW * CIN), kx0 = (k0 - ky0 * KW * CIN) / CIN, c0 = k0 - (ky0 * KW + kx0) * CIN;
      const int ky1r = k1 / (KW * CIN), kx1 = (k1 - ky1r * KW * CIN) / CIN, c1 = k1 - (ky1r * KW + kx1) * CIN;
      const int ky1 = ky1r < KH ? ky1r : KH - 1;
      const int o0 = (c0 * WR + ky0) * WC + kx0, o1 = (c1 * WR + ky1) * WC + kx1;
      const float a = wbase[khalf ? o1 : o0];
      const float b0 = bbase[st * 64], b1 = bbase[st * 64 + 32];
      acc[0] = mfma_32x32x2(a, b0, acc[0]);
      acc[1] = mfma_32x32x2(a, b1, acc[1]);
    }
  } else {
  int k = khalf * half_k;
  int ky = k / (kw * cin), kx = (k - ky * kw * cin) / cin, c = k - (ky * kw + kx) * cin;
  for (int st = 0; st < half_k; ++st, ++k) {
    const int kyc = ky < kh ? ky : kh - 1;
    const float a = win[(c * wr + wave + kyc) * wc + l31 + kx];
    const float b0 = ws[k * 64 + l31], b1 = ws[k * 64 + 32 + l31];
    acc[0] = mfma_32x32x2(a, b0, acc[0]);
    acc[1] = mfma_32x32x2(a, b1, acc[1]);
    const bool cw_ = c + 1 == cin;
    c = cw_ ? 0 : c + 1;
    const bool kw_ = cw_ && kx + 1 == kw;
    kx = kw_ ? 0 : (cw_ ? kx + 1 : kx);
    ky = kw_ ? ky + 1 : ky;
  }
  }
  const int oy = oy0 + wave;
  if (oy >= h) return;
  float addv[2][16];
#pragma unroll
  for (int nt = 0; nt < 2; ++nt)
#pragma unroll
    for (int r = 0; r < 16; ++r) {
      const int ox = ox0 + (r & 3) + 8 * (r >> 2) + 4 * khalf;
      const int oxc = ox < w ? ox : w - 1;
      addv[nt][r] = add_term ? add_term[((int64_t)b * hw + oy * w + oxc) * cout + co0 + 32 * nt + l31] : 0.f;
    }
#pragma unroll
  for (int nt = 0; nt < 2; ++nt) {
    const int ch = co0 + 32 * nt + l31;
    const float bv = bias ? bias[ch] : 0.f;
#pragma unroll
    for (int r = 0; r < 16; ++r) {
      const int ox = ox0 + (r & 3) + 8 * (r >> 2) + 4 * khalf;
      if (ox >= w) continue;
      const float v = acc[nt][r] + bv + addv[nt][r];
      out[(((int64_t)b * frames + t) * hw + oy * w + ox) * ldo + ch] = apply_act(v, act);
    }
  }
}

extern "C" int lfdm_conv_planar_in_cl_f32(const float* x, int batch, int cin, int cin_total,
                                          int frames, int h, int w, const float* wgt, int kh,
                                          int kw, int cout, const float* bias,
                                          const float* add_term, float* out, int ldo, int act,
                                          lfdm_stream_t stream_) {
  hipStream_t stream = (hipStream_t)stream_;
  if (!x || !wgt || !out || batch <= 0 || cin <= 0 || cin > cin_total || frames <= 0 || h <= 0 ||
      w <= 0 || kh <= 0 || kw <= 0 || !(kh & 1) || !(kw & 1) || cout <= 0 || cout % 64 != 0 ||
      kh * kw * cin > CPI_MAX_K || ldo < cout) {
    lfdm_set_error("conv_planar_in: unsupported shape (odd kernel, kh*kw*cin<=196, cout%64==0)");
    return LFDM_EINVAL;
  }
  const int64_t total = (int64_t)batch * frames * h * w;
  static const bool mfma_off = [] { const char* e = lfdm_knob("LFDM_STEM_MFMA"); return e && e[0] == '0'; }();
  const int tiles_x = (w + CPM_COLS - 1) / CPM_COLS, tiles_y = (h + CPM_ROWS - 1) / CPM_ROWS;
  const int64_t nblk = (int64_t)batch * frames * tiles_x * tiles_y;
  if (!mfma_off && cin <= 8 && kh <= 7 && kw <= 7 && (cout & 3) == 0 && ((((uintptr_t)wgt) & 15) == 0) && nblk < (1ll << 31)) {
    LFDM_LAUNCH(conv_planar_in_mfma_kernel, dim3((unsigned)nblk, cout / 64), dim3(256), 0, stream, x, batch, cin, cin_total, frames, h,
                w, wgt, kh, kw, cout, bias, add_term, out, ldo, act, tiles_x, tiles_y);
    return lfdm_check_launch("conv_planar_in_mfma");
  }
  const dim3 grid((unsigned)((total + CPI_PIX - 1) / CPI_PIX), cout / 64);
  LFDM_LAUNCH(conv_planar_in_kernel, grid, dim3(256), 0, stream, x, batch, cin, cin_total, frames, h, w, wgt, kh, kw, cout, bias,
              add_term, out, ldo, act);
  return lfdm_check_launch("conv_planar_in");
}

extern "C" int lfdm_heads_cl_to_planar_f32(const float* y_flow, const float* y_occ, int channels, int ld,
                                           const float* w_flow, const float* b_flow,
                                           const float* w_occ, const float* b_occ, float* out,
                                           int batch, int frames, int hw, lfdm_stream_t stream_) {
  hipStream_t stream = (hipStream_t)stream_;
  if (!y_flow || !y_occ || !w_flow || !b_flow || !w_occ || !b_occ || !out || channels <= 0 ||
      channels > 256 || channels % 4 != 0 || ld < channels || ld % 4 != 0 || batch <= 0 || frames <= 0 || hw <= 0) {
    lfdm_set_error("heads: bad arguments");
    return LFDM_EINVAL;
  }
  const int64_t total = (int64_t)batch * frames * hw;
  LFDM_LAUNCH(heads_kernel<false>, dim3((unsigned)((total + 255) / 256)), dim3(256), 0, stream, y_flow,
              y_occ, channels, ld, w_flow, b_flow, w_occ, b_occ, out, batch, frames, hw, (const float*)nullptr, 0, 0, (const float*)nullptr, 0, 0,
              (const float*)nullptr);
  return lfdm_check_launch("heads");
}

extern "C" int lfdm_heads_res_cl_to_planar_f32(const float* y_flow, const float* y_occ, int channels, int ld, const float* w_flow,
                                               const float* b_flow, const float* w_occ, const float* b_occ, const float* x0, int ld0, int c0,
                                               const float* x1, int ld1, int c1, const float* w_extra, float* out, int batch, int frames,
                                               int hw, lfdm_stream_t stream_) {
  hipStream_t stream = (hipStream_t)stream_;
  if (!y_flow || !y_occ || !w_flow || !b_flow || !w_occ || !b_occ || !out || !x0 || !w_extra || channels <= 0 || channels > 256 ||
      channels % 4 != 0 || ld < channels || ld % 4 != 0 || batch <= 0 || frames <= 0 || hw <= 0 || c0 <= 0 || c0 % 4 != 0 || ld0 < c0 ||
      ld0 % 4 != 0 || c1 < 0 || c1 % 4 != 0 || (c1 > 0 && (!x1 || ld1 < c1 || ld1 % 4 != 0)) || c0 + c1 > 512 ||
      (((uintptr_t)y_flow | (uintptr_t)y_occ | (uintptr_t)x0 | (uintptr_t)x1) & 15) != 0) {
    lfdm_set_error("heads_res: bad arguments (C % 4 == 0, c0 + c1 <= 512, 16-byte aligned rows)");
    return LFDM_EINVAL;
  }
  const int64_t total = (int64_t)batch * frames * hw;
  LFDM_LAUNCH(heads_kernel<true>, dim3((unsigned)((total + 255) / 256)), dim3(256), 0, stream, y_flow, y_occ, channels, ld, w_flow, b_flow,
              w_occ, b_occ, out, batch, frames, hw, x0, ld0, c0, x1 ? x1 : x0, ld1, c1, w_extra);
  return lfdm_check_launch("heads_res");
}

extern "C" int lfdm_heads_gn_res_cl_to_planar_f32(const float* y, int ld, int channels, const float* partial, int nchunk, int groups,
                                                  const float* gamma, const float* beta, float eps, const float* w_flow, const float* b_flow,
                                                  const float* w_occ, const float* b_occ, const float* x0, int ld0, int c0, const float* x1, int ld1,
                                                  int c1, const float* w_extra, float* out, int batch, int frames, int hw, lfdm_stream_t stream_) {
  hipStream_t stream = (hipStream_t)stream_;
  const int c2 = 2 * channels;
  if (!y || !partial || !gamma || !beta || !w_flow || !b_flow || !w_occ || !b_occ || !out || !x0 || !w_extra || channels <= 0 || c2 > 512 ||
      channels % 4 != 0 || ld < c2 || ld % 4 != 0 || batch <= 0 || batch > 65535 || frames <= 0 || hw <= 0 || nchunk <= 0 || groups <= 0 || groups > 64 ||
      c2 % groups != 0 || c0 <= 0 || c0 % 4 != 0 || ld0 < c0 || ld0 % 4 != 0 || c1 < 0 || c1 % 4 != 0 ||
      (c1 > 0 && (!x1 || ld1 < c1 || ld1 % 4 != 0)) || c0 + c1 > 512 || (((uintptr_t)y | (uintptr_t)x0 | (uintptr_t)x1) & 15) != 0) {
    lfdm_set_error("heads_gn_res: bad arguments (2C <= 512 and % groups == 0, C % 4 == 0, c0 + c1 <= 512, 16-byte aligned rows, <= 65535 samples)");
    return LFDM_EINVAL;
  }
  const int64_t pixels = (int64_t)frames * hw;
  const int rows_per_wg = pixels >= 32768 ? 128 : 32;
  LFDM_LAUNCH(heads_gn_kernel, dim3((unsigned)((pixels + rows_per_wg - 1) / rows_per_wg), (unsigned)batch), dim3(256), 0, stream, y, ld, channels, partial,
              nchunk, groups, gamma, beta, eps, w_flow, b_flow, w_occ, b_occ, x0, ld0, c0, x1 ? x1 : x0, ld1, c1, w_extra, out, frames, hw, rows_per_wg);
  return lfdm_check_launch("heads_gn_res");
}

extern "C" int lfdm_pack_conv_weight_f32(const float* w, int n_o, int n_i, int taps, int64_t stride_o, int64_t stride_i,
                                         int mode, float* out, lfdm_stream_t stream_) {
  hipStream_t stream = (hipStream_t)stream_;
  if (!w || !out || n_o <= 0 || n_i <= 0 || taps <= 0 || mode < 0 || mode > 2 || (mode == 2 && taps != 16) ||
      stride_o <= 0 || stride_i <= 0) {
    lfdm_set_error("pack_conv_weight: bad arguments (mode 0 conv, 1 data gradient, 2 ConvTranspose k4 s2 p1 parity packs)");
    return LFDM_EINVAL;
  }
  const int K = mode == 0 ? taps * n_i : mode == 1 ? taps * n_o : 4 * n_o;
  const int N = mode == 0 ? n_o : n_i;
  const int np = (N + 31) / 32 * 32;
  const int64_t total = (int64_t)((K + 31) / 32) * np * 32 * (mode == 2 ? 4 : 1);
  LFDM_LAUNCH(pack_conv_weight_kernel, dim3((unsigned)((total + 255) / 256)), dim3(256), 0, stream, w, n_o, n_i, taps,
              stride_o, stride_i, mode, K, N, np, out);
  return lfdm_check_launch("pack_conv_weight");
}
```

Before: 4.020 videos/s.

## Fold output projection into linear-attention context and use fast exp/rcp intrinsics

The linear-attention merge kernel gains a templated mode that multiplies the merged per-head context by the output-projection weights. The out2 kernel can then apply softmaxed queries directly to this folded matrix instead of doing two chained MFMA stages per head. Separately, expf and division in the attention, linear-attention, norm and conv softmax and SiLU paths become __expf, hardware reciprocal and silu_fast_. The fast variants lower transcendental and divide cost, but accuracy drops slightly and the workspace grows to hold the larger folded matrix.

After: 4.128 videos/s, median of 6. +2.7%, better.

```diff
diff --git a/cvpr23_lfdm_amd/csrc/attention.hip b/cvpr23_lfdm_amd/csrc/attention.hip
--- a/cvpr23_lfdm_amd/csrc/attention.hip
+++ b/cvpr23_lfdm_amd/csrc/attention.hip
@@ -128,16 +128,17 @@
     for (int tj = 0; tj < NT; ++tj)
 #pragma unroll
       for (int r = 0; r < 4; ++r) {
-        const float e = (tj * 16 + lq * 4 + r) < L ? expf(st[ti][tj][r] - m) : 0.f;
+        const float e = (tj * 16 + lq * 4 + r) < L ? fast_exp(st[ti][tj][r] - m) : 0.f;
         st[ti][tj][r] = e;
         sum += e;
       }
     sum += __shfl_xor(sum, 16);
     sum += __shfl_xor(sum, 32);
+    const float inv = fast_rcp(sum);
 #pragma unroll
     for (int tj = 0; tj < NT; ++tj)
 #pragma unroll
-      for (int r = 0; r < 4; ++r) st[ti][tj][r] = st[ti][tj][r] / sum;
+      for (int r = 0; r < 4; ++r) st[ti][tj][r] = st[ti][tj][r] * inv;
   }
 
 #pragma unroll
@@ -226,10 +227,10 @@
     for (int u = 0; u < 2; ++u) {
       const int nl = ln + 32 * u;
       const bool ok = n0 + nl < hw;
-      ek[nl][4 * lc4 + 0] = ok ? expf(rk[u].x - kmax[4 * lc4 + 0]) : 0.f;
-      ek[nl][4 * lc4 + 1] = ok ? expf(rk[u].y - kmax[4 * lc4 + 1]) : 0.f;
-      ek[nl][4 * lc4 + 2] = ok ? expf(rk[u].z - kmax[4 * lc4 + 2]) : 0.f;
-      ek[nl][4 * lc4 + 3] = ok ? expf(rk[u].w - kmax[4 * lc4 + 3]) : 0.f;
+      ek[nl][4 * lc4 + 0] = ok ? fast_exp(rk[u].x - kmax[4 * lc4 + 0]) : 0.f;
+      ek[nl][4 * lc4 + 1] = ok ? fast_exp(rk[u].y - kmax[4 * lc4 + 1]) : 0.f;
+      ek[nl][4 * lc4 + 2] = ok ? fast_exp(rk[u].z - kmax[4 * lc4 + 2]) : 0.f;
+      ek[nl][4 * lc4 + 3] = ok ? fast_exp(rk[u].w - kmax[4 * lc4 + 3]) : 0.f;
       *reinterpret_cast<float4*>(&vv[nl][4 * lc4]) = rv[u];
     }
     __syncthreads();
@@ -247,10 +248,11 @@
     __syncthreads();
   }
   float* dst = ctx_out + ((int64_t)blockIdx.x * DH + d) * DH + e0;
-  dst[0] = acc[0] / ssum;
-  dst[1] = acc[1] / ssum;
-  dst[2] = acc[2] / ssum;
-  dst[3] = acc[3] / ssum;
+  const float inv = fast_rcp(ssum);
+  dst[0] = acc[0] * inv;
+  dst[1] = acc[1] * inv;
+  dst[2] = acc[2] * inv;
+  dst[3] = acc[3] * inv;
 }
 
 __global__ __launch_bounds__(256) void linattn_output_kernel(const float* __restrict__ qkv,
@@ -281,12 +283,12 @@
   float sum = 0.f;
 #pragma unroll
   for (int i = 0; i < DH; ++i) {
-    q[i] = expf(q[i] - m);
+    q[i] = fast_exp(q[i] - m);
     sum += q[i];
   }
-  const float scale = 0.17677669529663687f;
-#pragma unroll
-  for (int i = 0; i < DH; ++i) q[i] = q[i] / sum * scale;
+  const float scale = 0.17677669529663687f * fast_rcp(sum);
+#pragma unroll
+  for (int i = 0; i < DH; ++i) q[i] = q[i] * scale;
   float* op = out + row * OUT_LD + h * DH;
   const float* ch = cs + h * CS;
 #pragma unroll
diff --git a/cvpr23_lfdm_amd/csrc/attention_fused.hip b/cvpr23_lfdm_amd/csrc/attention_fused.hip
--- a/cvpr23_lfdm_amd/csrc/attention_fused.hip
+++ b/cvpr23_lfdm_amd/csrc/attention_fused.hip
@@ -8,12 +8,6 @@
 constexpr int HEADS = 8;
 constexpr int DH = 32;
 constexpr int OUT_LD = HEADS * DH;
-
-#if defined(LFDM_EMU_BUILD)
-static inline float fast_exp(float x) { return expf(x); }
-#else
-__device__ __forceinline__ float fast_exp(float x) { return __expf(x); }
-#endif
 
 template <int NT>
 __device__ __forceinline__ void attend_store(const float (&qf)[NT][8], const float (&kf)[NT][8], const float (&vf)[2][4 * NT],
diff --git a/cvpr23_lfdm_amd/csrc/attn_lowres.hip b/cvpr23_lfdm_amd/csrc/attn_lowres.hip
--- a/cvpr23_lfdm_amd/csrc/attn_lowres.hip
+++ b/cvpr23_lfdm_amd/csrc/attn_lowres.hip
@@ -273,7 +273,7 @@
     const float mx = kmax[d];
     float s = 0.f;
     for (int n = part; n < hw; n += 8) {
-      const float e = expf(qkv[n * LDQ + DH + d] - mx);
+      const float e = fast_exp(qkv[n * LDQ + DH + d] - mx);
       qkv[n * LDQ + DH + d] = e;
       s += e;
     }
@@ -295,8 +295,8 @@
       const float4 v4 = *reinterpret_cast<const float4*>(qkv + n * LDQ + 2 * DH + e0);
       a0 = fmaf(e, v4.x, a0); a1 = fmaf(e, v4.y, a1); a2 = fmaf(e, v4.z, a2); a3 = fmaf(e, v4.w, a3);
     }
-    const float ss = ksum[d];
-    *reinterpret_cast<float4*>(&ctx[d][e0]) = make_float4(a0 / ss, a1 / ss, a2 / ss, a3 / ss);
+    const float ss = fast_rcp(ksum[d]);
+    *reinterpret_cast<float4*>(&ctx[d][e0]) = make_float4(a0 * ss, a1 * ss, a2 * ss, a3 * ss);
   }
   for (int n0 = 0; n0 < hw; n0 += 32) {
     const bool live = n0 + (tid >> 3) < hw;
@@ -304,10 +304,11 @@
     float4 q4 = *reinterpret_cast<const float4*>(qkv + n * LDQ + 4 * (tid & 7));
     float m = fmaxf(fmaxf(q4.x, q4.y), fmaxf(q4.z, q4.w));
     m = fmaxf(m, __shfl_xor(m, 1)); m = fmaxf(m, __shfl_xor(m, 2)); m = fmaxf(m, __shfl_xor(m, 4));
-    q4.x = expf(q4.x - m); q4.y = expf(q4.y - m); q4.z = expf(q4.z - m); q4.w = expf(q4.w - m);
+    q4.x = fast_exp(q4.x - m); q4.y = fast_exp(q4.y - m); q4.z = fast_exp(q4.z - m); q4.w = fast_exp(q4.w - m);
     float s = (q4.x + q4.y) + (q4.z + q4.w);
     s += __shfl_xor(s, 1); s += __shfl_xor(s, 2); s += __shfl_xor(s, 4);
-    q4.x = q4.x / s * ATT_SCALE; q4.y = q4.y / s * ATT_SCALE; q4.z = q4.z / s * ATT_SCALE; q4.w = q4.w / s * ATT_SCALE;
+    s = ATT_SCALE * fast_rcp(s);
+    q4.x *= s; q4.y *= s; q4.z *= s; q4.w *= s;
     if (live) *reinterpret_cast<float4*>(qkv + n * LDQ + 4 * (tid & 7)) = q4;
   }
   __syncthreads();
@@ -418,18 +419,19 @@
     for (int tj = 0; tj < NT; ++tj)
 #pragma unroll
       for (int r = 0; r < 4; ++r) {
-        const float e = (tj * 16 + lq * 4 + r) < L ? expf(st[tj][r] - m) : 0.f;
+        const float e = (tj * 16 + lq * 4 + r) < L ? fast_exp(st[tj][r] - m) : 0.f;
         st[tj][r] = e;
         sum += e;
       }
     sum += __shfl_xor(sum, 16);
     sum += __shfl_xor(sum, 32);
+    const float inv = fast_rcp(sum);
     f32x4 o0 = {0.f, 0.f, 0.f, 0.f}, o1 = o0;
 #pragma unroll
     for (int tj = 0; tj < NT; ++tj)
 #pragma unroll
       for (int r = 0; r < 4; ++r) {
-        const float p = st[tj][r] / sum;
+        const float p = st[tj][r] * inv;
         const float* vr = qkv + (16 * tj + 4 * lq + r) * LDQ + 2 * DH;
         o0 = mfma_16x16x4(p, vr[l15], o0);
         o1 = mfma_16x16x4(p, vr[16 + l15], o1);
diff --git a/cvpr23_lfdm_amd/csrc/conv_pw.hip b/cvpr23_lfdm_amd/csrc/conv_pw.hip
--- a/cvpr23_lfdm_amd/csrc/conv_pw.hip
+++ b/cvpr23_lfdm_amd/csrc/conv_pw.hip
@@ -241,8 +241,8 @@
         float4 rr = pre_r[g * TN + j];
         if (p.res_gn_partial) {
           const float4 ga = *reinterpret_cast<const float4*>(s_ga + col - n0), gb = *reinterpret_cast<const float4*>(s_gb + col - n0);
-          rr.x = siluf_(fmaf(rr.x, ga.x, gb.x)); rr.y = siluf_(fmaf(rr.y, ga.y, gb.y));
-          rr.z = siluf_(fmaf(rr.z, ga.z, gb.z)); rr.w = siluf_(fmaf(rr.w, ga.w, gb.w));
+          rr.x = silu_fast_(fmaf(rr.x, ga.x, gb.x)); rr.y = silu_fast_(fmaf(rr.y, ga.y, gb.y));
+          rr.z = silu_fast_(fmaf(rr.z, ga.z, gb.z)); rr.w = silu_fast_(fmaf(rr.w, ga.w, gb.w));
         }
         v.x += bb.x + rr.x; v.y += bb.y + rr.y; v.z += bb.z + rr.z; v.w += bb.w + rr.w;
       }
diff --git a/cvpr23_lfdm_amd/csrc/lfdm_device.h b/cvpr23_lfdm_amd/csrc/lfdm_device.h
--- a/cvpr23_lfdm_amd/csrc/lfdm_device.h
+++ b/cvpr23_lfdm_amd/csrc/lfdm_device.h
@@ -241,6 +241,13 @@
   for (int m = 32; m >= 1; m >>= 1) v = fmaxf(v, __shfl_xor(v, m));
   return v;
 }
+#if defined(LFDM_EMU_BUILD)
+static inline float fast_exp(float x) { return expf(x); }
+static inline float fast_rcp(float x) { return 1.0f / x; }
+#else
+__device__ __forceinline__ float fast_exp(float x) { return __expf(x); }
+__device__ __forceinline__ float fast_rcp(float x) { return __builtin_amdgcn_rcpf(x); }
+#endif
 __device__ __forceinline__ float sigmoidf_(float x) { return 1.0f / (1.0f + expf(-x)); }
 __device__ __forceinline__ float siluf_(float x) { return x / (1.0f + expf(-x)); }
 
diff --git a/cvpr23_lfdm_amd/csrc/linattn_fused.hip b/cvpr23_lfdm_amd/csrc/linattn_fused.hip
--- a/cvpr23_lfdm_amd/csrc/linattn_fused.hip
+++ b/cvpr23_lfdm_amd/csrc/linattn_fused.hip
@@ -97,13 +97,13 @@
     }
     m = fmaxf(m, __shfl_xor(m, 32));
     const float m_new = fmaxf(m_run, m);
-    const float alpha = expf(m_run - m_new);
+    const float alpha = fast_exp(m_run - m_new);
     float ssum = 0.f;
     float e[16];
 #pragma unroll
     for (int r = 0; r < 16; ++r) {
       const int tok = t0 + (r & 3) + 8 * (r >> 2) + 4 * kh;
-      e[r] = tok < n1 ? expf(ka[r] - m_new) : 0.f;
+      e[r] = tok < n1 ? fast_exp(ka[r] - m_new) : 0.f;
       ssum += e[r];
     }
     ssum += __shfl_xor(ssum, 32);
@@ -123,12 +123,24 @@
   }
 }
 
+template <bool FOLD>
 __global__ __launch_bounds__(256) void linattn_fused_merge_kernel(const float* __restrict__ part, int nsplit,
-                                                                  float* __restrict__ ctx_out) {
+                                                                  float* __restrict__ ctx_out, const float* __restrict__ wout) {
   constexpr int MAXS = 64;
   __shared__ float s_w[MAXS][DH];
+  __shared__ __attribute__((aligned(16))) float s_ctx[FOLD ? DH * DH : 4];
   const int tid = threadIdx.x;
   const float* base = part + (int64_t)blockIdx.x * nsplit * PART;
+  float4 wo[2][8];
+  if constexpr (FOLD) {
+    const int h = blockIdx.x & 7, cl = tid & 31;
+#pragma unroll
+    for (int cb = 0; cb < 2; ++cb)
+#pragma unroll
+      for (int j8 = 0; j8 < 8; ++j8)
+        wo[cb][j8] = *reinterpret_cast<const float4*>(wout + ((int64_t)(((h * 2 + cb) * 4 + (j8 >> 1)) * 64 + 32 * (j8 & 1) + cl)) * 4);
+  }
+  float acc[4];
   if (nsplit <= 8) {
     constexpr int PS = 8;
     float cv[4][PS], pm[PS], psum[PS];
@@ -148,10 +160,10 @@
       float den = 0.f, w[PS];
 #pragma unroll
       for (int p = 0; p < PS; ++p) {
-        w[p] = p < nsplit ? expf(pm[p] - mm) : 0.f;
+        w[p] = p < nsplit ? fast_exp(pm[p] - mm) : 0.f;
         den += w[p] * psum[p];
       }
-      const float inv = 1.0f / den;
+      const float inv = fast_rcp(den);
 #pragma unroll
       for (int p = 0; p < PS; ++p)
         if (p < nsplit) s_w[p][tid] = w[p] * inv;
@@ -159,36 +171,70 @@
     __syncthreads();
 #pragma unroll
     for (int e = 0; e < 4; ++e) {
+      const int d = (tid + 256 * e) >> 5;
+      float a = 0.f;
+#pragma unroll
+      for (int p = 0; p < PS; ++p)
+        if (p < nsplit) a += s_w[p][d] * cv[e][p];
+      acc[e] = a;
+    }
+  } else {
+    if (tid < DH) {
+      float mm = -3.0e38f;
+#pragma unroll 4
+      for (int p = 0; p < nsplit; ++p) mm = fmaxf(mm, base[(int64_t)p * PART + DH * DH + tid]);
+      float den = 0.f;
+#pragma unroll 4
+      for (int p = 0; p < nsplit; ++p) {
+        const float w = fast_exp(base[(int64_t)p * PART + DH * DH + tid] - mm);
+        s_w[p][tid] = w;
+        den += w * base[(int64_t)p * PART + DH * DH + DH + tid];
+      }
+      const float inv = fast_rcp(den);
+      for (int p = 0; p < nsplit; ++p) s_w[p][tid] *= inv;
+    }
+    __syncthreads();
+#pragma unroll
+    for (int e = 0; e < 4; ++e) {
       const int i = tid + 256 * e, d = i >> 5;
-      float acc = 0.f;
-#pragma unroll
-      for (int p = 0; p < PS; ++p)
-        if (p < nsplit) acc += s_w[p][d] * cv[e][p];
-      ctx_out[(int64_t)blockIdx.x * DH * DH + i] = acc;
-    }
-    return;
-  }
-  if (tid < DH) {
-    float mm = -3.0e38f;
+      float a = 0.f;
 #pragma unroll 4
-    for (int p = 0; p < nsplit; ++p) mm = fmaxf(mm, base[(int64_t)p * PART + DH * DH + tid]);
-    float den = 0.f;
-#pragma unroll 4
-    for (int p = 0; p < nsplit; ++p) {
-      const float w = expf(base[(int64_t)p * PART + DH * DH + tid] - mm);
-      s_w[p][tid] = w;
-      den += w * base[(int64_t)p * PART + DH * DH + DH + tid];
-    }
-    const float inv = 1.0f / den;
-    for (int p = 0; p < nsplit; ++p) s_w[p][tid] *= inv;
-  }
-  __syncthreads();
-  for (int i = tid; i < DH * DH; i += 256) {
-    const int d = i >> 5;
-    float acc = 0.f;
-#pragma unroll 4
-    for (int p = 0; p < nsplit; ++p) acc += s_w[p][d] * base[(int64_t)p * PART + i];
-    ctx_out[(int64_t)blockIdx.x * DH * DH + i] = acc;
+      for (int p = 0; p < nsplit; ++p) a += s_w[p][d] * base[(int64_t)p * PART + i];
+      acc[e] = a;
+    }
+  }
+  if constexpr (!FOLD) {
+#pragma unroll
+    for (int e = 0; e < 4; ++e) ctx_out[(int64_t)blockIdx.x * DH * DH + tid + 256 * e] = acc[e];
+  } else {
+#pragma unroll
+    for (int e = 0; e < 4; ++e) s_ctx[tid + 256 * e] = acc[e];
+    __syncthreads();
+    const float* crow = s_ctx + 4 * (tid >> 5) * DH;
+    float mt[2][4];
+#pragma unroll
+    for (int cb = 0; cb < 2; ++cb)
+#pragma unroll
+      for (int j = 0; j < 4; ++j) mt[cb][j] = 0.f;
+#pragma unroll
+    for (int j8 = 0; j8 < 8; ++j8)
+#pragma unroll
+      for (int j = 0; j < 4; ++j) {
+        const float4 c4 = *reinterpret_cast<const float4*>(crow + j * DH + 4 * j8);
+#pragma unroll
+        for (int cb = 0; cb < 2; ++cb) {
+          float a = mt[cb][j];
+          a = fmaf(wo[cb][j8].x, c4.x, a);
+          a = fmaf(wo[cb][j8].y, c4.y, a);
+          a = fmaf(wo[cb][j8].z, c4.z, a);
+          a = fmaf(wo[cb][j8].w, c4.w, a);
+          mt[cb][j] = a;
+        }
+      }
+#pragma unroll
+    for (int cb = 0; cb < 2; ++cb)
+      *reinterpret_cast<float4*>(ctx_out + ((int64_t)blockIdx.x * 2 * DH * DH / 4 + 256 * cb + tid) * 4) =
+          make_float4(mt[cb][0], mt[cb][1], mt[cb][2], mt[cb][3]);
   }
 }
 
@@ -218,11 +264,11 @@
     float sum = 0.f;
 #pragma unroll
     for (int r = 0; r < 16; ++r) {
-      q[r] = expf(q[r] - m);
+      q[r] = fast_exp(q[r] - m);
       sum += q[r];
     }
     sum += __shfl_xor(sum, 32);
-    const float inv = LA_SCALE / sum;
+    const float inv = LA_SCALE * fast_rcp(sum);
     const float* cb = ctx + ((int64_t)f * HEADS + h) * DH * DH + l31;
     f32x16 o;
 #pragma unroll
@@ -240,9 +286,8 @@
 
 constexpr int LDY = C + 4;
 __global__ __launch_bounds__(256, 2) void linattn_fused_out2_kernel(const float* __restrict__ x, int ldx, const float* __restrict__ wqkv,
-                                                                    const float* __restrict__ wout, const float* __restrict__ bias_out,
-                                                                    const float* __restrict__ ctx, int hw, float eps, float* __restrict__ out,
-                                                                    int ldo) {
+                                                                    const float* __restrict__ bias_out, const float* __restrict__ mt, int hw,
+                                                                    float eps, float* __restrict__ out, int ldo) {
   __shared__ __attribute__((aligned(16))) float s_y[4 * 32 * LDY];
   const int tid = threadIdx.x;
   const int wave = lfdm_uniform(tid >> 6);
@@ -259,6 +304,12 @@
     for (int r = 0; r < 16; ++r) yT[cb][r] = 0.f;
 #pragma unroll 1
   for (int h = 2 * wave; h < 2 * wave + 2; ++h) {
+    const float* msrc = mt + (((int64_t)f * HEADS + h) * (2 * DH * DH / 4) + lane) * 4;
+    float4 mf[2][4];
+#pragma unroll
+    for (int cb = 0; cb < 2; ++cb)
+#pragma unroll
+      for (int qd = 0; qd < 4; ++qd) mf[cb][qd] = *reinterpret_cast<const float4*>(msrc + (cb * 4 + qd) * 256);
     float wq[CH];
     load_wfrag(wqkv, 0, h, lane, wq);
     f32x16 q;
@@ -273,31 +324,22 @@
     float sum = 0.f;
 #pragma unroll
     for (int r = 0; r < 16; ++r) {
-      q[r] = expf(q[r] - m);
+      q[r] = fast_exp(q[r] - m);
       sum += q[r];
     }
     sum += __shfl_xor(sum, 32);
-    const float inv = LA_SCALE / sum;
-    const float* cb_ = ctx + ((int64_t)f * HEADS + h) * DH * DH + l31;
-    f32x16 oT;
-#pragma unroll
-    for (int r = 0; r < 16; ++r) oT[r] = 0.f;
-#pragma unroll
-    for (int r = 0; r < 16; ++r) oT = mfma_32x32x2(cb_[((r & 3) + 8 * (r >> 2) + 4 * kh) * DH], q[r] * inv, oT);
-#pragma unroll
-    for (int cb = 0; cb < 2; ++cb) {
-      const float* wsrc = wout + ((int64_t)((h * 2 + cb) * 4) * 64 + lane) * 4;
-      float4 wo[4];
-#pragma unroll
-      for (int qd = 0; qd < 4; ++qd) wo[qd] = *reinterpret_cast<const float4*>(wsrc + 256 * qd);
+    const float inv = LA_SCALE * fast_rcp(sum);
+#pragma unroll
+    for (int r = 0; r < 16; ++r) q[r] *= inv;
+#pragma unroll
+    for (int cb = 0; cb < 2; ++cb)
 #pragma unroll
       for (int qd = 0; qd < 4; ++qd) {
-        yT[cb] = mfma_32x32x2(wo[qd].x, oT[4 * qd + 0], yT[cb]);
-        yT[cb] = mfma_32x32x2(wo[qd].y, oT[4 * qd + 1], yT[cb]);
-        yT[cb] = mfma_32x32x2(wo[qd].z, oT[4 * qd + 2], yT[cb]);
-        yT[cb] = mfma_32x32x2(wo[qd].w, oT[4 * qd + 3], yT[cb]);
+        yT[cb] = mfma_32x32x2(mf[cb][qd].x, q[4 * qd + 0], yT[cb]);
+        yT[cb] = mfma_32x32x2(mf[cb][qd].y, q[4 * qd + 1], yT[cb]);
+        yT[cb] = mfma_32x32x2(mf[cb][qd].z, q[4 * qd + 2], yT[cb]);
+        yT[cb] = mfma_32x32x2(mf[cb][qd].w, q[4 * qd + 3], yT[cb]);
       }
-    }
   }
   float* ys = s_y + (wave * 32 + l31) * LDY;
 #pragma unroll
@@ -329,12 +371,12 @@
 
 extern "C" size_t lfdm_linear_attention_fused_ws_bytes(int n_frames, int hw) {
   const int nsplit = (hw + SPLIT_TOK - 1) / SPLIT_TOK;
-  return ((size_t)n_frames * HEADS * nsplit * PART + (size_t)n_frames * HEADS * DH * DH) * sizeof(float);
+  return ((size_t)n_frames * HEADS * nsplit * PART + (size_t)n_frames * HEADS * 2 * DH * DH) * sizeof(float);
 }
 
 namespace {
-void launch_ctx_and_merge(const float* x, int ldx, const float* wqkv, int n_frames, int hw, float ln_eps, void* ws, float** ctx_out,
-                          hipStream_t stream) {
+void launch_ctx_and_merge(const float* x, int ldx, const float* wqkv, const float* wout, int n_frames, int hw, float ln_eps, void* ws,
+                          float** ctx_out, hipStream_t stream) {
   const int tiles = (hw + 31) / 32;
   const int64_t pairs = (int64_t)n_frames * HEADS;
   int want = (int)((pairs <= 1536 ? 3072 : 4 * 3072 + pairs - 1) / pairs);
@@ -347,7 +389,8 @@
   float* part = (float*)ws;
   float* ctx = part + (size_t)n_frames * HEADS * ((hw + SPLIT_TOK - 1) / SPLIT_TOK) * PART;
   LFDM_LAUNCH(linattn_fused_ctx_kernel, dim3(n_frames * HEADS, nsplit), dim3(64), 0, stream, x, ldx, wqkv, hw, ln_eps, part, split_tok);
-  LFDM_LAUNCH(linattn_fused_merge_kernel, dim3(n_frames * HEADS), dim3(256), 0, stream, (const float*)part, nsplit, ctx);
+  if (wout) LFDM_LAUNCH((linattn_fused_merge_kernel<true>), dim3(n_frames * HEADS), dim3(256), 0, stream, (const float*)part, nsplit, ctx, wout);
+  else LFDM_LAUNCH((linattn_fused_merge_kernel<false>), dim3(n_frames * HEADS), dim3(256), 0, stream, (const float*)part, nsplit, ctx, wout);
   *ctx_out = ctx;
 }
 }
@@ -366,7 +409,7 @@
     return LFDM_EWORKSPACE;
   }
   float* ctx = nullptr;
-  launch_ctx_and_merge(x, ldx, wqkv, n_frames, hw, ln_eps, ws, &ctx, stream);
+  launch_ctx_and_merge(x, ldx, wqkv, nullptr, n_frames, hw, ln_eps, ws, &ctx, stream);
   const int64_t otiles = (int64_t)((hw + 31) / 32) * n_frames;
   const int hgroups = otiles >= 4096 ? 1 : (otiles >= 2048 ? 2 : 4);
   LFDM_LAUNCH(linattn_fused_out_kernel, dim3((hw + 31) / 32, n_frames, hgroups), dim3(64), 0, stream, x, ldx, wqkv,
@@ -388,9 +431,9 @@
     lfdm_set_error("linear_attention_fused_out: workspace too small");
     return LFDM_EWORKSPACE;
   }
-  float* ctx = nullptr;
-  launch_ctx_and_merge(x, ldx, wqkv, n_frames, hw, ln_eps, ws, &ctx, stream);
-  LFDM_LAUNCH(linattn_fused_out2_kernel, dim3((hw + 31) / 32, n_frames), dim3(256), 0, stream, x, ldx, wqkv, wout, bias_out, (const float*)ctx, hw,
+  float* mt = nullptr;
+  launch_ctx_and_merge(x, ldx, wqkv, wout, n_frames, hw, ln_eps, ws, &mt, stream);
+  LFDM_LAUNCH(linattn_fused_out2_kernel, dim3((hw + 31) / 32, n_frames), dim3(256), 0, stream, x, ldx, wqkv, bias_out, (const float*)mt, hw,
               ln_eps, out, ldo);
   return lfdm_check_launch("linear_attention_fused_out");
 }
diff --git a/cvpr23_lfdm_amd/csrc/norm.hip b/cvpr23_lfdm_amd/csrc/norm.hip
--- a/cvpr23_lfdm_amd/csrc/norm.hip
+++ b/cvpr23_lfdm_amd/csrc/norm.hip
@@ -164,10 +164,10 @@
     y.z = fmaf(v.z, a.z, d.z);
     y.w = fmaf(v.w, a.w, d.w);
     if (silu) {
-      y.x = siluf_(y.x);
-      y.y = siluf_(y.y);
-      y.z = siluf_(y.z);
-      y.w = siluf_(y.w);
+      y.x = silu_fast_(y.x);
+      y.y = silu_fast_(y.y);
+      y.z = silu_fast_(y.z);
+      y.w = silu_fast_(y.w);
     }
     if (rb) {
       const float4 r = k == 0 ? pre_r[0] : k == 1 ? pre_r[1] : rb[i];
diff --git a/cvpr23_lfdm_amd/csrc/small.hip b/cvpr23_lfdm_amd/csrc/small.hip
--- a/cvpr23_lfdm_amd/csrc/small.hip
+++ b/cvpr23_lfdm_amd/csrc/small.hip
@@ -311,8 +311,8 @@
       float s0 = 0.f, s1 = 0.f, s2 = 0.f;
 #pragma unroll
       for (int j = 0; j < 4; ++j) {
-        const float t0 = siluf_(fmaf(v[j].x, ra[j].x, rb[j].x)), t1 = siluf_(fmaf(v[j].y, ra[j].y, rb[j].y));
-        const float t2 = siluf_(fmaf(v[j].z, ra[j].z, rb[j].z)), t3 = siluf_(fmaf(v[j].w, ra[j].w, rb[j].w));
+        const float t0 = silu_fast_(fmaf(v[j].x, ra[j].x, rb[j].x)), t1 = silu_fast_(fmaf(v[j].y, ra[j].y, rb[j].y));
+        const float t2 = silu_fast_(fmaf(v[j].z, ra[j].z, rb[j].z)), t3 = silu_fast_(fmaf(v[j].w, ra[j].w, rb[j].w));
         s0 += (t0 * w0[j].x + t1 * w0[j].y) + (t2 * w0[j].z + t3 * w0[j].w);
         s1 += (t0 * w1[j].x + t1 * w1[j].y) + (t2 * w1[j].z + t3 * w1[j].w);
         s2 += (t0 * w2[j].x + t1 * w2[j].y) + (t2 * w2[j].z + t3 * w2[j].w);
@@ -338,7 +338,7 @@
       const float4 a = *reinterpret_cast<const float4*>(s_a + 4 * k), d = *reinterpret_cast<const float4*>(s_b + 4 * k);
       const float4 w0 = *reinterpret_cast<const float4*>(wl + 4 * k), w1 = *reinterpret_cast<const float4*>(wl + 512 + 4 * k);
       const float4 w2 = *reinterpret_cast<const float4*>(wl + 1024 + 4 * k);
-      const float t0 = siluf_(fmaf(v.x, a.x, d.x)), t1 = siluf_(fmaf(v.y, a.y, d.y)), t2 = siluf_(fmaf(v.z, a.z, d.z)), t3 = siluf_(fmaf(v.w, a.w, d.w));
+      const float t0 = silu_fast_(fmaf(v.x, a.x, d.x)), t1 = silu_fast_(fmaf(v.y, a.y, d.y)), t2 = silu_fast_(fmaf(v.z, a.z, d.z)), t3 = silu_fast_(fmaf(v.w, a.w, d.w));
       s0 += (t0 * w0.x + t1 * w0.y) + (t2 * w0.z + t3 * w0.w);
       s1 += (t0 * w1.x + t1 * w1.y) + (t2 * w1.z + t3 * w1.w);
       s2 += (t0 * w2.x + t1 * w2.y) + (t2 * w2.z + t3 * w2.w);
```
